# spcl/gms

Hardware: AMD Instinct MI355X
Metric: edges-intersected/sec + achieved HBM GB/s, RMAT-26 triangle count @1/2/4/8 GPU (higher is better)
Workload: dtype int32 ids / uint64 counts

## Files before the change

### gms_amd/capi.py

```python
import ctypes as C
import os
import weakref

import numpy as np

_HERE = os.path.dirname(os.path.abspath(__file__))
LIB_PATH = os.environ.get("GMSX_LIB") or os.path.join(_HERE, "lib", "libgmsx.so")

_i64p = np.ctypeslib.ndpointer(np.int64, flags="C_CONTIGUOUS")
_i32p = np.ctypeslib.ndpointer(np.int32, flags="C_CONTIGUOUS")
_u32p = np.ctypeslib.ndpointer(np.uint32, flags="C_CONTIGUOUS")

GEN_KRONECKER, GEN_UNIFORM = 0, 1
RELABEL_NEVER, RELABEL_AUTO, RELABEL_ALWAYS = 0, 1, 2
TC_AUTO, TC_ORIENTED, TC_FULL = 0, 1, 2
UPLOAD_DEFAULT, UPLOAD_TRUSTED, UPLOAD_FOR_TC = 0, 1, 2
PREPARE_TC = 1
SETOP_INTERSECT, SETOP_DIFFERENCE = 0, 1
OK, ERR_INVALID, ERR_NOMEM, ERR_IO, ERR_FORMAT, ERR_DIRECTED, ERR_NO_DEVICE = 0, -1, -2, -3, -4, -5, -6
ERR_DEVICE_MEM, ERR_NOT_CANONICAL, ERR_OVERFLOW, ERR_UNSUPPORTED, ERR_KERNEL, ERR_COMM, ERR_TIMEOUT = -7, -8, -9, -10, -11, -12, -13
COMM_ID_BYTES = 128

SYMBOLS = [
    "gmsx_strerror", "gmsx_version",
# ... 348 lines not shown
        _check(lib().gmsx_csr_save_sgx(self._h, os.fsencode(path)), "gmsx_csr_save_sgx")

    @property
    def is_mapped(self):
        return bool(lib().gmsx_csr_is_mapped(self._h))

    def relabel_by_degree(self):
        h = C.c_void_p()
        _check(lib().gmsx_csr_relabel_by_degree(self._h, C.byref(h)), "gmsx_csr_relabel_by_degree")
        return HostCSR(h)

    def worth_relabelling(self):
        return bool(lib().gmsx_csr_worth_relabelling(self._h))

    @property
    def num_nodes(self):
        return lib().gmsx_csr_num_nodes(self._h)

    @property
    def num_edges(self):
        return lib().gmsx_csr_num_edges(self._h)

    @property
    def nnz(self):
        return lib().gmsx_csr_num_edges_directed(self._h)

    def offsets(self):
        return np.ctypeslib.as_array(lib().gmsx_csr_offsets(self._h), shape=(self.num_nodes + 1,))

    def neighbors(self):
        nnz = self.nnz
        if nnz == 0:
            return np.zeros(0, dtype=np.int32)
        return np.ctypeslib.as_array(lib().gmsx_csr_neighbors(self._h), shape=(nnz,))

    def merge_elements(self):
        return int(lib().gmsx_csr_merge_elements(self._h))

    def fingerprint(self):
        return int(lib().gmsx_csr_fingerprint(self._h, 0)), int(lib().gmsx_csr_fingerprint(self._h, 1))

    def __del__(self):
        if getattr(self, "_h", None):
            lib().gmsx_csr_free(self._h)
            self._h = None


def set_host_threads(n=0):
    return int(lib().gmsx_set_host_threads(int(n)))


def set_option(name, value):
    _check(lib().gmsx_set_option(name.encode(), None if value is None else str(value).encode()), f"gmsx_set_option({name})")


def reset_options():
    lib().gmsx_reset_options()


def option_names():
    out, i, p = [], 0, C.c_char_p()
    while lib().gmsx_option_name(i, C.byref(p)) == 0:
        out.append(p.value.decode())
        i += 1
    return out


class options:

    def __init__(self, **kw):
        self.kw = kw

    def __enter__(self):
        for k, v in self.kw.items():
            set_option(k, v)
        return self

    def __exit__(self, *exc):
        for k in self.kw:
            set_option(k, None)
        return False


def init(device=-1):
    _check(lib().gmsx_init(device), "gmsx_init")


def set_stream(stream_ptr):
    _check(lib().gmsx_set_stream(C.c_void_p(stream_ptr)), "gmsx_set_stream")


def hbm_read_probe(nbytes=4 << 30, iterations=20):
    v = C.c_double(0)
    _check(lib().gmsx_hbm_read_probe(int(nbytes), int(iterations), C.byref(v)), "gmsx_hbm_read_probe")
    return v.value


def device_info():
    name = C.create_string_buffer(256)
    cu, mem = C.c_int(0), C.c_int64(0)
    _check(lib().gmsx_device_info(name, 256, C.byref(cu), C.byref(mem)), "gmsx_device_info")
    return {"name": name.value.decode(), "compute_units": cu.value, "hbm_bytes": mem.value}


class DeviceGraph:

    def __init__(self, handle):
        self._h = handle

    @classmethod
    def upload(cls, off, neigh, flags=UPLOAD_DEFAULT):
        off = np.ascontiguousarray(off, dtype=np.int64)
        neigh = np.ascontiguousarray(neigh, dtype=np.int32)
        h = C.c_void_p()
        _check(lib().gmsx_graph_upload(off.size - 1, off, neigh if neigh.size else np.zeros(1, np.int32), flags, C.byref(h)),
               "gmsx_graph_upload")
        g = cls(h)
        g._host = (weakref.ref(off), weakref.ref(neigh))
        return g

    @classmethod
    def from_csr(cls, csr, flags=UPLOAD_DEFAULT, shard=None):
        h = C.c_void_p()
        if shard is None:
            _check(lib().gmsx_graph_upload_csr(csr._h, flags, C.byref(h)), "gmsx_graph_upload_csr")
        else:
            _check(lib().gmsx_graph_upload_csr_shard(csr._h, flags, int(shard[0]), int(shard[1]), C.byref(h)), "gmsx_graph_upload_csr_shard")
        g = cls(h)
        g._host = (weakref.ref(csr),)
        return g

    num_nodes = property(lambda self: lib().gmsx_graph_num_nodes(self._h))
    num_edges = property(lambda self: lib().gmsx_graph_num_edges(self._h))
    device_bytes = property(lambda self: lib().gmsx_graph_device_bytes(self._h))
    max_out_degree = property(lambda self: lib().gmsx_graph_max_out_degree(self._h))
    tc_passes = property(lambda self: lib().gmsx_graph_tc_passes(self._h))

    def prepare(self, what=PREPARE_TC):
        _check(lib().gmsx_graph_prepare(self._h, what), "gmsx_graph_prepare")

    def tc_total(self, algo=TC_AUTO, stats=False):
        out, st = C.c_uint64(0), Stats()
        _check(lib().gmsx_tc_total(self._h, algo, C.byref(out), C.byref(st)), "gmsx_tc_total")
        return (int(out.value), st.as_dict()) if stats else int(out.value)

    def tc_partial(self, part, nparts, algo=TC_AUTO, stats=False):
        out, st = C.c_uint64(0), Stats()
        _check(lib().gmsx_tc_partial(self._h, algo, part, nparts, C.byref(out), C.byref(st)), "gmsx_tc_partial")
        return (int(out.value), st.as_dict()) if stats else int(out.value)

    BREAKDOWN = ["hub_rows_list", "hub_rows_bitset", "hub_rows_delta", "tail_rows_list", "tail_rows_delta", "entries", "pivot_containers",
                 "of_which_inline_rows", "light_streamed_hub_rows", "light_streamed_tail_rows", "light_pivot_lists_and_descriptors",
                 "count_entries", "count_inline_entries", "count_work_items", "count_light_streamed_members",
                 "core_matrix", "core_k", "reserved17", "reserved18", "reserved19", "reserved20"]
    BREAKDOWN_BYTES = ("hub_rows_list", "hub_rows_bitset", "hub_rows_delta", "tail_rows_list", "tail_rows_delta", "entries", "pivot_containers",
                       "light_streamed_hub_rows", "light_streamed_tail_rows", "light_pivot_lists_and_descriptors", "core_matrix")

    def tc_stream_breakdown(self):
        out = np.zeros(21, dtype=np.uint64)
        _check(lib().gmsx_tc_stream_breakdown(self._h, out), "gmsx_tc_stream_breakdown")
        return dict(zip(self.BREAKDOWN, (int(x) for x in out)))

    def tc_row_histogram(self):
        out = np.zeros(256, dtype=np.uint64)
        _check(lib().gmsx_tc_row_histogram(self._h, out), "gmsx_tc_row_histogram")
        return out[:240].reshape(5, 24, 2).astype(np.int64), out[240:].astype(np.int64)

    def tc_comembership(self, batch):
        out = np.zeros(8, dtype=np.uint64)
        _check(lib().gmsx_tc_comembership(self._h, int(batch), out), "gmsx_tc_comembership")
        return dict(entries=int(out[0]), units=int(out[1]), distinct_rows=int(out[2]), batched_units=int(out[3]), items=int(out[4]))

    def tc_vertex_count2(self, stats=False):
        c, st = np.zeros(self.num_nodes, dtype=np.int64), Stats()
        _check(lib().gmsx_tc_vertex_count2(self._h, c, C.byref(st)), "gmsx_tc_vertex_count2")
        return (c, st.as_dict()) if stats else c

    def intersect_count_batch(self, u, v, stats=False):
        u = np.ascontiguousarray(u, dtype=np.int32)
        v = np.ascontiguousarray(v, dtype=np.int32)
        out, st = np.zeros(max(u.size, 1), dtype=np.uint32), Stats()
        _check(lib().gmsx_intersect_count_batch(self._h, u.size, u if u.size else np.zeros(1, np.int32),
                                                v if v.size else np.zeros(1, np.int32), out, C.byref(st)),
               "gmsx_intersect_count_batch")
        out = out[:u.size]
        return (out, st.as_dict()) if stats else out

    def set_op_batch(self, op, u, v, stats=False):
        code = {"intersect": SETOP_INTERSECT, "difference": SETOP_DIFFERENCE}[op]
        u = np.ascontiguousarray(u, dtype=np.int32)
        v = np.ascontiguousarray(v, dtype=np.int32)
        uu, vv = (u if u.size else np.zeros(1, np.int32)), (v if v.size else np.zeros(1, np.int32))
        off, st = np.zeros(u.size + 1, dtype=np.int64), Stats()
        _check(lib().gmsx_set_op_batch(self._h, code, u.size, uu, vv, off, None, 0, C.byref(st)), "gmsx_set_op_batch (sizing)")
        ids = np.zeros(max(int(off[-1]), 1), dtype=np.int32)
        _check(lib().gmsx_set_op_batch(self._h, code, u.size, uu, vv, off, ids.ctypes.data_as(C.c_void_p), int(off[-1]), C.byref(st)), "gmsx_set_op_batch")
        ids = ids[:int(off[-1])]
        return (off, ids, st.as_dict()) if stats else (off, ids)

    SIM = {"jaccard": 0, "overlap": 1, "adamic_adar": 2, "resource": 3, "common_neighbors": 4, "total_neighbors": 5, "pref_attachment": 6}

    def vertex_similarity_batch(self, metric, u, v, stats=False):
        u = np.ascontiguousarray(u, dtype=np.int32)
        v = np.ascontiguousarray(v, dtype=np.int32)
        out, st = np.zeros(max(u.size, 1), dtype=np.float64), Stats()
        m = self.SIM[metric] if isinstance(metric, str) else int(metric)
        _check(lib().gmsx_vertex_similarity_batch(self._h, m, u.size, u if u.size else np.zeros(1, np.int32),
                                                  v if v.size else np.zeros(1, np.int32), out, C.byref(st)), "gmsx_vertex_similarity_batch")
        out = out[:u.size]
        return (out, st.as_dict()) if stats else out

    def kclique_count(self, k, stats=False):
        ordered, cliques, st = C.c_uint64(0), C.c_uint64(0), Stats()
        _check(lib().gmsx_kclique_count(self._h, k, C.byref(ordered), C.byref(cliques), C.byref(st)), "gmsx_kclique_count")
        r = (int(ordered.value), int(cliques.value))
        return (r + (st.as_dict(),)) if stats else r

    def kclique_star_count(self, k, members=True, stats=False):
        stars, mem, st = C.c_uint64(0), C.c_uint64(0), Stats()
        _check(lib().gmsx_kclique_star_count(self._h, k, C.byref(stars), C.byref(mem) if members else None, C.byref(st)), "gmsx_kclique_star_count")
        r = (int(stars.value), int(mem.value) if members else None)
        return (r + (st.as_dict(),)) if stats else r

    def kclique_star_list_info(self, k, cliques_only=False, part=0, nparts=1):
        info = KcliqueStarListInfo()
        flags = KCSTAR_CLIQUES_ONLY if cliques_only else KCSTAR_DEFAULT
        _check(lib().gmsx_kclique_star_list(self._h, k, flags, part, nparts, None, None, None, 0, 0, C.byref(info), None),
               "gmsx_kclique_star_list (sizing)")
        return info.as_dict()

    def kclique_star_list(self, k, cliques_only=False, part=0, nparts=1, stats=False):
        info, st = KcliqueStarListInfo(), Stats()
        flags = KCSTAR_CLIQUES_ONLY if cliques_only else KCSTAR_DEFAULT
        _check(lib().gmsx_kclique_star_list(self._h, k, flags, part, nparts, None, None, None, 0, 0, C.byref(info), C.byref(st)),
               "gmsx_kclique_star_list (sizing)")
        sizing = st.as_dict()
        nc, nm = int(info.cliques), int(info.star_members)
        cl = np.zeros(max(nc * k, 1), dtype=np.int32)
        soff = mem = None
        if not cliques_only:
            soff = np.zeros(nc + 1, dtype=np.int64)
            mem = np.zeros(max(nm, 1), dtype=np.int32)
        _check(lib().gmsx_kclique_star_list(self._h, k, flags, part, nparts, cl.ctypes.data_as(C.c_void_p),
                                            None if cliques_only else soff.ctypes.data_as(C.c_void_p),
                                            None if cliques_only else mem.ctypes.data_as(C.c_void_p), nc, nm, C.byref(info), C.byref(st)),
               "gmsx_kclique_star_list")
        cl = cl[:nc * k].reshape(nc, k)
        if mem is not None:
            mem = mem[:nm]
        if stats:
            return cl, soff, mem, {"sizing": sizing, "fill": st.as_dict(), "info": info.as_dict()}
        return cl, soff, mem

    def kclique_partial(self, k, part, nparts, stats=False):
        out, st = C.c_uint64(0), Stats()
        _check(lib().gmsx_kclique_partial(self._h, k, part, nparts, C.byref(out), C.byref(st)), "gmsx_kclique_partial")
        return (int(out.value), st.as_dict()) if stats else int(out.value)

    def bk_count(self, rank=None, stats=False):
        out, st = C.c_uint64(0), Stats()
        rp = None
        if rank is not None:
            rank = np.ascontiguousarray(rank, dtype=np.int32)
            rp = rank.ctypes.data_as(C.c_void_p)
        _check(lib().gmsx_bk_count(self._h, rp, C.byref(out), C.byref(st)), "gmsx_bk_count")
        return (int(out.value), st.as_dict()) if stats else int(out.value)

    def bk_partial(self, part, nparts, rank=None, stats=False):
        out, st = C.c_uint64(0), Stats()
        rp = None
        if rank is not None:
            rank = np.ascontiguousarray(rank, dtype=np.int32)
            rp = rank.ctypes.data_as(C.c_void_p)
        _check(lib().gmsx_bk_partial(self._h, rp, part, nparts, C.byref(out), C.byref(st)), "gmsx_bk_partial")
        return (int(out.value), st.as_dict()) if stats else int(out.value)

    def bk_list_info(self, rank=None, part=0, nparts=1):
        info = BkListInfo()
        rp = None
        if rank is not None:
            rank = np.ascontiguousarray(rank, dtype=np.int32)
            rp = rank.ctypes.data_as(C.c_void_p)
        _check(lib().gmsx_bk_list(self._h, rp, part, nparts, None, None, 0, 0, C.byref(info), None), "gmsx_bk_list (sizing)")
        return info.as_dict()

    def bk_list(self, rank=None, part=0, nparts=1, stats=False):
        info, st = BkListInfo(), Stats()
        rp = None
        if rank is not None:
            rank = np.ascontiguousarray(rank, dtype=np.int32)
            rp = rank.ctypes.data_as(C.c_void_p)
        _check(lib().gmsx_bk_list(self._h, rp, part, nparts, None, None, 0, 0, C.byref(info), C.byref(st)), "gmsx_bk_list (sizing)")
        sizing = st.as_dict()
        off = np.zeros(int(info.cliques) + 1, dtype=np.int64)
        mem = np.zeros(max(int(info.members), 1), dtype=np.int32)
        _check(lib().gmsx_bk_list(self._h, rp, part, nparts, off.ctypes.data_as(C.c_void_p), mem.ctypes.data_as(C.c_void_p), off.size,
                                  int(info.members), C.byref(info), C.byref(st)), "gmsx_bk_list")
        mem = mem[:int(info.members)]
        if stats:
            return off, mem, {"sizing": sizing, "fill": st.as_dict(), "info": info.as_dict()}
        return off, mem

    def adg_rank(self, epsilon=0.001, rank_format=True, stats=False):
        out, rounds, st = np.zeros(max(self.num_nodes, 1), dtype=np.int32), C.c_int32(0), Stats()
        _check(lib().gmsx_adg_rank(self._h, float(epsilon), int(bool(rank_format)), out, C.byref(rounds), C.byref(st)), "gmsx_adg_rank")
        r = (out[:self.num_nodes], int(rounds.value))
        return (r + (st.as_dict(),)) if stats else r
# ... 257 lines not shown
```

### gms_amd/csrc/hip/device_graph.hip

```cpp
#include "device_graph.hpp"

#include <algorithm>
#include <mutex>
#include <array>
#include <chrono>
#include <cstdio>
#include <cstdlib>
#include <cstring>
#include <memory>
#include <new>
#include <random>

#include <rocprim/device/device_radix_sort.hpp>
#include <rocprim/device/device_scan.hpp>
#include <rocprim/device/device_segmented_radix_sort.hpp>
#include <rocprim/iterator/transform_iterator.hpp>

#include "../host/gmsx_internal.hpp"
#include "../host/tc_core_plan.hpp"
#include "kc4_mfma.hpp"

namespace gmsx {

Ctx &ctx() {
    static Ctx c;
    return c;
}

int ensure_init() { return ctx().device >= 0 ? GMSX_OK : gmsx_init(-1); }


__device__ __forceinline__ unsigned long long arc_mix(unsigned long long x) {
    x ^= x >> 30;
    x *= 0xbf58476d1ce4e5b9ull;
    x ^= x >> 27;
    x *= 0x94d049bb133111ebull;
    x ^= x >> 31;
    return x;
}
__global__ __launch_bounds__(256) void k_validate(int64_t n, const int64_t *__restrict__ off,
                                                  const int32_t *__restrict__ adj, int check_symmetry, unsigned long long key0,
                                                  unsigned long long key1,
                                                  unsigned long long *__restrict__ acc ) {
    const int lane = threadIdx.x & 63;
    const int64_t wave0 = (int64_t(blockIdx.x) * blockDim.x + threadIdx.x) >> 6;
    const int64_t nwaves = (int64_t(gridDim.x) * blockDim.x) >> 6;
    unsigned flags = 0;
    unsigned long long elems = 0;
    unsigned long long maxdeg = 0;
    unsigned long long f0 = 0, r0 = 0, f1 = 0, r1 = 0;
    for (int64_t u = wave0; u < n; u += nwaves) {
        const int64_t b = off[u], e = off[u + 1];
        const unsigned long long du = (unsigned long long)(e - b);
        if (du > maxdeg) maxdeg = du;
        if (lane == 0) elems += du * du;
        for (int64_t j = b + lane; j < e; j += 64) {
            const int32_t v = adj[j];
            if (v < 0 || v >= n) { flags |= 2; continue; }
            if (v == u) flags |= 4;
            if (j + 1 < e && adj[j + 1] <= v) flags |= 1;
            if (check_symmetry) {
                const unsigned long long uv = ((unsigned long long)uint32_t(u) << 32) | uint32_t(v), vu = ((unsigned long long)uint32_t(v) << 32) | uint32_t(u);
                f0 += arc_mix(uv ^ key0);
                r0 += arc_mix(vu ^ key0);
                f1 += arc_mix(uv * 0x9e3779b97f4a7c15ull + key1);
                r1 += arc_mix(vu * 0x9e3779b97f4a7c15ull + key1);
            }
        }
    }
    for (int s = 32; s > 0; s >>= 1) {
        elems += __shfl_down(elems, s);
        flags |= __shfl_down(flags, s);
        const unsigned long long o = __shfl_down(maxdeg, s);
        maxdeg = o > maxdeg ? o : maxdeg;
        f0 += __shfl_down(f0, s);
        r0 += __shfl_down(r0, s);
        f1 += __shfl_down(f1, s);
        r1 += __shfl_down(r1, s);
    }
    if (lane == 0) {
        if (flags) atomicOr(&acc[0], (unsigned long long)flags);
        if (elems) atomicAdd(&acc[1], elems);
        atomicMax(&acc[2], maxdeg);
        if (check_symmetry) {
            atomicAdd(&acc[3], f0);
            atomicAdd(&acc[4], r0);
            atomicAdd(&acc[5], f1);
            atomicAdd(&acc[6], r1);
        }
    }
}

__global__ void k_rank_keys(int64_t n, const int64_t *__restrict__ off, unsigned long long *__restrict__ keys) {
    const int64_t u = int64_t(blockIdx.x) * blockDim.x + threadIdx.x;
    if (u < n) keys[u] = ((unsigned long long)(off[u + 1] - off[u]) << 32) | (unsigned long long)u;
}
__global__ void k_assign_ids(int64_t n, const unsigned long long *__restrict__ sorted_keys, int32_t *__restrict__ oldid,
                             int32_t *__restrict__ newid) {
    const int64_t i = int64_t(blockIdx.x) * blockDim.x + threadIdx.x;
    if (i < n) {
        const int32_t o = int32_t(sorted_keys[i] & 0xffffffffull);
        oldid[i] = o;
        newid[o] = int32_t(i);
    }
}

__global__ __launch_bounds__(256) void k_count_parts(int64_t n, const int64_t *__restrict__ off, const int32_t *__restrict__ adj,
                                                     const int32_t *__restrict__ newid, int hub_limit, int64_t *__restrict__ hcnt,
                                                     int64_t *__restrict__ tcnt, int32_t *__restrict__ dplus) {
    const int lane = threadIdx.x & 63;
    const int64_t wave0 = (int64_t(blockIdx.x) * blockDim.x + threadIdx.x) >> 6;
    const int64_t nwaves = (int64_t(gridDim.x) * blockDim.x) >> 6;
    for (int64_t u = wave0; u < n; u += nwaves) {
        const int64_t b = off[u], e = off[u + 1];
        const int32_t nu = newid[u];
        int ch = 0, ct = 0;
        for (int64_t j = b + lane; j < e; j += 64) {
            const int32_t nv = newid[adj[j]];
            if (nv < nu) {
                if (nv < hub_limit) ch++; else ct++;
            }
        }
        for (int s = 32; s > 0; s >>= 1) {
            ch += __shfl_down(ch, s);
            ct += __shfl_down(ct, s);
        }
        if (lane == 0) {
            hcnt[nu] = (ch + 1) & ~1;
            tcnt[nu] = ct;
            dplus[nu] = ch + ct;
        }
    }
}

__global__ __launch_bounds__(256) void k_fill_parts(int64_t n, const int64_t *__restrict__ off, const int32_t *__restrict__ adj,
                                                    const int32_t *__restrict__ newid, int hub_limit, const int64_t *__restrict__ hoff,
                                                    const int64_t *__restrict__ toff, uint16_t *__restrict__ hadj,
                                                    int32_t *__restrict__ tadj) {
    const int lane = threadIdx.x & 63;
    const int64_t wave0 = (int64_t(blockIdx.x) * blockDim.x + threadIdx.x) >> 6;
    const int64_t nwaves = (int64_t(gridDim.x) * blockDim.x) >> 6;
    for (int64_t u = wave0; u < n; u += nwaves) {
        const int64_t b = off[u], e = off[u + 1];
        const int32_t nu = newid[u];
        int64_t ho = hoff[nu], to = toff[nu];
        const int64_t hend = hoff[nu + 1];
        for (int64_t base = b; base < e; base += 64) {
            const int64_t j = base + lane;
            bool kh = false, kt = false;
            int32_t nv = 0;
            if (j < e) {
                nv = newid[adj[j]];
                kh = nv < nu && nv < hub_limit;
                kt = nv < nu && nv >= hub_limit;
            }
            const unsigned long long mh = __ballot(kh), mt = __ballot(kt);
            const unsigned long long below = (1ull << lane) - 1ull;
            if (kh) hadj[ho + __popcll(mh & below)] = uint16_t(nv);
            if (kt) tadj[to + __popcll(mt & below)] = nv;
            ho += __popcll(mh);
            to += __popcll(mt);
        }
        if (lane == 0 && ho < hend) hadj[ho] = 0xFFFF;
    }
}

__device__ inline uint32_t delta_encode(const uint16_t *__restrict__ row, int len, uint32_t *__restrict__ emit) {
    uint32_t units = 0;
    int i = 0;
    while (i < len && row[i] != 0xFFFFu) {
        uint32_t w[4] = {row[i], 0u, 0u, 0u};
        uint32_t cur = row[i];
// ... 212 lines not shown
    else
        for (int64_t w = 0; w < units * 4; ++w) dst[w] = w < len ? uint32_t(tadj[b + w]) : 0xfffffffeu;
}

__global__ void k_dense_sizes(int32_t limit, const int32_t *__restrict__ dplus, int64_t *__restrict__ sizes) {
    const int32_t v = int32_t(blockIdx.x * blockDim.x + threadIdx.x);
    if (v < limit) sizes[v] = bitset_words(v);
    if (v == limit) sizes[v] = 0;
}
__global__ __launch_bounds__(256) void k_dense_fill(int32_t limit, const int64_t *__restrict__ hoff, const uint16_t *__restrict__ hadj,
                                                    const int64_t *__restrict__ toff, const int32_t *__restrict__ tadj,
                                                    const int64_t *__restrict__ bmoff, uint32_t *__restrict__ pool) {
    const int lane = threadIdx.x & 63;
    const int32_t wave0 = int32_t((int64_t(blockIdx.x) * blockDim.x + threadIdx.x) >> 6);
    const int32_t nwaves = int32_t((int64_t(gridDim.x) * blockDim.x) >> 6);
    for (int32_t v = wave0; v < limit; v += nwaves) {
        const int64_t b = bmoff[v];
        if (bmoff[v + 1] == b) continue;
        for (int64_t j = hoff[v] + lane; j < hoff[v + 1]; j += 64) {
            const uint32_t id = hadj[j];
            if (id != 0xFFFFu) atomicOr(&pool[b + (id >> 5)], 1u << (id & 31u));
        }
        for (int64_t j = toff[v] + lane; j < toff[v + 1]; j += 64) {
            const uint32_t id = uint32_t(tadj[j]);
            atomicOr(&pool[b + (id >> 5)], 1u << (id & 31u));
        }
    }
}
__global__ __launch_bounds__(256) void k_core_fill(int32_t K, int WS, const int64_t *__restrict__ hoff, const uint16_t *__restrict__ hadj,
                                                   uint32_t *__restrict__ bits) {
    const int lane = threadIdx.x & 63;
    const int32_t wave0 = int32_t((int64_t(blockIdx.x) * blockDim.x + threadIdx.x) >> 6);
    const int32_t nwaves = int32_t((int64_t(gridDim.x) * blockDim.x) >> 6);
    for (int32_t i = wave0; i < K; i += nwaves)
        for (int64_t j = hoff[i] + lane; j < hoff[i + 1]; j += 64) {
            const uint32_t id = hadj[j];
            if (id < uint32_t(i)) atomicOr(&bits[size_t(i) * size_t(WS) + (id >> 5)], 1u << (id & 31u));
        }
}
__global__ __launch_bounds__(256) void k_core_units(int32_t cap, const int64_t *__restrict__ hoff, const uint16_t *__restrict__ hadj,
                                                    const int32_t *__restrict__ dplus, unsigned long long *__restrict__ bucket) {
    const int lane = threadIdx.x & 63;
    const int32_t wave0 = int32_t((int64_t(blockIdx.x) * blockDim.x + threadIdx.x) >> 6);
    const int32_t nwaves = int32_t((int64_t(gridDim.x) * blockDim.x) >> 6);
    for (int32_t u = wave0; u < cap; u += nwaves) {
        const int64_t hb = hoff[u];
        const int hl = int(hoff[u + 1] - hb);
        unsigned long long units = 0;
        for (int i = lane; i < hl; i += 64) {
            const uint32_t v = hadj[hb + i];
            if (v >= uint32_t(u)) continue;
            const uint32_t ids = uint32_t(min(i, dplus[v]));
            units += min((ids + 7u) / 8u, (v + 127u) / 128u);
        }
        for (int s = 32; s > 0; s >>= 1) units += __shfl_down(units, s);
        if (lane == 0 && units) atomicAdd(&bucket[u / kTcCoreBucket], units);
    }
}
__global__ __launch_bounds__(256) void k_tail_split(int64_t n, const int64_t *__restrict__ toff, const int32_t *__restrict__ tadj, int32_t limit,
                                                    int32_t *__restrict__ tsplit) {
    const int lane = threadIdx.x & 63;
    const int64_t wave0 = (int64_t(blockIdx.x) * blockDim.x + threadIdx.x) >> 6;
    const int64_t nwaves = (int64_t(gridDim.x) * blockDim.x) >> 6;
    for (int64_t u = wave0; u < n; u += nwaves) {
        int c = 0;
        for (int64_t j = toff[u] + lane; j < toff[u + 1]; j += 64) c += tadj[j] < limit;
        for (int s = 32; s > 0; s >>= 1) c += __shfl_down(c, s);
        if (lane == 0) tsplit[u] = c;
    }
}

__global__ void k_order_keys(int64_t n, const int32_t *__restrict__ dplus, int32_t *__restrict__ keys, int32_t *__restrict__ vals) {
    const int64_t i = int64_t(blockIdx.x) * blockDim.x + threadIdx.x;
    if (i < n) {
        keys[i] = dplus[i];
        vals[i] = int32_t(i);
    }
}

__global__ void k_warm(unsigned long long *p) {
    if (p) p[0] = 0;
}
__global__ void k_count_ge(int64_t n, const int32_t *__restrict__ order, const int32_t *__restrict__ dplus, int32_t thr, int64_t *__restrict__ out) {
    int64_t lo = 0, hi = n;
    while (lo < hi) {
        const int64_t mid = (lo + hi) >> 1;
        if (dplus[order[mid]] >= thr) lo = mid + 1; else hi = mid;
    }
    out[0] = lo;
}
__global__ void k_task_limits(int64_t n, const unsigned long long *__restrict__ srow, const unsigned long long *__restrict__ srow2,
                              const unsigned long long *__restrict__ trow, uint32_t hub_max, uint32_t tail_max, unsigned long long *__restrict__ out) {
    const int64_t v = int64_t(blockIdx.x) * blockDim.x + threadIdx.x;
    if (v >= n) return;
    if ((srow[v] & 0x3fffffull) > hub_max || (srow2[v] & 0x3fffffull) > hub_max || (trow[v] & 0x3fffffull) > tail_max) atomicOr(out, 1ull);
}

static constexpr int kInlineChunk = 64;
static constexpr int kDefaultInlineFirst = 28;
static constexpr int kInlineFirstMax = 64;
__device__ __forceinline__ bool takes_inline(int32_t v, int32_t inline_limit, const int32_t *__restrict__ dplus) {
    return v < inline_limit || dplus[v] >= kHeavy;
}
template <bool FILL>
__global__ __launch_bounds__(256) void k_inline_rows(int64_t first, int64_t end, const int32_t *__restrict__ order, const int64_t *__restrict__ hoff,
                                                     const uint16_t *__restrict__ hadj, const int64_t *__restrict__ toff, const int32_t *__restrict__ tadj,
                                                     const int32_t *__restrict__ dplus, int32_t inline_limit, int inline_first, int32_t core, const int32_t *__restrict__ opos, int nparts, int part,
                                                     unsigned long long *__restrict__ cnt_h,
                                                     unsigned long long *__restrict__ cnt_t, const int64_t *__restrict__ ihoff,
                                                     const int64_t *__restrict__ itoff, int64_t base_h, uint16_t *__restrict__ pool_h, int64_t base_t,
                                                     int32_t *__restrict__ pool_t) {
    const int lane = threadIdx.x & 63;
    const int64_t wave0 = (int64_t(blockIdx.x) * blockDim.x + threadIdx.x) >> 6;
    const int64_t nwaves = (int64_t(gridDim.x) * blockDim.x) >> 6;
    for (int64_t pos = first + wave0; pos < end; pos += nwaves) {
        const int32_t u = order[pos];
        if (u < core) continue;
        const int64_t hb = hoff[u], tb = toff[u];
        const int first_u = dplus[u] >= kHeavy ? inline_first : kInlineFirstMax;
        const int hl = min(int(hoff[u + 1] - hb), first_u), tl = min(int(toff[u + 1] - tb), first_u - hl);
        int32_t mv = 0x7fffffff;
        if (lane < hl) {
            const uint32_t x = hadj[hb + lane];
            if (x != 0xFFFFu) mv = int32_t(x);
        } else if (lane - hl < tl) {
            mv = tadj[tb + (lane - hl)];
        }
        const bool valid = mv != 0x7fffffff, is_tail = valid && lane >= hl;
        const unsigned long long vmask = __ballot(valid);
        const int nhub = __popcll(__ballot(valid && lane < hl));
        const int below = __popcll(vmask & ((1ull << lane) - 1ull));
        const bool give = valid && below > 0 && takes_inline(mv, inline_limit, dplus);
        const bool mine = give && (nparts <= 1 || shard_of(opos[mv], nparts) == part);
        const int nh = mine ? (is_tail ? nhub : below) : 0;
        const int nt = mine && is_tail ? lane - hl : 0;
        if (!FILL) {
            if (nh) atomicAdd(&cnt_h[mv], (unsigned long long)nh);
            if (nt) atomicAdd(&cnt_t[mv], (unsigned long long)nt);
        } else {
            int64_t at_h = 0, at_t = 0;
            if (nh) at_h = (base_h + ihoff[mv]) * 8 + int64_t(atomicAdd(&cnt_h[mv], (unsigned long long)nh));
            if (nt) at_t = (base_t + itoff[mv]) * 4 + int64_t(atomicAdd(&cnt_t[mv], (unsigned long long)nt));
            for (int k = 0; k < nhub; ++k) {
                const int32_t x = __shfl(mv, k);
                if (k < nh) pool_h[at_h + k] = uint16_t(x);
            }
            for (int k = 0; k < tl; ++k) {
                const int32_t x = __shfl(mv, hl + k);
                if (k < nt) pool_t[at_t + k] = x;
            }
        }
    }
}
__global__ void k_inline_units(int64_t n, const unsigned long long *__restrict__ ids_h, const unsigned long long *__restrict__ ids_t,
                               int64_t *__restrict__ units_h, int64_t *__restrict__ units_t) {
    const int64_t v = int64_t(blockIdx.x) * blockDim.x + threadIdx.x;
    if (v > n) return;
    units_h[v] = v < n ? int64_t((ids_h[v] + 7) / 8) : 0;
    units_t[v] = v < n ? int64_t((ids_t[v] + 3) / 4) : 0;
}
static constexpr int kDefaultHotWindows = 0, kDefaultHotKB = 2048, kDefaultHotMin = 16;
__device__ __forceinline__ int64_t receiver_of(int32_t w, const int32_t *__restrict__ dplus, const int32_t *__restrict__ opos, const int64_t *__restrict__ lidx,
                                               int64_t n_heavy) {
    return dplus[w] >= kHeavy ? int64_t(opos[w]) : n_heavy + lidx[w];
}
__global__ void k_opos(int64_t n, const int32_t *__restrict__ order, int32_t *__restrict__ opos) {
    const int64_t p = int64_t(blockIdx.x) * blockDim.x + threadIdx.x;
    if (p < n) opos[order[p]] = int32_t(p);
}
__global__ void k_light_flags(int64_t limit, const int32_t *__restrict__ dplus, int64_t *__restrict__ flags) {
    const int64_t w = int64_t(blockIdx.x) * blockDim.x + threadIdx.x;
    if (w <= limit) flags[w] = (w < limit && dplus[w] < kHeavy) ? 1 : 0;
}
__global__ void k_recv_vertices(int64_t n_heavy, int64_t limit, const int32_t *__restrict__ order, const int32_t *__restrict__ dplus, const int64_t *__restrict__ lidx,
                                int32_t *__restrict__ recv_v) {
    const int64_t i = int64_t(blockIdx.x) * blockDim.x + threadIdx.x;
    if (i < n_heavy) recv_v[i] = order[i];
    if (i < limit && dplus[i] < kHeavy) recv_v[n_heavy + lidx[i]] = int32_t(i);
}
template <bool FILL>
__global__ void k_inline_entries(int64_t n, const int32_t *__restrict__ dplus, const int32_t *__restrict__ opos, const int64_t *__restrict__ lidx, int64_t n_heavy,
                                 int32_t inline_limit, const int64_t *__restrict__ ihoff, const int64_t *__restrict__ itoff, int64_t base_h, int64_t base_t,
                                 uint32_t *__restrict__ cnt, uint32_t *__restrict__ cur, const int64_t *__restrict__ hbeg, const int64_t *__restrict__ tbeg,
                                 TaskList htask, TaskList ttask, unsigned long long *__restrict__ totals, TcClasses cc) {
    const int kClasses = cc.count();
    const int64_t v = int64_t(blockIdx.x) * blockDim.x + threadIdx.x;
    if (v >= n) return;
    const int64_t uh = ihoff[v + 1] - ihoff[v], ut = itoff[v + 1] - itoff[v];
    if (uh == 0 && ut == 0) return;
    if (dplus[v] < kHeavy && v >= inline_limit) return;
    const int64_t p = receiver_of(int32_t(v), dplus, opos, lidx, n_heavy);
    uint32_t *c = cnt + p * kClasses;
    for (int64_t o = 0; o < uh; o += kInlineChunk) {
        const unsigned long long units = (unsigned long long)min(int64_t(kInlineChunk), uh - o);
        const unsigned long long d = ((unsigned long long)(base_h + ihoff[v] + o) << 24) | ((unsigned long long)kFormList << 22) | units;
        const int cls = hub_class(cc, d);
        if (!FILL) atomicAdd(&c[cls], 1u);
        else htask.put(hbeg[p] + c[cls] + atomicAdd(&cur[p * kClasses + cls], 1u), d);
    }
    for (int64_t o = 0; o < ut; o += kInlineChunk) {
        const unsigned long long units = (unsigned long long)min(int64_t(kInlineChunk), ut - o);
        const unsigned long long d = ((unsigned long long)(base_t + itoff[v] + o) << 24) | ((unsigned long long)kFormList << 22) | units;
        const int cls = tail_class(cc, d);
        if (!FILL) atomicAdd(&c[cls], 1u);
        else ttask.put(tbeg[p] + c[cls] + atomicAdd(&cur[p * kClasses + cls], 1u), d);
    }
    if (!FILL) {
        atomicAdd(&totals[0], (unsigned long long)((uh + kInlineChunk - 1) / kInlineChunk));
        atomicAdd(&totals[1], (unsigned long long)((ut + kInlineChunk - 1) / kInlineChunk));
    }
}
__global__ void k_list_sizes(int64_t n_recv, uint32_t *__restrict__ cnt, int64_t *__restrict__ hcnt, int64_t *__restrict__ tcnt, TcClasses cc) {
    const int kClasses = cc.count(), hub_end = cc.tail_base();
    const int64_t p = int64_t(blockIdx.x) * blockDim.x + threadIdx.x;
    if (p > n_recv) return;
    if (p == n_recv) { hcnt[p] = 0; tcnt[p] = 0; return; }
    uint32_t *c = cnt + p * kClasses;
    uint32_t run = 0;
    for (int k = 0; k < hub_end; ++k) { const uint32_t x = c[k]; c[k] = run; run += x; }
    hcnt[p] = run;
    run = 0;
    for (int k = hub_end; k < kClasses; ++k) { const uint32_t x = c[k]; c[k] = run; run += x; }
    tcnt[p] = run;
}

__global__ void k_ledge_count(int64_t first, int64_t end, const int32_t *__restrict__ order, const int64_t *__restrict__ toff, const int32_t *__restrict__ tadj,
                              const int32_t *__restrict__ tsplit, const int32_t *__restrict__ dplus, int32_t core, int64_t *__restrict__ cnt) {
    const int64_t pos = first + int64_t(blockIdx.x) * blockDim.x + threadIdx.x;
    if (pos > end) return;
    int64_t c = 0;
    if (pos < end) {
        const int32_t u = order[pos];
        const int64_t tb = toff[u];
        const int tl = int(toff[u + 1] - tb);
        if (u >= core)
            for (int i = tsplit[u]; i < tl; ++i) c += dplus[tadj[tb + i]] < kHeavy ? 1 : 0;
    }
    cnt[pos - first] = c;
}
__global__ void k_ledge_fill(int64_t first, int64_t end, const int32_t *__restrict__ order, const int64_t *__restrict__ hoff, const int64_t *__restrict__ toff,
                             const int32_t *__restrict__ tadj, const int32_t *__restrict__ tsplit, const int32_t *__restrict__ dplus,
                             int32_t core, const int64_t *__restrict__ ebeg, int nparts, int part, uint4 *__restrict__ ledge) {
    const int64_t pos = first + int64_t(blockIdx.x) * blockDim.x + threadIdx.x;
    if (pos >= end) return;
    const int32_t u = order[pos];
    if (u < core) return;
    const int64_t hb = hoff[u], tb = toff[u];
    const int tl = int(toff[u + 1] - tb);
    const unsigned long long hu = (unsigned long long)hb | ((unsigned long long)(hoff[u + 1] - hb) << 40);
    int64_t e = ebeg[pos - first];
    for (int i = tsplit[u]; i < tl; ++i) {
        const int32_t v = tadj[tb + i];
        if (dplus[v] >= kHeavy) continue;
        if (nparts <= 1 || shard_of(e, nparts) == part) {
            const unsigned long long tu = (unsigned long long)tb | ((unsigned long long)i << 40);
            const unsigned long long hv = (unsigned long long)hoff[v] | ((unsigned long long)(hoff[v + 1] - hoff[v]) << 40);
            const unsigned long long tv = (unsigned long long)toff[v] | ((unsigned long long)(toff[v + 1] - toff[v]) << 40);
            const int64_t slot = nparts <= 1 ? e : e / nparts;
            ledge[2 * slot] = make_uint4(uint32_t(hu), uint32_t(hu >> 32), uint32_t(tu), uint32_t(tu >> 32));
            ledge[2 * slot + 1] = make_uint4(uint32_t(hv), uint32_t(hv >> 32), uint32_t(tv), uint32_t(tv >> 32));
        }
        ++e;
    }
}

__global__ void k_lpack_count(int64_t first, int64_t end, const int32_t *__restrict__ order, const int64_t *__restrict__ hoff, const uint16_t *__restrict__ hadj,
                              const int64_t *__restrict__ toff, const int32_t *__restrict__ tadj, const int32_t *__restrict__ tsplit, const int32_t *__restrict__ dplus,
                              int32_t core, int64_t *__restrict__ cnt) {
    const int64_t p = int64_t(blockIdx.x) * blockDim.x + threadIdx.x, nl = end - first;
    if (p >= nl) return;
    int64_t c[kLightClasses];
#pragma unroll
    for (int k = 0; k < kLightClasses; ++k) c[k] = 0;
    const int32_t u = order[first + p];
    if (u >= core) {
        const int64_t tb = toff[u];
        const int tl = int(toff[u + 1] - tb), ah = light_hub_ids(hoff, hadj, u);
        for (int i = tsplit[u]; i < tl; ++i) {
            const int32_t v = tadj[tb + i];
            if (dplus[v] >= kHeavy) continue;
            const int cls = light_class(ah, i, light_hub_ids(hoff, hadj, v), int(toff[v + 1] - toff[v]));
#pragma unroll
            for (int k = 0; k < kLightClasses; ++k) c[k] += cls == k ? 1 : 0;
        }
    }
#pragma unroll
    for (int k = 0; k < kLightClasses; ++k) cnt[int64_t(k) * nl + p] = c[k];
}
struct LpackPlan {
    int64_t class_beg[kLightClasses];
    int64_t unit_base[kLightClasses];
};
__device__ __forceinline__ uint4 lpack_hub_unit(const uint16_t *__restrict__ row, int len, int q) {
    uint32_t w[4];
#pragma unroll
    for (int j = 0; j < 4; ++j) {
        const int i = 8 * q + 2 * j;
        const uint32_t lo = i < len ? row[i] : 0xFFFFu, hi = i + 1 < len ? row[i + 1] : 0xFFFFu;
        w[j] = lo | (hi << 16);
    }
    return make_uint4(w[0], w[1], w[2], w[3]);
}
__device__ __forceinline__ uint4 lpack_tail_unit(const int32_t *__restrict__ row, int len, int q, uint32_t filler) {
    uint32_t w[4];
#pragma unroll
    for (int j = 0; j < 4; ++j) w[j] = 4 * q + j < len ? uint32_t(row[4 * q + j]) : filler;
    return make_uint4(w[0], w[1], w[2], w[3]);
}
__global__ void k_lpack_fill(int64_t first, int64_t end, const int32_t *__restrict__ order, const int64_t *__restrict__ hoff, const uint16_t *__restrict__ hadj,
                             const int64_t *__restrict__ toff, const int32_t *__restrict__ tadj, const int32_t *__restrict__ tsplit, const int32_t *__restrict__ dplus,
                             int32_t core, const int64_t *__restrict__ beg, const LpackPlan plan, int nparts, int part, uint4 *__restrict__ lpack) {
    const int64_t p = int64_t(blockIdx.x) * blockDim.x + threadIdx.x, nl = end - first;
    if (p >= nl) return;
    const int32_t u = order[first + p];
    if (u < core) return;
    int64_t next[kLightClasses];
#pragma unroll
    for (int k = 0; k < kLightClasses; ++k) next[k] = beg[int64_t(k) * nl + p] - plan.class_beg[k];
    const int64_t hb = hoff[u], tb = toff[u];
    const int tl = int(toff[u + 1] - tb), ah = light_hub_ids(hoff, hadj, u);
    for (int i = tsplit[u]; i < tl; ++i) {
        const int32_t v = tadj[tb + i];
        if (dplus[v] >= kHeavy) continue;
        const int64_t hv = hoff[v], tv = toff[v];
        const int bh = light_hub_ids(hoff, hadj, v), bt = int(toff[v + 1] - tv);
        const int cls = light_class(ah, i, bh, bt);
        int64_t k = 0, base = 0;
#pragma unroll
        for (int c = 0; c < kLightClasses; ++c)
            if (cls == c) {
                k = next[c]++;
                base = plan.unit_base[c];
            }
        if (nparts > 1 && shard_of(k, nparts) != part) continue;
        const LightShape sh = light_shape(cls);
        uint4 *blk = lpack + base + (nparts <= 1 ? k : k / nparts) * sh.stride();
        for (int q = 0; q < sh.ah; ++q) *blk++ = lpack_hub_unit(hadj + hb, ah, q);
        for (int q = 0; q < sh.at; ++q) *blk++ = lpack_tail_unit(tadj + tb, i, q, 0xFFFFFFFFu);
        for (int q = 0; q < sh.bh; ++q) *blk++ = lpack_hub_unit(hadj + hv, bh, q);
        for (int q = 0; q < sh.bt; ++q) *blk++ = lpack_tail_unit(tadj + tv, bt, q, 0xFFFFFFFEu);
    }
}

__device__ __forceinline__ uint32_t cut_hub_units(const uint32_t *__restrict__ spool, unsigned long long d, int below, int32_t v) {
    const uint32_t units = uint32_t(d) & 0x3fffffu, form = (uint32_t(d) >> 22) & 3u;
    if (form == kFormList) return min(units, uint32_t(below + 7) / 8u);
    if (form == kFormBitset) return min(units, uint32_t(v + 127) / 128u);
    const uint4 *row = reinterpret_cast<const uint4 *>(spool) + (d >> 24);
    uint32_t lo = 0, hi = units;
    while (lo < hi) {
        const uint32_t mid = (lo + hi) >> 1;
        if (int32_t(row[mid].x & 0xffffu) < v) lo = mid + 1; else hi = mid;
    }
    return lo;
}
__device__ __forceinline__ uint32_t cut_tail_units(const uint32_t *__restrict__ tpool, unsigned long long d, int below, int32_t v) {
    const uint32_t units = uint32_t(d) & 0x3fffffu, form = (uint32_t(d) >> 22) & 3u;
    if (form != kFormDelta) return min(units, uint32_t(below + 3) / 4u);
    const uint4 *row = reinterpret_cast<const uint4 *>(tpool) + (d >> 24);
    uint32_t lo = 0, hi = units;
    while (lo < hi) {
        const uint32_t mid = (lo + hi) >> 1;
        if (int32_t(row[mid].x) < v) lo = mid + 1; else hi = mid;
    }
    return lo;
}
__device__ __forceinline__ uint32_t claim_by_class(uint32_t *ctr, int cls, bool active, int lane) {
    uint32_t mine = 0;
    unsigned long long todo = __ballot(active);
    while (todo) {
        const int leader = __ffsll((long long)todo) - 1;
        const int c = __builtin_amdgcn_readlane(cls, leader);
        const unsigned long long same = __ballot(active && cls == c);
        uint32_t base = 0;
        if (lane == leader) base = atomicAdd(&ctr[c], uint32_t(__popcll(same)));
        base = uint32_t(__builtin_amdgcn_readlane(int(base), leader));
        if (active && cls == c) mine = base + uint32_t(__popcll(same & ((1ull << lane) - 1ull)));
        todo &= ~same;
    }
    return mine;
}
template <bool FILL>
__global__ __launch_bounds__(256) void k_task_lists(int64_t n_heavy, const int32_t *__restrict__ order, const int64_t *__restrict__ hoff,
                                                    const uint16_t *__restrict__ hadj, const int64_t *__restrict__ toff, const int32_t *__restrict__ tadj,
                                                    const int32_t *__restrict__ dplus, const unsigned long long *__restrict__ srow,
                                                    const unsigned long long *__restrict__ srow2, const int32_t *__restrict__ ksplit,
                                                    const unsigned long long *__restrict__ trow, int two_sided, const int32_t *__restrict__ opos,
                                                    uint32_t *__restrict__ cnt, uint32_t *__restrict__ cur, const int64_t *__restrict__ hbeg,
                                                    const int64_t *__restrict__ tbeg, TaskList htask, TaskList ttask,
                                                    int32_t *__restrict__ tunits, unsigned long long *__restrict__ reversed, const uint32_t *__restrict__ spool,
                                                    const uint32_t *__restrict__ tpool, int32_t inline_limit, int inline_first, int32_t core, int nparts, int part, TcClasses cc) {
    const int kClasses = cc.count();
    const int lane = threadIdx.x & 63;
    const int64_t wave0 = (int64_t(blockIdx.x) * blockDim.x + threadIdx.x) >> 6;
    const int64_t nwaves = (int64_t(gridDim.x) * blockDim.x) >> 6;
    unsigned long long rev = 0;
    for (int64_t pos = wave0; pos < n_heavy; pos += nwaves) {
        const int32_t u = order[pos];
        if (u < core) continue;
        const int64_t hb = hoff[u], tb = toff[u];
        const int hl = int(hoff[u + 1] - hb), tl = int(toff[u + 1] - tb);
        const unsigned long long du_s = srow[u], du_s2 = srow2[u], du_t = trow[u];
        const int ks_u = ksplit[u];
        uint32_t *cu = cnt + pos * kClasses, *ru = cur + pos * kClasses;
        const bool own_u = nparts <= 1 || shard_of(pos, nparts) == part;
        int kept = 0;
        for (int base = 0; base < hl + tl; base += 64) {
            const int i = base + lane;
            int32_t v = -1;
            if (i < hl) {
                const uint32_t x = hadj[hb + i];
                if (x != 0xFFFFu) v = int32_t(x);
            } else if (i < hl + tl) v = tadj[tb + i - hl];
            if (v >= 0 && i > 0 && i < inline_first && takes_inline(v, inline_limit, dplus)) v = -1;
            bool reverse = false;
            uint32_t ch = 0, ch2 = 0, ct = 0;
            if (v >= 0 && i > 0 && two_sided && dplus[v] >= kHeavy) {
                if (i < hl) {
                    ch = cut_hub_units(spool, du_s, i, v);
                    if (du_s2 && i > ks_u) ch2 = cut_hub_units(spool, du_s2, i - ks_u, v);
                } else {
                    ch = uint32_t(du_s) & 0x3fffffu;
                    ch2 = uint32_t(du_s2) & 0x3fffffu;
                }
                ct = (i < hl || toff[v + 1] == toff[v]) ? 0u : cut_tail_units(tpool, du_t, i - hl, v);
                const uint32_t keep = uint32_t(srow[v] & 0x3fffffull) + uint32_t(srow2[v] & 0x3fffffull) + (i > hl ? uint32_t(trow[v] & 0x3fffffull) : 0u);
                reverse = ch + ch2 + ct < keep;
            }
            const bool fwd = v >= 0 && !reverse && own_u;
            if (reverse && nparts > 1 && shard_of(opos[v], nparts) != part) v = -1;
            const unsigned long long fh = (fwd && i > 0) ? srow[v] : 0ull, fh2 = (fwd && i > 0) ? srow2[v] : 0ull, ft = (fwd && i > hl) ? trow[v] : 0ull;
            const bool fh_on = (fh & 0x3fffffull) != 0, fh2_on = (fh2 & 0x3fffffull) != 0, ft_on = (ft & 0x3fffffull) != 0;
            const uint32_t sh = claim_by_class(FILL ? ru : cu, hub_class(cc, fh), fh_on, lane);
            const uint32_t sh2 = claim_by_class(FILL ? ru : cu, hub_class(cc, fh2), fh2_on, lane);
            const uint32_t st = claim_by_class(FILL ? ru : cu, tail_class(cc, ft), ft_on, lane);
            if (FILL) {
                if (fh_on) htask.put(hbeg[pos] + cu[hub_class(cc, fh)] + sh, fh);
                if (fh2_on) htask.put(hbeg[pos] + cu[hub_class(cc, fh2)] + sh2, fh2);
                if (ft_on) ttask.put(tbeg[pos] + cu[tail_class(cc, ft)] + st, ft);
            }
            kept += __popcll(__ballot(fwd));
            if (v >= 0 && reverse) {
                const int64_t pv = opos[v];
                const unsigned long long rh = ch ? (du_s & ~0x3fffffull) | ch : 0ull, rh2 = ch2 ? (du_s2 & ~0x3fffffull) | ch2 : 0ull,
                                         rt = ct ? (du_t & ~0x3fffffull) | ct : 0ull;
                uint32_t *cv = cnt + pv * kClasses;
                if (!FILL) {
                    if (rh) atomicAdd(&cv[hub_class(cc, rh)], 1u);
                    if (rh2) atomicAdd(&cv[hub_class(cc, rh2)], 1u);
                    if (rt) atomicAdd(&cv[tail_class(cc, rt)], 1u);
                    atomicAdd(&tunits[pv], 1);
                    ++rev;
                } else {
                    uint32_t *rv = cur + pv * kClasses;
                    if (rh) htask.put(hbeg[pv] + cv[hub_class(cc, rh)] + atomicAdd(&rv[hub_class(cc, rh)], 1u), rh);
                    if (rh2) htask.put(hbeg[pv] + cv[hub_class(cc, rh2)] + atomicAdd(&rv[hub_class(cc, rh2)], 1u), rh2);
                    if (rt) ttask.put(tbeg[pv] + cv[tail_class(cc, rt)] + atomicAdd(&rv[tail_class(cc, rt)], 1u), rt);
                }
            }
        }
        if (!FILL && lane == 0 && kept) atomicAdd(&tunits[pos], kept);
    }
    if (!FILL) {
        for (int s = 32; s > 0; s >>= 1) rev += __shfl_down(rev, s);
        if (lane == 0 && rev) atomicAdd(reversed, rev);
    }
}
__global__ void k_item_counts(int64_t n_recv, const int64_t *__restrict__ lbeg, const uint32_t *__restrict__ cnt, TcClasses cc, int phases, int64_t *__restrict__ items) {
    const int64_t p = int64_t(blockIdx.x) * blockDim.x + threadIdx.x;
    if (p > n_recv) return;
    if (p == n_recv) { items[int64_t(phases) * n_recv] = 0; return; }
    for (int ph = 0; ph < phases; ++ph) {
        int64_t b = 0, e = lbeg[p + 1] - lbeg[p];
        if (phases > 1) hub_phase_range(cc, cnt + p * cc.count(), e, ph, &b, &e);
        items[int64_t(ph) * n_recv + p] = (e - b + kTaskChunk - 1) / kTaskChunk;
    }
}
__global__ void k_item_fill(int64_t n_recv, const int32_t *__restrict__ recv_v, const int32_t *__restrict__ opos, const int64_t *__restrict__ lbeg,
                            const int64_t *__restrict__ ioff, TaskList task, const int64_t *__restrict__ coff, int kind,
                            const uint32_t *__restrict__ cnt, TcClasses cc, int phases, gmsx_tc_item *__restrict__ items) {
    const int64_t p = int64_t(blockIdx.x) * blockDim.x + threadIdx.x;
    if (p >= n_recv) return;
    const int32_t w = recv_v[p];
    const uint64_t cont = uint64_t(coff[w]) | (uint64_t(coff[w + 1] - coff[w]) << 40);
    for (int ph = 0; ph < phases; ++ph) {
    int64_t b = 0, e = lbeg[p + 1] - lbeg[p];
    if (phases > 1) hub_phase_range(cc, cnt + p * cc.count(), e, ph, &b, &e);
    b += lbeg[p];
    e += lbeg[p];
    int64_t k = ioff[int64_t(ph) * n_recv + p];
    for (int64_t x = b; x < e; x += kTaskChunk, ++k) {
        const int ne = int(min(int64_t(kTaskChunk), e - x));
        gmsx_tc_item it{};
        it.bc = uint64_t(x) | (uint64_t(ne) << 40);
        it.cont = cont;
        it.pivot = w;
        it.pos = opos[w];
        it.kind = uint32_t(kind);
        for (int f = 0; f < 4; ++f) {
            int lo = 0, hi = ne;
            while (lo < hi) {
                const int mid = (lo + hi) >> 1;
                if (int((uint32_t(task.get(x + mid)) >> 22) & 3u) < f) lo = mid + 1; else hi = mid;
            }
            it.fbeg[f] = uint16_t(lo);
        }
        items[k] = it;
    }
    }
}

static int grid_for_waves(int64_t rows) {
    const int64_t want = (rows + 3) / 4;
    const int64_t cap = int64_t(ctx().compute_units > 0 ? ctx().compute_units : 256) * 32;
    return int(want < 1 ? 1 : (want > cap ? cap : want));
}

template <class T>
static int dmalloc(T **p, int64_t count, gmsx_graph *g, int line = __builtin_LINE()) {
    const size_t bytes = size_t(count > 0 ? count : 1) * sizeof(T);
    const bool trace = opt("MEM_TRACE") != nullptr;
    if (trace && g && bytes >= (1u << 20)) std::fprintf(stderr, "gmsx mem: device_graph.hip:%d %.3f GB (elements of %zu B)\n", line, double(bytes) * 1e-9, sizeof(T));
    if (g && g->tc_building && g->tc_limit_bytes > 0 && g->device_bytes + int64_t(bytes) - g->tc_base_bytes > g->tc_limit_bytes) {
        *p = nullptr;
        return GMSX_ERR_DEVICE_MEM;
    }
    if (hipMalloc(reinterpret_cast<void **>(p), bytes) != hipSuccess) {
        (void)hipGetLastError();
        *p = nullptr;
        return GMSX_ERR_DEVICE_MEM;
    }
    if (g) g->device_bytes += int64_t(bytes);
    return GMSX_OK;
}

struct DevGuard {
    void *p;
    ~DevGuard() { (void)hipFree(p); }
};

static void free_tc(gmsx_graph *g) {
    auto drop = [](auto *&p) {
        (void)hipFree(p);
        p = nullptr;
    };
    drop(g->tsplit); drop(g->srow); drop(g->srow2); drop(g->ksplit); drop(g->spool); drop(g->trow); drop(g->htask.lo); drop(g->htask.hi); drop(g->ttask.lo); drop(g->ttask.hi); drop(g->hitem); drop(g->titem); drop(g->tunits);
    drop(g->ledge); drop(g->lpack); drop(g->tpool); drop(g->shard_hitem); drop(g->shard_titem); drop(g->core_bits);
    g->tc_core = 0;
    g->shard_idx_part = g->shard_idx_nparts = -1;
    g->device_bytes -= g->tc_bytes;
    g->tc_bytes = 0;
    g->tc_ready = false;
    g->htask_entries = g->ttask_entries = g->hitems = g->titems = g->inline_hentries = g->inline_tentries = 0;
    g->n_ledge = g->ledge_total = 0;
    for (int c = 0; c < 8; ++c) g->lpack_base[c] = g->lpack_n[c] = g->lpack_total[c] = 0;
    g->task_reverse = g->inline_units = g->spool_units = g->tpool_units = 0;
    g->stats_part = g->stats_nparts = -1;
}

static void free_graph(gmsx_graph *g) {
    if (!g) return;
    (void)hipFree(g->off);
    (void)hipFree(g->adj);
    (void)hipFree(g->newid);
    (void)hipFree(g->oldid);
    (void)hipFree(g->hoff);
    (void)hipFree(g->hadj);
    (void)hipFree(g->toff);
    (void)hipFree(g->tadj);
    (void)hipFree(g->bmoff);
    (void)hipFree(g->bmpool);
    (void)hipFree(g->tsplit);
    (void)hipFree(g->srow);
    (void)hipFree(g->srow2);
    (void)hipFree(g->ksplit);
    (void)hipFree(g->spool);
    (void)hipFree(g->trow);
    (void)hipFree(g->htask.lo);
    (void)hipFree(g->htask.hi);
    (void)hipFree(g->ttask.lo);
    (void)hipFree(g->ttask.hi);
    (void)hipFree(g->hitem);
    (void)hipFree(g->titem);
    (void)hipFree(g->tunits);
    (void)hipFree(g->shard_hitem);
    (void)hipFree(g->shard_titem);
    (void)hipFree(g->ledge);
    (void)hipFree(g->lpack);
    (void)hipFree(g->core_bits);
    (void)hipFree(g->tpool);
    (void)hipFree(g->dplus);
    (void)hipFree(g->order);
    (void)hipFree(g->kc_rel);
    (void)hipFree(g->kc_aoff);
    (void)hipFree(g->kc_arena);
    (void)hipFree(g->kc_rec);
    (void)hipFree(g->kc_item);
    (void)hipFree(g->kc_relt);
    (void)hipFree(g->kc_rect);
    (void)hipFree(g->kc_itemt);
    (void)hipFree(g->scratch);
    (void)hipFree(g->acc);
    delete g;
}

int exclusive_scan_i64(const int64_t *in, int64_t *out, int64_t count, hipStream_t s) {
    size_t tmp_bytes = 0;
    GMSX_HIP(rocprim::exclusive_scan(nullptr, tmp_bytes, in, out, int64_t(0), size_t(count), rocprim::plus<int64_t>(), s));
    void *tmp = nullptr;
    GMSX_HIP(hipMalloc(&tmp, tmp_bytes ? tmp_bytes : 8));
    DevGuard g_tmp{tmp};
    GMSX_HIP(rocprim::exclusive_scan(tmp, tmp_bytes, in, out, int64_t(0), size_t(count), rocprim::plus<int64_t>(), s));
    GMSX_HIP(hipStreamSynchronize(s));
    return GMSX_OK;
}

struct OffsetMinus {
    int64_t base;
    __host__ __device__ int64_t operator()(int64_t x) const { return x - base; }
};
__global__ void k_lower_bound_i64(int64_t count, const int64_t *__restrict__ a, int64_t target, int64_t *__restrict__ out) {
    int64_t lo = 0, hi = count;
    while (lo < hi) {
        const int64_t mid = (lo + hi) >> 1;
        if (a[mid] < target) lo = mid + 1; else hi = mid;
    }
    out[0] = lo;
}
template <class K>
static int sort_rows(K *keys, int64_t entries, int64_t n, const int64_t *d_off, int end_bit, hipStream_t s) {
    if (n <= 0 || entries <= 0) return GMSX_OK;
    int64_t chunk = int64_t(1) << 31;
    if (const char *e = opt("SORT_CHUNK")) {
        const long long v = std::atoll(e);
        if (v > 0) chunk = v;
    }
    int64_t *d_v = nullptr;
    GMSX_HIP(hipMalloc(reinterpret_cast<void **>(&d_v), sizeof(int64_t)));
    DevGuard g_v{d_v};
    GMSX_HIP(hipStreamSynchronize(s));
    int64_t v0 = 0, base = 0;
    while (v0 < n) {
        int64_t v1 = n;
        if (entries - base > chunk) {
            hipLaunchKernelGGL(k_lower_bound_i64, dim3(1), dim3(1), 0, s, n + 1, d_off, base + chunk + 1, d_v);
            GMSX_HIP(hipStreamSynchronize(s));
            GMSX_HIP(hipMemcpy(&v1, d_v, sizeof(int64_t), hipMemcpyDeviceToHost));
            v1 = std::max(v0 + 1, std::min(n, v1 - 1));
        }
        int64_t end = 0;
        GMSX_HIP(hipMemcpy(&end, d_off + v1, sizeof(int64_t), hipMemcpyDeviceToHost));
        const int64_t cnt = end - base;
        if (cnt >= (int64_t(1) << 32)) return GMSX_ERR_UNSUPPORTED;
        if (cnt > 0) {
            K *sorted = nullptr;
            GMSX_HIP(hipMalloc(reinterpret_cast<void **>(&sorted), size_t(cnt) * sizeof(K)));
            DevGuard g_sorted{sorted};
            auto begin = rocprim::make_transform_iterator(d_off + v0, OffsetMinus{base});
            auto endit = rocprim::make_transform_iterator(d_off + v0 + 1, OffsetMinus{base});
            size_t tmp_bytes = 0;
            GMSX_HIP(rocprim::segmented_radix_sort_keys(nullptr, tmp_bytes, keys + base, sorted, unsigned(cnt), unsigned(v1 - v0), begin, endit, 0, end_bit, s));
            void *tmp = nullptr;
            GMSX_HIP(hipMalloc(&tmp, tmp_bytes ? tmp_bytes : 8));
            DevGuard g_tmp{tmp};
            GMSX_HIP(rocprim::segmented_radix_sort_keys(tmp, tmp_bytes, keys + base, sorted, unsigned(cnt), unsigned(v1 - v0), begin, endit, 0, end_bit, s));
            GMSX_HIP(hipMemcpyAsync(keys + base, sorted, size_t(cnt) * sizeof(K), hipMemcpyDeviceToDevice, s));
            GMSX_HIP(hipStreamSynchronize(s));
        }
        v0 = v1;
        base = end;
    }
    return GMSX_OK;
}

template <class K, class V>
static int sort_segment_pairs(K *keys, V *vals, int64_t entries, int64_t n, const int64_t *d_off, int end_bit, hipStream_t s) {
    if (n <= 0 || entries <= 0) return GMSX_OK;
    int64_t chunk = int64_t(1) << 31;
    if (const char *e = opt("SORT_CHUNK")) {
        const long long v = std::atoll(e);
        if (v > 0) chunk = v;
    }
    int64_t *d_v = nullptr;
    GMSX_HIP(hipMalloc(reinterpret_cast<void **>(&d_v), sizeof(int64_t)));
    DevGuard g_v{d_v};
    GMSX_HIP(hipStreamSynchronize(s));
    int64_t v0 = 0, base = 0;
    while (v0 < n) {
        int64_t v1 = n;
        if (entries - base > chunk) {
            hipLaunchKernelGGL(k_lower_bound_i64, dim3(1), dim3(1), 0, s, n + 1, d_off, base + chunk + 1, d_v);
            GMSX_HIP(hipStreamSynchronize(s));
            GMSX_HIP(hipMemcpy(&v1, d_v, sizeof(int64_t), hipMemcpyDeviceToHost));
            v1 = std::max(v0 + 1, std::min(n, v1 - 1));
        }
        int64_t end = 0;
        GMSX_HIP(hipMemcpy(&end, d_off + v1, sizeof(int64_t), hipMemcpyDeviceToHost));
        const int64_t cnt = end - base;
        if (cnt >= (int64_t(1) << 32)) return GMSX_ERR_UNSUPPORTED;
        if (cnt > 0) {
            K *k_out = nullptr;
            V *v_out = nullptr;
            GMSX_HIP(hipMalloc(reinterpret_cast<void **>(&k_out), size_t(cnt) * sizeof(K)));
            DevGuard g_ko{k_out};
            GMSX_HIP(hipMalloc(reinterpret_cast<void **>(&v_out), size_t(cnt) * sizeof(V)));
            DevGuard g_vo{v_out};
            auto begin = rocprim::make_transform_iterator(d_off + v0, OffsetMinus{base});
            auto endit = rocprim::make_transform_iterator(d_off + v0 + 1, OffsetMinus{base});
            size_t tmp_bytes = 0;
// ... 157 lines not shown
    GMSX_HIP(hipMemsetAsync(g->hadj + g->hub_entries, 0xff, 8 * sizeof(uint16_t), s));
    GMSX_HIP(hipMemsetAsync(g->tadj + g->tail_entries, 0xff, 4 * sizeof(int32_t), s));
    if (n > 0)
        hipLaunchKernelGGL(k_fill_parts, dim3(grid_for_waves(n)), dim3(256), 0, s, n, g->off, g->adj, g->newid, hub_limit, g->hoff, g->toff,
                           g->hadj, g->tadj);

    pt.mark("containers count+fill");
    if (int rc = sort_rows(g->hadj, g->hub_entries, n, g->hoff, 16, s)) return rc;
    if (int rc = sort_rows(g->tadj, g->tail_entries, n, g->toff, 32, s)) return rc;
    g->rows_sorted = true;

    pt.mark("row sorts");
    g->dense_limit = int32_t(std::min<int64_t>(n, hub_limit));
    g->bitset_limit = g->dense_limit;
    {
        const int32_t K = g->bitset_limit;
        int64_t *sizes = nullptr;
        if (int rc = dmalloc(&sizes, int64_t(K) + 1, nullptr)) return rc;
        DevGuard g_sz{sizes};
        if (int rc = dmalloc(&g->bmoff, int64_t(K) + 1, g)) return rc;
        hipLaunchKernelGGL(k_dense_sizes, dim3(unsigned(K / 256 + 1)), dim3(256), 0, s, K, g->dplus, sizes);
        if (int rc = exclusive_scan_i64(sizes, g->bmoff, int64_t(K) + 1, s)) return rc;
        GMSX_HIP(hipMemcpy(&g->bmpool_words, g->bmoff + K, sizeof(int64_t), hipMemcpyDeviceToHost));
        if (int rc = dmalloc(&g->bmpool, g->bmpool_words + 4, g)) return rc;
        GMSX_HIP(hipMemsetAsync(g->bmpool, 0, size_t(g->bmpool_words + 4) * sizeof(uint32_t), s));
        if (K > 0 && g->bmpool_words > 0)
            hipLaunchKernelGGL(k_dense_fill, dim3(grid_for_waves(K)), dim3(256), 0, s, K, g->hoff, g->hadj, g->toff, g->tadj, g->bmoff, g->bmpool);
    }
    pt.mark("bitsets");
    if (int rc = dmalloc(&g->order, n, g)) return rc;
    if (n > 0) {
        int32_t *keys_in = nullptr, *vals_in = nullptr, *keys_out = nullptr;
        if (int rc = dmalloc(&keys_out, n, nullptr)) return rc;
        DevGuard g_ko{keys_out};
        if (int rc = dmalloc(&keys_in, n, nullptr)) return rc;
        DevGuard g_ki{keys_in};
        if (int rc = dmalloc(&vals_in, n, nullptr)) return rc;
        DevGuard g_vi{vals_in};
        hipLaunchKernelGGL(k_order_keys, dim3(tb), dim3(256), 0, s, n, g->dplus, keys_in, vals_in);
        size_t tmp_bytes = 0;
        GMSX_HIP(rocprim::radix_sort_pairs_desc(nullptr, tmp_bytes, keys_in, keys_out, vals_in, g->order, size_t(n), 0, 32, s));
        void *tmp = nullptr;
        GMSX_HIP(hipMalloc(&tmp, tmp_bytes ? tmp_bytes : 8));
        DevGuard g_tmp{tmp};
        GMSX_HIP(rocprim::radix_sort_pairs_desc(tmp, tmp_bytes, keys_in, keys_out, vals_in, g->order, size_t(n), 0, 32, s));
        int32_t top = 0;
        GMSX_HIP(hipMemcpyAsync(&top, keys_out, sizeof(int32_t), hipMemcpyDeviceToHost, s));
        GMSX_HIP(hipStreamSynchronize(s));
        g->max_dplus = top;
    }

    pt.mark("d+ order");
    GMSX_HIP(hipStreamSynchronize(s));
    GMSX_HIP(hipGetLastError());
    g->hub_limit = hub_limit;
    g->upload_flags = flags;
    return GMSX_OK;
}

static int build_tc_sets(gmsx_graph *g) {
    hipStream_t s = ctx().stream;
    PhaseTimer pt(s, "tc build");
    const int64_t n = g->n;
    const uint32_t flags = g->upload_flags;
    const int hub_limit = g->hub_limit;
    const unsigned tb = unsigned((n + 255) / 256);
    int32_t *opos = nullptr;
    if (int rc = dmalloc(&opos, n + 1, nullptr)) return rc;
    DevGuard g_opos{opos};
    if (n > 0) hipLaunchKernelGGL(k_opos, dim3(tb), dim3(256), 0, s, n, g->order, opos);
    {
        long long want = kTcCoreDefault;
        if (const char *e = opt("TC_CORE")) want = std::atoll(e);
        g->tc_core = 0;
        if (want > 0) g->tc_core = tc_core_clamp(want, hub_limit, n);
        else if (want < 0) {
            const int cap = tc_core_clamp(kTcCoreCap, hub_limit, n) / kTcCoreBucket * kTcCoreBucket;
            if (cap > 0) {
                const int nbk = cap / kTcCoreBucket;
                unsigned long long *bucket = nullptr;
                if (int rc = dmalloc(&bucket, nbk, nullptr)) return rc;
                DevGuard g_b{bucket};
                GMSX_HIP(hipMemsetAsync(bucket, 0, size_t(nbk) * sizeof(unsigned long long), s));
                hipLaunchKernelGGL(k_core_units, dim3(grid_for_waves(cap)), dim3(256), 0, s, cap, g->hoff, g->hadj, g->dplus, bucket);
                std::vector<uint64_t> h(size_t(nbk), 0);
                static_assert(sizeof(uint64_t) == sizeof(unsigned long long), "bucket words");
                GMSX_HIP(hipMemcpyAsync(h.data(), bucket, size_t(nbk) * sizeof(uint64_t), hipMemcpyDeviceToHost, s));
                GMSX_HIP(hipStreamSynchronize(s));
                g->tc_core = choose_tc_core(h, cap);
            }
        }
        if (g->tc_core > 0) {
            const int32_t K = g->tc_core;
            const int WS = kc4m_stride(K);
            const int64_t words = int64_t(K) * WS + 8;
            if (int rc = dmalloc(&g->core_bits, words, g)) return rc;
            GMSX_HIP(hipMemsetAsync(g->core_bits, 0, size_t(words) * sizeof(uint32_t), s));
            hipLaunchKernelGGL(k_core_fill, dim3(grid_for_waves(K)), dim3(256), 0, s, K, WS, g->hoff, g->hadj, g->core_bits);
        }
    }
    pt.mark("core matrix");
    {
        int64_t want = std::min<int64_t>(524288, n / 256);
        bool forced = false;
        if (const char *e = opt("INLINE_LIMIT")) {
            const long long v = std::atoll(e);
            if (v >= 0 && v <= (1ll << 31) - 1) { want = v; forced = true; }
        }
        if (!forced && ((flags >> 8) & 0xffffu)) want = int64_t(4) * hub_limit;
        g->inline_limit = int32_t(std::min<int64_t>(n, std::max<int64_t>(want, g->dense_limit)));
        g->inline_first = kDefaultInlineFirst;
        if (const char *e = opt("TC_INLINE_FIRST")) g->inline_first = std::max(1, std::min(kInlineFirstMax, std::atoi(e)));
        if (int rc = dmalloc(&g->tsplit, n, g)) return rc;
        if (n > 0) hipLaunchKernelGGL(k_tail_split, dim3(grid_for_waves(n)), dim3(256), 0, s, n, g->toff, g->tadj, g->inline_limit, g->tsplit);
    }

    pt.mark("tail split");
    int64_t n_heavy = 0, n_work = 0;
    unsigned long long *inl_h = nullptr, *inl_t = nullptr;
    int64_t *ihoff = nullptr, *itoff = nullptr;
    if (int rc = dmalloc(&inl_h, n + 1, nullptr)) return rc;
    DevGuard g_inl_h{inl_h};
    if (int rc = dmalloc(&inl_t, n + 1, nullptr)) return rc;
    DevGuard g_inl_t{inl_t};
    if (int rc = dmalloc(&ihoff, n + 1, nullptr)) return rc;
    DevGuard g_ihoff{ihoff};
    if (int rc = dmalloc(&itoff, n + 1, nullptr)) return rc;
    DevGuard g_itoff{itoff};
    int64_t inline_h_units = 0, inline_t_units = 0;
    {
        if (n > 0) {
            int64_t *d_cnt = nullptr;
            if (int rc = dmalloc(&d_cnt, 2, nullptr)) return rc;
            DevGuard g_c{d_cnt};
            hipLaunchKernelGGL(k_count_ge, dim3(1), dim3(1), 0, s, n, g->order, g->dplus, int32_t(kHeavy), d_cnt);
            hipLaunchKernelGGL(k_count_ge, dim3(1), dim3(1), 0, s, n, g->order, g->dplus, int32_t(2), d_cnt + 1);
            GMSX_HIP(hipStreamSynchronize(s));
            int64_t h[2] = {0, 0};
            GMSX_HIP(hipMemcpy(h, d_cnt, sizeof(h), hipMemcpyDeviceToHost));
            n_heavy = h[0];
            n_work = h[1];
        }
        GMSX_HIP(hipMemsetAsync(inl_h, 0, size_t(n + 1) * sizeof(unsigned long long), s));
        GMSX_HIP(hipMemsetAsync(inl_t, 0, size_t(n + 1) * sizeof(unsigned long long), s));
        if (n_work > 0)
            hipLaunchKernelGGL(k_inline_rows<false>, dim3(grid_for_waves(n_work)), dim3(256), 0, s, int64_t(0), n_work, g->order, g->hoff, g->hadj,
                               g->toff, g->tadj, g->dplus, g->inline_limit, g->inline_first, g->tc_core, opos, g->shard_nparts, g->shard_part, inl_h, inl_t, ihoff, itoff, int64_t(0), static_cast<uint16_t *>(nullptr),
                               int64_t(0), static_cast<int32_t *>(nullptr));
        int64_t *uh = nullptr, *ut = nullptr;
        if (int rc = dmalloc(&uh, n + 1, nullptr)) return rc;
        DevGuard g_uh{uh};
        if (int rc = dmalloc(&ut, n + 1, nullptr)) return rc;
        DevGuard g_ut{ut};
        hipLaunchKernelGGL(k_inline_units, dim3(unsigned(n / 256 + 1)), dim3(256), 0, s, n, inl_h, inl_t, uh, ut);
        if (int rc = exclusive_scan_i64(uh, ihoff, n + 1, s)) return rc;
        if (int rc = exclusive_scan_i64(ut, itoff, n + 1, s)) return rc;
        GMSX_HIP(hipMemcpy(&inline_h_units, ihoff + n, sizeof(int64_t), hipMemcpyDeviceToHost));
        GMSX_HIP(hipMemcpy(&inline_t_units, itoff + n, sizeof(int64_t), hipMemcpyDeviceToHost));
        g->inline_units = inline_h_units + inline_t_units;
    }

    pt.mark("inline row sizes");
    int64_t inline_h_base = 0, inline_t_base = 0;
    {
        int delta_mode = g->rows_sorted ? 1 : 0;
        if (const char *e = opt("TC_DELTA")) {
            const int v = std::atoi(e);
            if (v >= 0 && v <= 2 && g->rows_sorted) delta_mode = v;
        }
        int delta_pct = 85;
        if (const char *e = opt("TC_DELTA_PCT")) {
            const int v = std::atoi(e);
            if (v >= 10 && v <= 100) delta_pct = v;
        }
        int gap12_mode = 0;
        if (const char *e = opt("TC_GAP12")) {
            const int v = std::atoi(e);
            if (v >= 0 && v <= 2 && g->rows_sorted) gap12_mode = v;
        }
        int hybrid_mode = 0;
        if (const char *e = opt("TC_HYBRID")) {
            const int v = std::atoi(e);
            if (v >= 0 && v <= 2 && g->rows_sorted) hybrid_mode = v;
        }
        int64_t *units = nullptr, *uoff = nullptr, *small = nullptr, *soff = nullptr;
        uint32_t *real = nullptr;
        unsigned char *form = nullptr;
        const int64_t n2 = 2 * n;
        if (int rc = dmalloc(&units, n2 + 1, nullptr)) return rc;
        DevGuard g_u{units};
        if (int rc = dmalloc(&uoff, n2 + 1, nullptr)) return rc;
        DevGuard g_o{uoff};
        if (int rc = dmalloc(&small, n2 + 1, nullptr)) return rc;
        DevGuard g_s{small};
        if (int rc = dmalloc(&soff, n2 + 1, nullptr)) return rc;
        DevGuard g_so{soff};
        if (int rc = dmalloc(&real, n2 + 1, nullptr)) return rc;
        DevGuard g_r{real};
        if (int rc = dmalloc(&form, n2 + 1, nullptr)) return rc;
        DevGuard g_f{form};
        if (int rc = dmalloc(&g->ksplit, n + 1, g)) return rc;
        hipLaunchKernelGGL(k_srow_sizes, dim3(unsigned(n / 256 + 1)), dim3(256), 0, s, n, g->hoff, g->hadj, g->dplus, g->dense_limit, delta_mode, delta_pct, gap12_mode,
                           hybrid_mode, units, small, real, form, g->ksplit);
        if (int rc = exclusive_scan_i64(units, uoff, n2 + 1, s)) return rc;
        if (int rc = exclusive_scan_i64(small, soff, n2 + 1, s)) return rc;
        int64_t big_units = 0, small_units = 0;
        GMSX_HIP(hipMemcpy(&big_units, uoff + n2, sizeof(int64_t), hipMemcpyDeviceToHost));
        GMSX_HIP(hipMemcpy(&small_units, soff + n2, sizeof(int64_t), hipMemcpyDeviceToHost));
        g->spool_units = big_units + small_units + inline_h_units;
        inline_h_base = big_units + small_units;
        if (g->spool_units >= (int64_t(1) << 40)) return GMSX_ERR_DEVICE_MEM;
        if (int rc = dmalloc(&g->srow, n, g)) return rc;
        if (int rc = dmalloc(&g->srow2, n, g)) return rc;
        if (int rc = dmalloc(&g->spool, (g->spool_units + kPoolSlack) * 4, g)) return rc;
        GMSX_HIP(hipMemsetAsync(g->spool, 0, size_t((g->spool_units + kPoolSlack) * 4) * sizeof(uint32_t), s));
        if (inline_h_units > 0) GMSX_HIP(hipMemsetAsync(g->spool + inline_h_base * 4, 0xff, size_t(inline_h_units) * 16, s));
        if (n > 0)
            hipLaunchKernelGGL(k_srow_fill, dim3(unsigned((n + 255) / 256)), dim3(256), 0, s, n, g->hoff, g->hadj, g->bmoff, g->bmpool, uoff, soff, real, form,
                               g->ksplit, g->srow, g->srow2, g->spool);
        GMSX_HIP(hipStreamSynchronize(s));
    }
    {
        int delta_mode = g->rows_sorted ? 1 : 0;
        if (const char *e = opt("TC_TAIL_DELTA")) {
            const int v = std::atoi(e);
            if (v >= 0 && v <= 2 && g->rows_sorted) delta_mode = v;
        }
        int64_t *units = nullptr, *uoff = nullptr, *small = nullptr, *soff = nullptr;
        uint32_t *real = nullptr;
        unsigned char *form = nullptr;
        if (int rc = dmalloc(&units, n + 1, nullptr)) return rc;
        DevGuard g_u{units};
        if (int rc = dmalloc(&uoff, n + 1, nullptr)) return rc;
        DevGuard g_o{uoff};
        if (int rc = dmalloc(&small, n + 1, nullptr)) return rc;
        DevGuard g_s{small};
        if (int rc = dmalloc(&soff, n + 1, nullptr)) return rc;
        DevGuard g_so{soff};
        if (int rc = dmalloc(&real, n + 1, nullptr)) return rc;
        DevGuard g_r{real};
        if (int rc = dmalloc(&form, n + 1, nullptr)) return rc;
        DevGuard g_f{form};
        hipLaunchKernelGGL(k_trow_sizes, dim3(unsigned(n / 256 + 1)), dim3(256), 0, s, n, g->toff, g->tadj, delta_mode, units, small, real, form);
        if (int rc = exclusive_scan_i64(units, uoff, n + 1, s)) return rc;
        if (int rc = exclusive_scan_i64(small, soff, n + 1, s)) return rc;
        int64_t big_units = 0, small_units = 0;
        GMSX_HIP(hipMemcpy(&big_units, uoff + n, sizeof(int64_t), hipMemcpyDeviceToHost));
        GMSX_HIP(hipMemcpy(&small_units, soff + n, sizeof(int64_t), hipMemcpyDeviceToHost));
        inline_t_base = big_units + small_units;
        g->tpool_units = inline_t_base + inline_t_units;
        if (g->tpool_units >= (int64_t(1) << 40)) return GMSX_ERR_DEVICE_MEM;
        if (int rc = dmalloc(&g->trow, n, g)) return rc;
        if (int rc = dmalloc(&g->tpool, (g->tpool_units + kPoolSlack) * 4, g)) return rc;
        GMSX_HIP(hipMemsetD32Async(reinterpret_cast<hipDeviceptr_t>(g->tpool), int(0xFFFFFFFEu), size_t(g->tpool_units + kPoolSlack) * 4, s));
        if (n > 0)
            hipLaunchKernelGGL(k_trow_fill, dim3(unsigned((n + 255) / 256)), dim3(256), 0, s, n, g->toff, g->tadj, uoff, soff, real, form, g->trow, g->tpool);
        GMSX_HIP(hipStreamSynchronize(s));
    }

    pt.mark("tail stream rows");
    if (n_work > 0) {
        GMSX_HIP(hipMemsetAsync(inl_h, 0, size_t(n + 1) * sizeof(unsigned long long), s));
        GMSX_HIP(hipMemsetAsync(inl_t, 0, size_t(n + 1) * sizeof(unsigned long long), s));
        hipLaunchKernelGGL(k_inline_rows<true>, dim3(grid_for_waves(n_work)), dim3(256), 0, s, int64_t(0), n_work, g->order, g->hoff, g->hadj, g->toff,
                           g->tadj, g->dplus, g->inline_limit, g->inline_first, g->tc_core, opos, g->shard_nparts, g->shard_part, inl_h, inl_t, ihoff, itoff, inline_h_base, reinterpret_cast<uint16_t *>(g->spool),
                           inline_t_base, reinterpret_cast<int32_t *>(g->tpool));
    }
    pt.mark("inline rows fill");
    {
        const int64_t nl = n_work - n_heavy;
        g->n_ledge = g->ledge_total = 0;
        g->light_packed = opt_int("TC_LIGHT_PACKED", 1) != 0;
        for (int c = 0; c < 8; ++c) g->lpack_base[c] = g->lpack_n[c] = g->lpack_total[c] = 0;
        if (nl > 0 && g->light_packed) {
            int64_t *ecnt = nullptr, *ebeg = nullptr;
            const int64_t cells = int64_t(kLightClasses) * nl;
            if (int rc = dmalloc(&ecnt, cells + 1, nullptr)) return rc;
            DevGuard g_ec{ecnt};
            if (int rc = dmalloc(&ebeg, cells + 1, nullptr)) return rc;
            DevGuard g_eb{ebeg};
            GMSX_HIP(hipMemsetAsync(ecnt + cells, 0, sizeof(int64_t), s));
            hipLaunchKernelGGL(k_lpack_count, dim3(unsigned(nl / 256 + 1)), dim3(256), 0, s, n_heavy, n_work, g->order, g->hoff, g->hadj, g->toff, g->tadj, g->tsplit, g->dplus,
                               g->tc_core, ecnt);
            if (int rc = exclusive_scan_i64(ecnt, ebeg, cells + 1, s)) return rc;
            const int np = g->shard_nparts > 1 ? g->shard_nparts : 1, pp = g->shard_nparts > 1 ? g->shard_part : 0;
            LpackPlan plan{};
            int64_t units = 0;
            for (int c = 0; c < kLightClasses; ++c) {
                int64_t b[2] = {0, 0};
                GMSX_HIP(hipMemcpy(&b[0], ebeg + int64_t(c) * nl, sizeof(int64_t), hipMemcpyDeviceToHost));
                GMSX_HIP(hipMemcpy(&b[1], ebeg + int64_t(c + 1) * nl, sizeof(int64_t), hipMemcpyDeviceToHost));
                const int64_t total = b[1] - b[0], full = total / np, rem = total % np;
                plan.class_beg[c] = b[0];
                plan.unit_base[c] = units;
                g->lpack_total[c] = total;
                g->lpack_n[c] = np <= 1 ? total : full + (((full & 1) ? np - 1 - pp : pp) < rem ? 1 : 0);
                g->lpack_base[c] = units;
                units += g->lpack_n[c] * light_shape(c).stride();
                g->ledge_total += total;
                g->n_ledge += g->lpack_n[c];
            }
            if (opt("MEM_TRACE"))
                for (int c = 0; c < kLightClasses; ++c) {
                    const LightShape k = light_shape(c);
                    std::fprintf(stderr, "gmsx light class %d (ids <= %d / %d / %d / %d, %d units): %lld blocks\n", c, 8 * k.ah, 4 * k.at, 8 * k.bh, 4 * k.bt, k.stride(),
                                 (long long)g->lpack_total[c]);
                }
            if (int rc = dmalloc(&g->lpack, units + 1, g)) return rc;
            hipLaunchKernelGGL(k_lpack_fill, dim3(unsigned(nl / 256 + 1)), dim3(256), 0, s, n_heavy, n_work, g->order, g->hoff, g->hadj, g->toff, g->tadj, g->tsplit, g->dplus,
                               g->tc_core, ebeg, plan, np, pp, g->lpack);
            GMSX_HIP(hipStreamSynchronize(s));
        } else if (nl > 0) {
            int64_t *ecnt = nullptr, *ebeg = nullptr;
            if (int rc = dmalloc(&ecnt, nl + 1, nullptr)) return rc;
            DevGuard g_ec{ecnt};
            if (int rc = dmalloc(&ebeg, nl + 1, nullptr)) return rc;
            DevGuard g_eb{ebeg};
            hipLaunchKernelGGL(k_ledge_count, dim3(unsigned(nl / 256 + 1)), dim3(256), 0, s, n_heavy, n_work, g->order, g->toff, g->tadj, g->tsplit, g->dplus, g->tc_core, ecnt);
            if (int rc = exclusive_scan_i64(ecnt, ebeg, nl + 1, s)) return rc;
            GMSX_HIP(hipMemcpy(&g->ledge_total, ebeg + nl, sizeof(int64_t), hipMemcpyDeviceToHost));
            const int np = g->shard_nparts > 1 ? g->shard_nparts : 1, pp = g->shard_nparts > 1 ? g->shard_part : 0;
            {
                const int64_t full = g->ledge_total / np, rem = g->ledge_total % np;
                g->n_ledge = np <= 1 ? g->ledge_total : full + (((full & 1) ? np - 1 - pp : pp) < rem ? 1 : 0);
            }
            if (int rc = dmalloc(&g->ledge, 2 * g->n_ledge + 2, g)) return rc;
            hipLaunchKernelGGL(k_ledge_fill, dim3(unsigned(nl / 256 + 1)), dim3(256), 0, s, n_heavy, n_work, g->order, g->hoff, g->toff, g->tadj, g->tsplit, g->dplus, g->tc_core, ebeg,
                               np, pp, g->ledge);
            GMSX_HIP(hipStreamSynchronize(s));
        }
    }
    pt.mark("light pivot list");
    {
        int two_sided = 1;
        if (const char *e = opt("TC_TWO_SIDED")) two_sided = std::atoi(e) != 0;
        const unsigned vb = unsigned(n / 256 + 1);
        const int64_t L = g->inline_limit;
        int64_t *lflag = nullptr, *lidx = nullptr;
        if (int rc = dmalloc(&lflag, L + 1, nullptr)) return rc;
        DevGuard g_lf{lflag};
        if (int rc = dmalloc(&lidx, L + 1, nullptr)) return rc;
        DevGuard g_li{lidx};
        hipLaunchKernelGGL(k_light_flags, dim3(unsigned(L / 256 + 1)), dim3(256), 0, s, L, g->dplus, lflag);
        if (int rc = exclusive_scan_i64(lflag, lidx, L + 1, s)) return rc;
        int64_t n_light_recv = 0;
        GMSX_HIP(hipMemcpy(&n_light_recv, lidx + L, sizeof(int64_t), hipMemcpyDeviceToHost));
        const int64_t n_recv = n_heavy + n_light_recv;
        int32_t *recv_v = nullptr;
        if (int rc = dmalloc(&recv_v, n_recv + 1, nullptr)) return rc;
        DevGuard g_rv{recv_v};
        if (std::max<int64_t>(n_heavy, L) > 0)
            hipLaunchKernelGGL(k_recv_vertices, dim3(unsigned(std::max<int64_t>(n_heavy, L) / 256 + 1)), dim3(256), 0, s, n_heavy, L, g->order, g->dplus, lidx, recv_v);
        {
            auto env_int = [](const char *name, int dflt) { return int(opt_int(name, dflt)); };
            g->tc_hot_windows = std::max(0, std::min(kMaxHotWindows, env_int("TC_HOT_WINDOWS", kDefaultHotWindows)));
            g->tc_window_units = uint32_t(std::max(1, env_int("TC_HOT_KB", kDefaultHotKB))) * 64u;
            g->tc_hot_min = std::max(1, env_int("TC_HOT_MIN", kDefaultHotMin));
        }
        const TcClasses cc{g->tc_hot_windows, g->tc_window_units, g->tc_hot_min};
        const int kClasses = cc.count();
        uint32_t *cnt = nullptr, *cur = nullptr;
        if (int rc = dmalloc(&cnt, n_recv * kClasses + 1, nullptr)) return rc;
        DevGuard g_cnt{cnt};
        if (int rc = dmalloc(&cur, n_recv * kClasses + 1, nullptr)) return rc;
        DevGuard g_cur{cur};
        GMSX_HIP(hipMemsetAsync(cnt, 0, size_t(n_recv * kClasses + 1) * sizeof(uint32_t), s));
        GMSX_HIP(hipMemsetAsync(cur, 0, size_t(n_recv * kClasses + 1) * sizeof(uint32_t), s));
        if (int rc = dmalloc(&g->tunits, n_heavy + 1, g)) return rc;
        GMSX_HIP(hipMemsetAsync(g->tunits, 0, size_t(n_heavy + 1) * sizeof(int32_t), s));
        unsigned long long *totals = nullptr;
        if (int rc = dmalloc(&totals, 4, nullptr)) return rc;
        DevGuard g_tot{totals};
        GMSX_HIP(hipMemsetAsync(totals, 0, 4 * sizeof(unsigned long long), s));
        int64_t *hcnt = nullptr, *tcnt = nullptr, *hbeg = nullptr, *tbeg = nullptr;
        if (int rc = dmalloc(&hcnt, n_recv + 1, nullptr)) return rc;
        DevGuard g_hc{hcnt};
        if (int rc = dmalloc(&tcnt, n_recv + 1, nullptr)) return rc;
        DevGuard g_tc{tcnt};
        if (int rc = dmalloc(&hbeg, n_recv + 1, nullptr)) return rc;
        DevGuard g_hb{hbeg};
        if (int rc = dmalloc(&tbeg, n_recv + 1, nullptr)) return rc;
        DevGuard g_tb{tbeg};
        const int grid = grid_for_waves(n_heavy);
        if (g->spool_units + kPoolSlack >= (int64_t(1) << 32) || g->tpool_units + kPoolSlack >= (int64_t(1) << 32)) return GMSX_ERR_DEVICE_MEM;
        {
            uint32_t hub_max = kTaskHubUnitsMax, tail_max = kTaskTailUnitsMax;
            if (const char *e = opt("TC_TEST_MAX_UNITS")) hub_max = tail_max = uint32_t(std::max(1, std::atoi(e)));
            if (n > 0) hipLaunchKernelGGL(k_task_limits, dim3(vb), dim3(256), 0, s, n, g->srow, g->srow2, g->trow, hub_max, tail_max, totals + 3);
        }
        if (n > 0)
            hipLaunchKernelGGL(k_inline_entries<false>, dim3(vb), dim3(256), 0, s, n, g->dplus, opos, lidx, n_heavy, g->inline_limit, ihoff, itoff, inline_h_base,
                               inline_t_base, cnt, cur, hbeg, tbeg, TaskList{}, TaskList{}, totals, cc);
        if (n_heavy > 0)
            hipLaunchKernelGGL(k_task_lists<false>, dim3(grid), dim3(256), 0, s, n_heavy, g->order, g->hoff, g->hadj, g->toff, g->tadj, g->dplus, g->srow, g->srow2, g->ksplit, g->trow,
                               two_sided, opos, cnt, cur, hbeg, tbeg, TaskList{}, TaskList{}, g->tunits,
                               totals + 2, g->spool, g->tpool, g->inline_limit, g->inline_first, g->tc_core, g->shard_nparts, g->shard_part, cc);
        pt.mark("task lists count");
        hipLaunchKernelGGL(k_list_sizes, dim3(unsigned(n_recv / 256 + 1)), dim3(256), 0, s, n_recv, cnt, hcnt, tcnt, cc);
        if (int rc = exclusive_scan_i64(hcnt, hbeg, n_recv + 1, s)) return rc;
        if (int rc = exclusive_scan_i64(tcnt, tbeg, n_recv + 1, s)) return rc;
        unsigned long long tot[4] = {0, 0, 0, 0};
        GMSX_HIP(hipMemcpy(&g->htask_entries, hbeg + n_recv, sizeof(int64_t), hipMemcpyDeviceToHost));
        GMSX_HIP(hipMemcpy(&g->ttask_entries, tbeg + n_recv, sizeof(int64_t), hipMemcpyDeviceToHost));
        GMSX_HIP(hipMemcpy(tot, totals, sizeof(tot), hipMemcpyDeviceToHost));
        if (tot[3]) return GMSX_ERR_UNSUPPORTED;
        g->inline_hentries = int64_t(tot[0]);
        g->inline_tentries = int64_t(tot[1]);
        g->task_reverse = int64_t(tot[2]);
        if (g->htask_entries >= (int64_t(1) << 40) || g->ttask_entries >= (int64_t(1) << 40)) return GMSX_ERR_DEVICE_MEM;
        if (int rc = dmalloc(&g->htask.lo, g->htask_entries + 2, g)) return rc;
        if (int rc = dmalloc(&g->htask.hi, g->htask_entries + 2, g)) return rc;
        if (int rc = dmalloc(&g->ttask.lo, g->ttask_entries + 2, g)) return rc;
        if (int rc = dmalloc(&g->ttask.hi, g->ttask_entries + 2, g)) return rc;
        if (n > 0)
            hipLaunchKernelGGL(k_inline_entries<true>, dim3(vb), dim3(256), 0, s, n, g->dplus, opos, lidx, n_heavy, g->inline_limit, ihoff, itoff, inline_h_base,
                               inline_t_base, cnt, cur, hbeg, tbeg, g->htask, g->ttask, totals, cc);
        if (n_heavy > 0)
            hipLaunchKernelGGL(k_task_lists<true>, dim3(grid), dim3(256), 0, s, n_heavy, g->order, g->hoff, g->hadj, g->toff, g->tadj, g->dplus, g->srow, g->srow2, g->ksplit, g->trow,
                               two_sided, opos, cnt, cur, hbeg, tbeg, g->htask, g->ttask, g->tunits, totals + 2, g->spool, g->tpool, g->inline_limit, g->inline_first, g->tc_core, g->shard_nparts, g->shard_part, cc);
        pt.mark("task lists fill");
        const int hub_phases = cc.hub_phases();
        const int64_t slots = int64_t(hub_phases) * n_recv;
        int64_t *icnt = nullptr, *ioff = nullptr;
        if (int rc = dmalloc(&icnt, slots + 1, nullptr)) return rc;
        DevGuard g_ic{icnt};
        if (int rc = dmalloc(&ioff, slots + 1, nullptr)) return rc;
        DevGuard g_io{ioff};
        const unsigned rb = unsigned(n_recv / 256 + 1);
        hipLaunchKernelGGL(k_item_counts, dim3(rb), dim3(256), 0, s, n_recv, hbeg, cnt, cc, hub_phases, icnt);
        if (int rc = exclusive_scan_i64(icnt, ioff, slots + 1, s)) return rc;
        GMSX_HIP(hipMemcpy(&g->hitems, ioff + slots, sizeof(int64_t), hipMemcpyDeviceToHost));
        if (int rc = dmalloc(&g->hitem, g->hitems + 1, g)) return rc;
        if (n_recv > 0) hipLaunchKernelGGL(k_item_fill, dim3(rb), dim3(256), 0, s, n_recv, recv_v, opos, hbeg, ioff, g->htask, g->hoff, 0, cnt, cc, hub_phases, g->hitem);
        hipLaunchKernelGGL(k_item_counts, dim3(rb), dim3(256), 0, s, n_recv, tbeg, cnt, cc, 1, icnt);
        if (int rc = exclusive_scan_i64(icnt, ioff, n_recv + 1, s)) return rc;
        GMSX_HIP(hipMemcpy(&g->titems, ioff + n_recv, sizeof(int64_t), hipMemcpyDeviceToHost));
        if (int rc = dmalloc(&g->titem, g->titems + 1, g)) return rc;
        if (n_recv > 0) hipLaunchKernelGGL(k_item_fill, dim3(rb), dim3(256), 0, s, n_recv, recv_v, opos, tbeg, ioff, g->ttask, g->toff, 1, cnt, cc, 1, g->titem);
        if (g->hitems >= (int64_t(1) << 31) || g->titems >= (int64_t(1) << 31)) return GMSX_ERR_DEVICE_MEM;
        GMSX_HIP(hipStreamSynchronize(s));
    }
    pt.mark("work items");
    GMSX_HIP(hipStreamSynchronize(s));
    GMSX_HIP(hipGetLastError());
    {
        auto drop = [&](auto *&p, size_t bytes) {
            if (!p) return;
            (void)hipFree(p);
            p = nullptr;
            g->device_bytes -= int64_t(bytes);
        };
        const size_t nn = size_t(n > 0 ? n : 1);
        drop(g->tsplit, nn * sizeof(int32_t));
        drop(g->srow2, nn * sizeof(unsigned long long));
        const char *keep = opt("TC_KEEP_ROWS");
        if (!(keep && std::atoi(keep) != 0)) {
            drop(g->srow, nn * sizeof(unsigned long long));
            drop(g->trow, nn * sizeof(unsigned long long));
        }
        drop(g->ksplit, size_t(n + 1) * sizeof(int32_t));
    }
    return GMSX_OK;
}

static int build_tc_once(gmsx_graph *g) {
    g->tc_base_bytes = g->device_bytes;
    g->tc_building = true;
    const int rc = build_tc_sets(g);
    g->tc_building = false;
    g->tc_bytes = g->device_bytes - g->tc_base_bytes;
    if (rc) {
        free_tc(g);
        return rc;
    }
    g->tc_ready = true;
    return GMSX_OK;
}

int ensure_tc(const gmsx_graph *cg) {
    gmsx_graph *g = const_cast<gmsx_graph *>(cg);
    if (g->tc_ready) return GMSX_OK;
    if (const char *e = opt("TC_MEM_LIMIT_MB")) {
        const long long v = std::atoll(e);
        g->tc_limit_bytes = v > 0 ? int64_t(v) << 20 : 0;
    }
    int rc = build_tc_once(g);
    if (rc == GMSX_ERR_DEVICE_MEM && g->shard_nparts == 1) {
        (void)hipGetLastError();
        for (int k = 2; k <= 4096 && rc == GMSX_ERR_DEVICE_MEM; k *= 2) {
            g->shard_part = 0;
            g->shard_nparts = k;
            rc = build_tc_once(g);
            if (rc == GMSX_OK) g->tc_passes = k;
        }
        if (rc) {
            g->shard_part = 0;
            g->shard_nparts = 1;
        }
    }
    return rc;
}

__global__ void k_shard_flags(int64_t n_items, const gmsx_tc_item *__restrict__ items, int nparts, int part, int64_t *__restrict__ flags) {
    const int64_t i = int64_t(blockIdx.x) * blockDim.x + threadIdx.x;
    if (i <= n_items) flags[i] = (i < n_items && shard_of(items[i].pos, nparts) == part) ? 1 : 0;
}
__global__ void k_shard_scatter(int64_t n_items, const int64_t *__restrict__ flags, const int64_t *__restrict__ slot, const gmsx_tc_item *__restrict__ items,
                                gmsx_tc_item *__restrict__ out) {
    const int64_t i = int64_t(blockIdx.x) * blockDim.x + threadIdx.x;
    if (i < n_items && flags[i]) out[slot[i]] = items[i];
}
int tc_shard_items(const gmsx_graph *g, int part, int nparts) {
    if (g->shard_idx_part == part && g->shard_idx_nparts == nparts) return GMSX_OK;
    hipStream_t s = ctx().stream;
    (void)hipFree(g->shard_hitem);
    (void)hipFree(g->shard_titem);
    g->shard_hitem = g->shard_titem = nullptr;
    g->shard_idx_part = g->shard_idx_nparts = -1;
    auto one = [&](const gmsx_tc_item *items, int64_t n_items, gmsx_tc_item **idx, int64_t *count) -> int {
        *count = 0;
        if (n_items == 0) return GMSX_OK;
        int64_t *flags = nullptr, *slot = nullptr;
        if (int rc = dmalloc(&flags, n_items + 1, nullptr)) return rc;
        DevGuard g_f{flags};
        if (int rc = dmalloc(&slot, n_items + 1, nullptr)) return rc;
        DevGuard g_s{slot};
        hipLaunchKernelGGL(k_shard_flags, dim3(unsigned(n_items / 256 + 1)), dim3(256), 0, s, n_items, items, nparts, part, flags);
        if (int rc = exclusive_scan_i64(flags, slot, n_items + 1, s)) return rc;
        GMSX_HIP(hipMemcpy(count, slot + n_items, sizeof(int64_t), hipMemcpyDeviceToHost));
        if (int rc = dmalloc(idx, *count + 1, nullptr)) return rc;
        hipLaunchKernelGGL(k_shard_scatter, dim3(unsigned(n_items / 256 + 1)), dim3(256), 0, s, n_items, flags, slot, items, *idx);
        GMSX_HIP(hipStreamSynchronize(s));
        return GMSX_OK;
    };
    if (int rc = one(g->hitem, g->hitems, &g->shard_hitem, &g->shard_hitems)) return rc;
    if (int rc = one(g->titem, g->titems, &g->shard_titem, &g->shard_titems)) return rc;
    g->shard_idx_part = part;
    g->shard_idx_nparts = nparts;
    return GMSX_OK;
}

int ensure_tc_shard(const gmsx_graph *cg, int part, int nparts) {
    gmsx_graph *g = const_cast<gmsx_graph *>(cg);
    if (g->tc_ready && g->shard_part == part && g->shard_nparts == nparts) return GMSX_OK;
    free_tc(g);
    g->shard_part = part;
    g->shard_nparts = nparts;
    return build_tc_once(g);
}

int count_dplus_ge(const gmsx_graph *g, int32_t threshold, int64_t *out) {
    if (g->n == 0) {
        *out = 0;
        return GMSX_OK;
    }
    for (int i = 0; i < g->ge_used; ++i)
        if (g->ge_thr[i] == threshold) {
            *out = g->ge_cnt[i];
            return GMSX_OK;
        }
    hipStream_t s = ctx().stream;
    hipLaunchKernelGGL(k_count_ge, dim3(1), dim3(1), 0, s, g->n, g->order, g->dplus, threshold, reinterpret_cast<int64_t *>(g->scratch + 8));
    GMSX_HIP(hipMemcpyAsync(out, g->scratch + 8, sizeof(int64_t), hipMemcpyDeviceToHost, s));
    GMSX_HIP(hipStreamSynchronize(s));
    if (g->ge_used < 40) {
        g->ge_thr[g->ge_used] = threshold;
        g->ge_cnt[g->ge_used] = *out;
        ++g->ge_used;
    }
    return GMSX_OK;
}

}

using namespace gmsx;

extern "C" {

int gmsx_init(int device) {
    return gmsx::guard([&]() -> int {
        Ctx &c = ctx();
        int count = 0;
        if (hipGetDeviceCount(&count) != hipSuccess || count <= 0) {
            (void)hipGetLastError();
            return GMSX_ERR_NO_DEVICE;
        }
        if (device < 0) {
            if (hipGetDevice(&device) != hipSuccess) return GMSX_ERR_NO_DEVICE;
        }
        if (device >= count) return GMSX_ERR_INVALID;
        if (c.device >= 0 && c.device != device) return GMSX_ERR_UNSUPPORTED;
        if (hipSetDevice(device) != hipSuccess) return GMSX_ERR_NO_DEVICE;
        if (c.device == device) return GMSX_OK;
        if (!c.own_stream) {
            if (hipStreamCreateWithFlags(&c.own_stream, hipStreamNonBlocking) != hipSuccess) return GMSX_ERR_NO_DEVICE;
            for (auto &e : c.ev)
                if (hipEventCreate(&e) != hipSuccess) return GMSX_ERR_NO_DEVICE;
            for (auto &st : c.side)
                if (hipStreamCreateWithFlags(&st, hipStreamNonBlocking) != hipSuccess) return GMSX_ERR_NO_DEVICE;
            if (hipEventCreateWithFlags(&c.ev_fork, hipEventDisableTiming) != hipSuccess) return GMSX_ERR_NO_DEVICE;
            for (auto &e : c.ev_join)
                if (hipEventCreateWithFlags(&e, hipEventDisableTiming) != hipSuccess) return GMSX_ERR_NO_DEVICE;
        }
        hipDeviceProp_t prop;
        if (hipGetDeviceProperties(&prop, device) != hipSuccess) return GMSX_ERR_NO_DEVICE;
        c.compute_units = prop.multiProcessorCount;
        c.stream = c.own_stream;
        c.device = device;
        if (const char *e = opt("INIT_LAZY"); !(e && std::atoi(e) != 0)) {
            hipLaunchKernelGGL(gmsx::k_warm, dim3(1), dim3(64), 0, c.stream, static_cast<unsigned long long *>(nullptr));
            if (!gmsx::h2d_staged_off()) (void)gmsx::h2d_stage();
            if (hipStreamSynchronize(c.stream) != hipSuccess) return GMSX_ERR_NO_DEVICE;
        }
        return GMSX_OK;
    });
}

int gmsx_set_stream(void *hip_stream) {
    return gmsx::guard([&]() -> int {
        if (int rc = ensure_init()) return rc;
        ctx().stream = hip_stream ? static_cast<hipStream_t>(hip_stream) : ctx().own_stream;
        return GMSX_OK;
    });
}

int gmsx_device_info(char *name, size_t name_len, int *compute_units, int64_t *hbm_bytes) {
    return gmsx::guard([&]() -> int {
        if (int rc = ensure_init()) return rc;
        hipDeviceProp_t prop;
// ... 110 lines not shown
```

### gms_amd/csrc/hip/device_graph.hpp

```cpp
#pragma once
#include <hip/hip_runtime.h>

#include <cstdint>

#include "gmsx.h"
#include "gmsx_internal.hpp"

#if !defined(GMSX_DEV_HOOKS) &&                                                                                                               \
    (defined(GMSX_KC_NO_PROBE) || defined(GMSX_KC_NO_HITS) || defined(GMSX_KC_NO_TAIL) || defined(GMSX_KC_NO_INNER) || defined(GMSX_KC_CELLS_ONLY) ||   \
     defined(GMSX_KC_NO_ROWS) || defined(GMSX_KC_BUILD_ONLY) || defined(GMSX_KC_NO_SLAB_CALL) || defined(GMSX_KC_NO_PAIRS) || defined(GMSX_KC_SLAB_ROW_SCAN) || \
     defined(GMSX_BK_AB) || defined(GMSX_BK_NO_HIT_ATOMICS) || defined(GMSX_BK_STATS) || defined(GMSX_TC_NO_PROBE) || defined(GMSX_TC_STAGING_ONLY))
#error "A/B switches need -DGMSX_DEV_HOOKS (tools/ab_lib.sh sets it); the default build of libgmsx.so carries none of them"
#endif

struct __attribute__((aligned(64))) gmsx_tc_item {
    uint64_t bc;
    uint64_t cont;
    int32_t pivot;
    int32_t pos;
    uint32_t kind;
    uint16_t fbeg[4];
    uint32_t reserved[7];
};
static_assert(sizeof(gmsx_tc_item) == 64, "work item record = one 64-byte line");
constexpr uint32_t kTaskHubUnitsMax = (1u << 14) - 1, kTaskTailUnitsMax = (1u << 15) - 1;
struct TaskList {
    uint32_t *lo = nullptr;
    uint16_t *hi = nullptr;
    bool tail = false;
    __host__ __device__ TaskList at(int64_t first) const { return TaskList{lo + first, hi + first, tail}; }
    __device__ __forceinline__ unsigned long long get(int64_t i) const {
        const uint32_t l = lo[i], h = hi[i];
        const unsigned long long first = ((unsigned long long)h << 16) | (l >> 16);
        const uint32_t form = tail ? ((l >> 15) & 1u) << 1 : (l >> 14) & 3u, units = tail ? l & kTaskTailUnitsMax : l & kTaskHubUnitsMax;
        return (first << 24) | ((unsigned long long)form << 22) | units;
    }
    __device__ __forceinline__ void put(int64_t i, unsigned long long d) const {
        const uint32_t first = uint32_t(d >> 24), form = (uint32_t(d) >> 22) & 3u, units = uint32_t(d) & 0x3fffffu;
        lo[i] = (first << 16) | (tail ? (form >> 1) << 15 : form << 14) | units;
        hi[i] = uint16_t(first >> 16);
    }
};
struct gmsx_graph {
    int64_t n = 0, nnz = 0, m = 0;
    int64_t *off = nullptr;
    int32_t *adj = nullptr;
    int32_t *newid = nullptr;
    int32_t *oldid = nullptr;
    int64_t *hoff = nullptr;
    uint16_t *hadj = nullptr;
    int64_t *toff = nullptr;
    int32_t *tadj = nullptr;
    int64_t *bmoff = nullptr;
    uint32_t *bmpool = nullptr;
    int32_t dense_limit = 0;
    int32_t bitset_limit = 0;
    unsigned long long *srow = nullptr;
    unsigned long long *srow2 = nullptr;
    int32_t *ksplit = nullptr;
    uint32_t *spool = nullptr;
    int64_t spool_units = 0;
    TaskList htask{nullptr, nullptr, false};
    TaskList ttask{nullptr, nullptr, true};
    int64_t htask_entries = 0, ttask_entries = 0;
    struct gmsx_tc_item *hitem = nullptr, *titem = nullptr;
    int64_t hitems = 0, titems = 0;
    int64_t inline_hentries = 0, inline_tentries = 0;
    mutable struct gmsx_tc_item *shard_hitem = nullptr, *shard_titem = nullptr;
    mutable int64_t shard_hitems = 0, shard_titems = 0;
    mutable int shard_idx_part = -1, shard_idx_nparts = -1;
    int32_t *tunits = nullptr;
    int64_t task_reverse = 0;
    uint4 *ledge = nullptr;
    int64_t n_ledge = 0, ledge_total = 0;
    uint4 *lpack = nullptr;
    int64_t lpack_base[8] = {0, 0, 0, 0, 0, 0, 0, 0};
    int64_t lpack_n[8] = {0, 0, 0, 0, 0, 0, 0, 0};
    int64_t lpack_total[8] = {0, 0, 0, 0, 0, 0, 0, 0};
    bool light_packed = false;
    uint32_t *core_bits = nullptr;
    int32_t tc_core = 0;
    mutable int core_bytes_k = -1, core_bytes_part = -1, core_bytes_nparts = -1;
    mutable uint64_t core_bytes = 0;
    int tc_hot_windows = 0;
    uint32_t tc_window_units = 1;
    int tc_hot_min = 0;
    int inline_first = 64;
    int32_t inline_limit = 0;
    int64_t inline_units = 0;
    unsigned long long *trow = nullptr;
    uint32_t *tpool = nullptr;
    int64_t tpool_units = 0;
    int32_t *tsplit = nullptr;
    int64_t dense_rows = 0, bmpool_words = 0;
    bool rows_sorted = false;
    int32_t *dplus = nullptr;
    int32_t *order = nullptr;
    int64_t hub_entries = 0, tail_entries = 0;
    int32_t max_dplus = 0;
    int32_t max_deg = 0;
    mutable bool kc_rev_tried = false;
    mutable uint32_t *kc_rel = nullptr;
    mutable int64_t *kc_aoff = nullptr;
    mutable uint32_t *kc_arena = nullptr;
    mutable ulonglong2 *kc_rec = nullptr;
    mutable uint4 *kc_item = nullptr;
    mutable uint32_t *kc_relt = nullptr;
    mutable ulonglong2 *kc_rect = nullptr;
    mutable uint4 *kc_itemt = nullptr;
    mutable int64_t kc_recst = 0, kc_itemst = 0;
    mutable int64_t kc_recs = 0, kc_items = 0, kc_arena_words = 0, kc_rev_bytes = 0;
    mutable double kc_rev_build_ms = 0.0;
    unsigned long long *scratch = nullptr;
    unsigned long long *acc = nullptr;
    mutable int32_t ge_thr[40] = {0};
    mutable int64_t ge_cnt[40] = {0};
    mutable int ge_used = 0;
    mutable int stats_part = -1, stats_nparts = -1;
    mutable uint64_t stats_units = 0, stats_probes = 0, stats_bytes = 0;
    int shard_part = 0, shard_nparts = 1;
    int tc_passes = 1;
    int64_t tc_limit_bytes = 0, tc_base_bytes = 0;
    bool tc_building = false;
    bool tc_ready = false;
    int64_t tc_bytes = 0;
    int hub_limit = 0;
    uint32_t upload_flags = 0;
    uint64_t alg_elements = 0;
    int64_t device_bytes = 0;
};

namespace gmsx {

static constexpr int kHub = 65535;
static constexpr int kBitmapWords = 2048;
static constexpr int kAccWords = 64 * 16 + 16;
static constexpr int kFormList = 0, kFormBitset = 1, kFormDelta = 2, kFormGap12 = 3;
static constexpr int kPoolSlack = 64;
static constexpr int kTaskChunk = 512;
static constexpr int kLenClasses = 12;
static constexpr int kHubClasses = 4 * kLenClasses, kTailClasses = 2 * kLenClasses;
static constexpr int kMaxHotWindows = 8;
struct TcClasses {
    int hot_windows;
    uint32_t window_units;
    int hot_min;
    __host__ __device__ int hub_phases() const { return hot_windows + 1; }
    __host__ __device__ int tail_base() const { return hub_phases() * kHubClasses; }
    __host__ __device__ int count() const { return tail_base() + kTailClasses; }
    __host__ __device__ int phase(unsigned long long d) const {
        if (hot_windows <= 0) return 0;
        const unsigned long long w = (d >> 24) / window_units;
        return w < (unsigned long long)hot_windows ? int(w) : hot_windows;
    }
};
__host__ __device__ inline int length_class(uint32_t u) {
    return u <= 16 ? (u <= 4 ? 0 : u <= 8 ? 1 : u <= 12 ? 2 : 3) : u <= 64 ? (u <= 24 ? 4 : u <= 32 ? 5 : u <= 48 ? 6 : 7) : (u <= 96 ? 8 : u <= 128 ? 9 : u <= 192 ? 10 : 11);
}
__host__ __device__ inline int hub_class(const TcClasses &cc, unsigned long long d) {
    return cc.phase(d) * kHubClasses + int((uint32_t(d) >> 22) & 3u) * kLenClasses + length_class(uint32_t(d) & 0x3fffffu);
}
__host__ __device__ inline int tail_class(const TcClasses &cc, unsigned long long d) {
    return cc.tail_base() + (((uint32_t(d) >> 22) & 3u) == 2u ? kLenClasses : 0) + length_class(uint32_t(d) & 0x3fffffu);
}
__host__ __device__ inline void hub_phase_range(const TcClasses &cc, const uint32_t *c, int64_t len, int ph, int64_t *b, int64_t *e) {
    int64_t start = 0;
    for (int q = 0;; ++q) {
        const int64_t end = q < cc.hot_windows ? int64_t(c[(q + 1) * kHubClasses]) : len;
        const bool own = q == cc.hot_windows || end - start >= cc.hot_min;
        if (q == ph) {
            *b = start;
            *e = own ? end : start;
            return;
        }
        if (own) start = end;
    }
}
__host__ __device__ inline int shard_of(int64_t pos, int nparts) {
    const int j = int(pos % nparts);
    return ((pos / nparts) & 1) ? nparts - 1 - j : j;
}
static constexpr int kHeavy = 64;
static constexpr int kDeltaIds = 14;

struct LightShape {
    int ah, at, bh, bt;
    __host__ __device__ constexpr int stride() const { return ah + at + bh + bt; }
};
static constexpr int kLightClasses = 6;
static_assert(kLightClasses <= 8, "gmsx_graph::lpack_base");
__host__ __device__ constexpr LightShape light_shape(int c) {
    return c == 0 ? LightShape{2, 3, 2, 4} : c == 1 ? LightShape{1, 2, 5, 8} : c == 2 ? LightShape{2, 4, 5, 9} : c == 3 ? LightShape{3, 8, 4, 9}
         : c == 4 ? LightShape{6, 8, 6, 10} : LightShape{8, 16, 8, 16};
}
static_assert(kHeavy <= 8 * light_shape(kLightClasses - 1).ah && kHeavy <= 4 * light_shape(kLightClasses - 1).at &&
              kHeavy <= 8 * light_shape(kLightClasses - 1).bh && kHeavy <= 4 * light_shape(kLightClasses - 1).bt, "the last class must hold every light row");
static constexpr int kLightMaxUnits = light_shape(kLightClasses - 1).stride();
__host__ __device__ inline int light_class(int ah, int at, int bh, int bt) {
    for (int c = 0; c < kLightClasses - 1; ++c) {
        const LightShape k = light_shape(c);
        if (ah <= 8 * k.ah && at <= 4 * k.at && bh <= 8 * k.bh && bt <= 4 * k.bt) return c;
    }
    return kLightClasses - 1;
}
__device__ __forceinline__ int light_hub_ids(const int64_t *__restrict__ hoff, const uint16_t *__restrict__ hadj, int32_t v) {
    const int64_t b = hoff[v], e = hoff[v + 1];
    return int(e - b) - ((e > b && hadj[e - 1] == 0xFFFFu) ? 1 : 0);
}

__host__ __device__ inline int64_t bitset_words(int32_t v) { return ((int64_t(v) + 31) / 32 + 3) & ~int64_t(3); }

struct Ctx {
    int device = -1;
    hipStream_t stream = nullptr;
    hipStream_t own_stream = nullptr;
    hipEvent_t ev[4] = {nullptr, nullptr, nullptr, nullptr};
    hipStream_t side[2] = {nullptr, nullptr};
    hipEvent_t ev_fork = nullptr, ev_join[2] = {nullptr, nullptr};
    int compute_units = 0;
};
Ctx &ctx();
int ensure_init();
int kclique_vertex_counts(const gmsx_graph *g, unsigned long long *d_counts, gmsx_stats *st);
int count_dplus_ge(const gmsx_graph *g, int32_t threshold, int64_t *out);
int exclusive_scan_i64(const int64_t *in, int64_t *out, int64_t count, hipStream_t s);
int ensure_tc(const gmsx_graph *g);
int ensure_tc_shard(const gmsx_graph *g, int part, int nparts);
int tc_shard_items(const gmsx_graph *g, int part, int nparts);
int tc_vertex_counts_device(const gmsx_graph *g, unsigned long long *d_counts, gmsx_stats *st);
int tc_full_partial(const gmsx_graph *g, int part, int nparts, uint64_t *partial, gmsx_stats *st);

__device__ __forceinline__ int uni32(int x) { return __builtin_amdgcn_readfirstlane(x); }
__device__ __forceinline__ uint32_t uni32(uint32_t x) { return uint32_t(__builtin_amdgcn_readfirstlane(int(x))); }
__device__ __forceinline__ int64_t uni64(int64_t x) {
    const uint32_t lo = uint32_t(__builtin_amdgcn_readfirstlane(int(uint32_t(uint64_t(x)))));
    const uint32_t hi = uint32_t(__builtin_amdgcn_readfirstlane(int(uint32_t(uint64_t(x) >> 32))));
    return int64_t((uint64_t(hi) << 32) | lo);
}
__device__ __forceinline__ unsigned long long uni64(unsigned long long x) { return (unsigned long long)uni64(int64_t(x)); }

#define GMSX_HIP(call)                                                    \
    do {                                                                  \
// ... 9 lines not shown
```

### gms_amd/csrc/hip/tc.hip

```cpp
#include "device_graph.hpp"
#include "kc4_mfma.hpp"
#include "../host/tc_core_plan.hpp"

#include <algorithm>
#include <type_traits>
#include <rocprim/device/device_radix_sort.hpp>
#include <rocprim/device/device_reduce.hpp>
#include <rocprim/device/device_reduce_by_key.hpp>
#include <cstdio>
#include <cstdlib>
#include <cstring>

namespace gmsx {

static constexpr int kAccSlots = 64;
static constexpr int kAccStride = 16;

struct __attribute__((packed, aligned(4))) u4u { uint32_t x, y, z, w; };

__device__ __forceinline__ int64_t readlane64(int64_t x, int l) {
    const uint32_t lo = __builtin_amdgcn_readlane(uint32_t(uint64_t(x)), l);
    const uint32_t hi = __builtin_amdgcn_readlane(uint32_t(uint64_t(x) >> 32), l);
    return int64_t((uint64_t(hi) << 32) | lo);
}
// ... 678 lines not shown
    if (trips > 0) {
        Units cur = load(0);
        for (int64_t t = 0; t < trips; ++t) {
#pragma unroll
            for (int s = 0; s < STEPS; ++s) mine[16 * s + sub] = cur.u[s];
            wave_lds_fence();
            cur = load(t + 1);
            uint32_t c = 0;
#pragma unroll
            for (int r = 0; r < RAH; ++r) {
                const uint32_t a = ah[sub + 16 * r];
                c += (lds_has<BH>(bh, a) && a != 0xFFFFu && (16 * (r + 1) <= AH || sub + 16 * r < AH)) ? 1u : 0u;
            }
#pragma unroll
            for (int r = 0; r < RAT; ++r) {
                const uint32_t a = (16 * (r + 1) <= AT || sub + 16 * r < AT) ? at[sub + 16 * r] : 0xFFFFFFFFu;
                c += lds_has<BT>(bt, a) ? 1u : 0u;
            }
            wave_lds_fence();
            total += g0 + t * ngroups < count ? c : 0u;
        }
    }
    block_add(total, red, lane, wave, tid, acc);
}

__global__ __launch_bounds__(1024) void k_tc_core(const uint32_t *__restrict__ bits, int WS, int K, int nb, int nblk, int part, int nparts,
                                                  unsigned long long *__restrict__ acc) {
    __shared__ unsigned long long red[16];
    auto lane_id = [] { return int(__builtin_amdgcn_mbcnt_hi(~0u, __builtin_amdgcn_mbcnt_lo(~0u, 0u))); };
    const int wave = uni32(int(threadIdx.x) >> 6);
    const int x = blockIdx.x & 7, y = blockIdx.x >> 3, Y = int(gridDim.x) >> 3;
    const int Q = 16 * Y, q = y * 16 + wave;
    const int ns = (nblk - part + nparts - 1) / nparts;
    uint32_t cnt = 0;
    for (int j = 0;; ++j) {
        const int sidx = (8 * j + ((j & 1) ? 7 - x : x)) * Q + q;
        if (sidx >= ns) break;
        const int t = sidx * nparts + part;
        int c = int((__builtin_sqrtf(8.0f * float(t) + 1.0f) - 1.0f) * 0.5f);
        while (c * (c + 1) / 2 > t) --c;
        while ((c + 1) * (c + 2) / 2 <= t) ++c;
        const int bj = nb - 1 - c, bi = bj + (t - c * (c + 1) / 2);
        int lane = lane_id();
        asm volatile("" : "+v"(lane));
        cnt += Kc4mBlock<2>::run(bits, WS, K, bi, bj, lane);
    }
    const int lane = lane_id();
    unsigned long long total = cnt;
    for (int sft = 32; sft > 0; sft >>= 1) total += __shfl_down(total, sft);
    if (lane == 0) red[wave] = total;
    __syncthreads();
    if (wave == 0 && lane == 0) {
        unsigned long long t = 0;
        for (int w = 0; w < 16; ++w) t += red[w];
        if (t) atomicAdd(&acc[(blockIdx.x & (kAccSlots - 1)) * kAccStride], t);
    }
}

__global__ __launch_bounds__(256) void k_tc_stats(const int64_t *__restrict__ hoff, const uint16_t *__restrict__ hadj,
                                                  const int64_t *__restrict__ toff, const int32_t *__restrict__ tadj,
                                                  const int32_t *__restrict__ dplus, const int32_t *__restrict__ order,
                                                  const int32_t *__restrict__ tunits, int32_t inline_limit, int inline_first, int32_t core, int packed, int64_t end, int nparts, int part,
                                                  unsigned long long *__restrict__ out) {
    const int lane = threadIdx.x & 63;
    const int64_t wave0 = (int64_t(blockIdx.x) * blockDim.x + threadIdx.x) >> 6;
    const int64_t nwaves = (int64_t(gridDim.x) * blockDim.x) >> 6;
    unsigned long long units = 0, probes = 0, bytes = 0;
    for (int64_t pos = wave0; pos < end; pos += nwaves) {
        if (nparts > 1 && shard_of(pos, nparts) != part) continue;
        const int32_t u = order[pos];
        const int du = dplus[u];
        if (du >= kHeavy) {
            if (lane == 0) units += (unsigned long long)tunits[pos];
            if (u < core) {
                if (lane == 0) units += (unsigned long long)du;
                continue;
            }
            const int hl = min(int(hoff[u + 1] - hoff[u]), inline_first), tl = min(int(toff[u + 1] - toff[u]), inline_first - hl);
            int32_t v = -1;
            if (lane < hl) {
                const uint32_t x = hadj[hoff[u] + lane];
                if (x != 0xFFFFu) v = int32_t(x);
            } else if (lane - hl < tl) v = tadj[toff[u] + lane - hl];
            if (v >= 0 && lane > 0 && (v < inline_limit || dplus[v] >= kHeavy)) ++units;
            continue;
        }
        const int hl = int(hoff[u + 1] - hoff[u]);
        if (lane == 0) units += (unsigned long long)du;
        if (du < 2 || u < core) continue;
        const int ah = packed ? light_hub_ids(hoff, hadj, u) : 0;
        for (int64_t j = toff[u] + lane; j < toff[u + 1]; j += 64) {
            const int32_t v = tadj[j];
            if (v < inline_limit || dplus[v] >= kHeavy) continue;
            const unsigned long long hv = (unsigned long long)(hoff[v + 1] - hoff[v]), tv = (unsigned long long)(toff[v + 1] - toff[v]);
            if (packed) bytes += 16ull * (unsigned long long)light_shape(light_class(ah, int(j - toff[u]), light_hub_ids(hoff, hadj, v), int(tv))).stride();
            else bytes += 32ull + 2ull * hl + 4ull * (unsigned long long)(j - toff[u]) + 2ull * hv + 4ull * tv;
            probes += hv + tv;
        }
    }
    for (int s = 32; s > 0; s >>= 1) {
        units += __shfl_down(units, s);
        probes += __shfl_down(probes, s);
        bytes += __shfl_down(bytes, s);
    }
    if (lane == 0) {
        if (units) atomicAdd(&out[0], units);
        if (probes) atomicAdd(&out[1], probes);
        if (bytes) atomicAdd(&out[2], bytes);
    }
}
__global__ __launch_bounds__(256) void k_tc_item_stats(const int64_t *__restrict__ coff, int bytes_per_id, int tail, const TaskList task,
                                                       const gmsx_tc_item *__restrict__ items, int64_t n_items, int nparts, int part,
                                                       unsigned long long *__restrict__ out) {
    const int lane = threadIdx.x & 63;
    const int64_t wave0 = (int64_t(blockIdx.x) * blockDim.x + threadIdx.x) >> 6;
    const int64_t nwaves = (int64_t(gridDim.x) * blockDim.x) >> 6;
    unsigned long long probes = 0, bytes = 0;
    auto slots = [tail](unsigned long long d) -> unsigned long long {
        const unsigned long long n = d & 0x3fffffull, f = (d >> 22) & 3ull;
        return n * (tail ? (f == kFormDelta ? 6ull : 4ull) : (f == kFormList ? 8ull : f == kFormDelta ? 14ull : f == kFormGap12 ? 10ull : 4ull));
    };
    for (int64_t q = wave0; q < n_items; q += nwaves) {
        const gmsx_tc_item &it = items[q];
        if (nparts > 1 && shard_of(it.pos, nparts) != part) continue;
        const int ne = int(it.bc >> 40);
        const int64_t b = int64_t(it.bc & 0xffffffffffull);
        if (lane == 0) bytes += (unsigned long long)bytes_per_id * (unsigned long long)(coff[it.pivot + 1] - coff[it.pivot]);
        for (int i = lane; i < ne; i += 64) {
            const unsigned long long d = task.get(b + i);
            bytes += 6ull + 16ull * (d & 0x3fffffull);
            probes += slots(d);
        }
    }
    for (int s = 32; s > 0; s >>= 1) {
        probes += __shfl_down(probes, s);
        bytes += __shfl_down(bytes, s);
    }
    if (lane == 0) {
        if (probes) atomicAdd(&out[1], probes);
        if (bytes) atomicAdd(&out[2], bytes);
    }
}

__global__ __launch_bounds__(256) void k_tc_breakdown(const int64_t *__restrict__ hoff, const uint16_t *__restrict__ hadj, const int64_t *__restrict__ toff, const int32_t *__restrict__ tadj,
                                                      const int32_t *__restrict__ dplus, const int32_t *__restrict__ order,
                                                      const TaskList htask, const gmsx_tc_item *__restrict__ hitem, int64_t hitems,
                                                      const TaskList ttask, const gmsx_tc_item *__restrict__ titem, int64_t titems,
                                                      int32_t inline_limit, int32_t core, int packed, int64_t first_light, int64_t end_light,
                                                      unsigned long long *__restrict__ out) {
    const int lane = threadIdx.x & 63;
    const int64_t wave0 = (int64_t(blockIdx.x) * blockDim.x + threadIdx.x) >> 6;
    const int64_t nwaves = (int64_t(gridDim.x) * blockDim.x) >> 6;
    unsigned long long c[15] = {0, 0, 0, 0, 0, 0, 0, 0, 0, 0, 0, 0, 0, 0, 0};
    for (int64_t q = wave0; q < hitems + titems; q += nwaves) {
        const bool tail = q >= hitems;
        const gmsx_tc_item &it = tail ? titem[q - hitems] : hitem[q];
        const TaskList task = tail ? ttask : htask;
        const int ne = int(it.bc >> 40);
        const int64_t b0 = int64_t(it.bc & 0xffffffffffull);
        if (lane == 0) {
            c[6] += tail ? 4ull * (unsigned long long)(toff[it.pivot + 1] - toff[it.pivot]) : 2ull * (unsigned long long)(hoff[it.pivot + 1] - hoff[it.pivot]);
            c[11] += (unsigned long long)ne;
            c[13] += 1;
        }
        for (int i = lane; i < ne; i += 64) {
            const unsigned long long d = task.get(b0 + i);
            const unsigned long long db = 16ull * (d & 0x3fffffull);
            const int fd = int((d >> 22) & 3);
            if (tail) c[fd == kFormDelta ? 4 : 3] += db;
            else c[fd == kFormList ? 0 : fd == kFormBitset ? 1 : 2] += db;
            c[5] += 6;
        }
    }
    for (int64_t pos = first_light + wave0; pos < end_light; pos += nwaves) {
        const int32_t u = order[pos];
        if (u < core) continue;
        const int64_t tb0 = toff[u], te = toff[u + 1];
        const unsigned long long hl = (unsigned long long)(hoff[u + 1] - hoff[u]);
        const int ah = packed ? light_hub_ids(hoff, hadj, u) : 0;
        for (int64_t j = tb0 + lane; j < te; j += 64) {
            const int32_t v = tadj[j];
            if (v < inline_limit || dplus[v] >= kHeavy) continue;
            c[14] += 1;
            if (packed) {
                const LightShape k = light_shape(light_class(ah, int(j - tb0), light_hub_ids(hoff, hadj, v), int(toff[v + 1] - toff[v])));
                c[8] += 16ull * (unsigned long long)(k.ah + k.bh);
                c[9] += 16ull * (unsigned long long)(k.at + k.bt);
                continue;
            }
            c[8] += 2ull * (unsigned long long)(hoff[v + 1] - hoff[v]);
            c[9] += 4ull * (unsigned long long)(toff[v + 1] - toff[v]);
            c[10] += 32ull + 2ull * hl + 4ull * (unsigned long long)(j - tb0);
        }
    }
    for (int k = 0; k < 15; ++k) {
        unsigned long long x = c[k];
        for (int s = 32; s > 0; s >>= 1) x += __shfl_down(x, s);
        if (lane == 0 && x) atomicAdd(&out[k], x);
    }
}

__device__ __forceinline__ int hist_bin(unsigned long long units) {
    if (units <= 16) return int(units) - 1;
    int b = 16;
    for (unsigned long long lim = 32; units > lim && b < 23; lim <<= 1) ++b;
    return b;
}
__global__ __launch_bounds__(256) void k_tc_comember_keys(const TaskList htask, const gmsx_tc_item *__restrict__ hitem, int64_t hitems, int batch,
                                                         unsigned long long *__restrict__ keys, uint32_t *__restrict__ vals, unsigned long long *__restrict__ sums) {
    unsigned long long ents = 0, units = 0;
    for (int64_t i = blockIdx.x; i < hitems; i += gridDim.x) {
        const gmsx_tc_item it = hitem[i];
        const unsigned long long first = it.bc & 0xffffffffffull;
        const int n = int(it.bc >> 40);
        const unsigned long long b = (unsigned long long)(it.pos / batch) << 40;
        for (int e = threadIdx.x; e < n; e += 256) {
            const unsigned long long d = htask.get(int64_t(first + e));
            keys[first + e] = b | (d >> 24);
            vals[first + e] = uint32_t(d & 0x3fffffull);
            ++ents;
            units += d & 0x3fffffull;
        }
    }
    for (int sft = 32; sft > 0; sft >>= 1) {
        ents += __shfl_xor(ents, sft);
        units += __shfl_xor(units, sft);
    }
    if ((threadIdx.x & 63) == 0) {
        atomicAdd(&sums[0], ents);
        atomicAdd(&sums[1], units);
    }
}
__global__ __launch_bounds__(256) void k_tc_sum_u32(const uint32_t *__restrict__ v, unsigned long long n, unsigned long long *__restrict__ out) {
    unsigned long long t = 0;
    for (unsigned long long i = (unsigned long long)blockIdx.x * 256 + threadIdx.x; i < n; i += (unsigned long long)gridDim.x * 256) t += v[i];
    for (int sft = 32; sft > 0; sft >>= 1) t += __shfl_xor(t, sft);
    if ((threadIdx.x & 63) == 0) atomicAdd(out, t);
}
__global__ __launch_bounds__(256) void k_tc_row_hist(const int64_t *__restrict__ hoff, const uint16_t *__restrict__ hadj,
                                                     const int64_t *__restrict__ toff, const int32_t *__restrict__ tadj,
                                                     const int32_t *__restrict__ dplus, const int32_t *__restrict__ order,
                                                     const unsigned long long *__restrict__ srow, const unsigned long long *__restrict__ trow,
                                                     const TaskList htask, const gmsx_tc_item *__restrict__ hitem, int64_t hitems,
                                                     const TaskList ttask, const gmsx_tc_item *__restrict__ titem, int64_t titems,
                                                     int64_t end, unsigned long long *__restrict__ out) {
    __shared__ unsigned long long h[256];
    for (int i = threadIdx.x; i < 256; i += 256) h[i] = 0;
    __syncthreads();
    const int lane = threadIdx.x & 63;
    const int64_t wave0 = (int64_t(blockIdx.x) * blockDim.x + threadIdx.x) >> 6;
    const int64_t nwaves = (int64_t(gridDim.x) * blockDim.x) >> 6;
    auto add = [&](int cls, unsigned long long units) {
        if (units == 0) return;
        const int b = (cls * 24 + hist_bin(units)) * 2;
        atomicAdd(&h[b], 1ull);
        atomicAdd(&h[b + 1], units);
    };
    for (int64_t q = wave0; q < hitems + titems; q += nwaves) {
        const bool tail = q >= hitems;
        const gmsx_tc_item &it = tail ? titem[q - hitems] : hitem[q];
        const TaskList task = tail ? ttask : htask;
        const int ne = int(it.bc >> 40);
        const int64_t b0 = int64_t(it.bc & 0xffffffffffull);
        if (lane == 0) {
            atomicAdd(&h[240], (unsigned long long)ne);
            atomicAdd(&h[242], 1ull);
            atomicAdd(&h[243], tail ? 4ull * (unsigned long long)(toff[it.pivot + 1] - toff[it.pivot]) : 2ull * (unsigned long long)(hoff[it.pivot + 1] - hoff[it.pivot]));
        }
        for (int i = lane; i < ne; i += 64) {
            const unsigned long long d = task.get(b0 + i);
            if (tail) add(((d >> 22) & 3) == kFormDelta ? 4 : 3, d & 0x3fffffull);
            else add(min(int((d >> 22) & 3), 2), d & 0x3fffffull);
        }
    }
    for (int64_t pos = wave0; pos < end; pos += nwaves) {
        if (!srow || !trow) break;
        const int32_t u = order[pos];
        const int du = dplus[u];
        if (du < 2) continue;
        const int64_t hb = hoff[u], tb = toff[u];
        const int hl = int(hoff[u + 1] - hb), tl = int(toff[u + 1] - tb);
        const unsigned long long su = (srow[u] & 0x3fffffull) + (trow[u] & 0x3fffffull);
        unsigned long long cur = 0, best = 0, cut = 0;
        for (int i = lane; i < hl + tl; i += 64) {
            int32_t v;
            if (i < hl) {
                const uint32_t x = hadj[hb + i];
                if (x == 0xFFFFu) continue;
                v = int32_t(x);
            } else v = tadj[tb + i - hl];
            const unsigned long long sv = (srow[v] & 0x3fffffull) + (trow[v] & 0x3fffffull);
            cur += sv;
            best += min(su, sv);
            cut += min(sv, dplus[v] >= kHeavy ? (su * (unsigned long long)i + du - 1) / (unsigned long long)du : ~0ull);
        }
        atomicAdd(&h[du >= kHeavy ? 248 : 250], cur);
        atomicAdd(&h[du >= kHeavy ? 249 : 251], best);
        if (du >= kHeavy) atomicAdd(&h[252], cut);
    }
    __syncthreads();
    for (int i = threadIdx.x; i < 256; i += 256)
        if (h[i]) atomicAdd(&out[i], h[i]);
}

static int tc_one(const gmsx_graph *g, int part, int nparts, int cpart, int cnparts, uint64_t *partial, gmsx_stats *st);
static uint64_t core_bytes_of(const gmsx_graph *g, int part, int nparts) {
    if (g->tc_core <= 0 || nparts < 1) return 0;
    if (!(g->core_bytes_k == g->tc_core && g->core_bytes_part == part && g->core_bytes_nparts == nparts)) {
        g->core_bytes = tc_core_bytes(g->tc_core, part, nparts);
        g->core_bytes_k = g->tc_core;
        g->core_bytes_part = part;
        g->core_bytes_nparts = nparts;
    }
    return g->core_bytes;
}

static int tc_oriented(const gmsx_graph *g, int part, int nparts, uint64_t *partial, gmsx_stats *st) {
    if (int rc = ensure_tc(g)) return rc;
    if (g->tc_passes == 1) return tc_one(g, part, nparts, part, nparts, partial, st);
    if (nparts > 1) {
        auto restore = [&](int rc) {
            gmsx_graph *m = const_cast<gmsx_graph *>(g);
            if (m->tc_ready && m->shard_part == 0 && m->shard_nparts == m->tc_passes) return rc;
            (void)ensure_tc_shard(g, 0, g->tc_passes);
            return rc;
        };
        int J = nparts >= g->tc_passes ? 1 : (g->tc_passes + nparts - 1) / nparts;
        if (J > 1 && (J & 1)) ++J;
        for (;; J *= 2) {
            uint64_t total = 0;
            gmsx_stats sum{};
            int rc = GMSX_OK;
            for (int a = 0; a < J && rc == GMSX_OK; ++a) {
                const int sub = a * nparts + ((a & 1) ? nparts - 1 - part : part);
                rc = ensure_tc_shard(g, sub, nparts * J);
                if (rc) break;
                uint64_t pp = 0;
                gmsx_stats sp{};
                rc = tc_one(g, sub, nparts * J, part, a == 0 ? nparts : 0, &pp, st ? &sp : nullptr);
                total += pp;
                sum.kernel_ms += sp.kernel_ms;
                sum.setup_ms += sp.setup_ms;
                sum.units += sp.units;
                sum.probes += sp.probes;
                sum.stream_bytes += sp.stream_bytes;
                sum.launches += sp.launches;
            }
            if (rc == GMSX_ERR_DEVICE_MEM && nparts * J <= (1 << 20)) continue;
            if (rc) return restore(rc);
            *partial = total;
            if (st) *st = sum;
            return GMSX_OK;
// ... 72 lines not shown
            for (int i = 0; i < 2; ++i)
                if (armed[i] && hipEventRecord(c.ev_join[i], c.side[i]) == hipSuccess) (void)hipStreamWaitEvent(s, c.ev_join[i], 0);
        }
    } join{c, s};
    const bool side_light = sides && cnt_light > 0 && n_hitems + n_titems > 0;
    const bool side_tail = sides && !persist && n_hitems > 0 && n_titems > 0;
    if (side_light || side_tail) GMSX_HIP(hipEventRecord(c.ev_fork, s));
    if (side_tail) {
        GMSX_HIP(hipStreamWaitEvent(c.side[0], c.ev_fork, 0));
        join.armed[0] = true;
    }
    if (side_light) {
        GMSX_HIP(hipStreamWaitEvent(c.side[1], c.ev_fork, 0));
        join.armed[1] = true;
    }
    const bool run_core = g->tc_core > 0 && cnparts > 0 && !only;
    if (run_core) {
        const int K = g->tc_core, nb = (K + 63) / 64, nblk = int(tc_core_blocks(K));
        const int64_t ns = (int64_t(nblk) - cpart + cnparts - 1) / cnparts;
        if (ns > 0) {
            const int64_t wgs = std::max<int64_t>(8, std::min<int64_t>(cus / 8 * 8, ((ns + 15) / 16 + 7) / 8 * 8));
            hipLaunchKernelGGL(k_tc_core, dim3(unsigned(wgs)), dim3(1024), 0, s, g->core_bits, kc4m_stride(K), K, nb, nblk, cpart, cnparts, acc);
            ++launches;
        }
    }
    if (persist) {
        const int wgs_env = [] { const char *e = opt("TC_ITEM_WGS"); return e ? std::atoi(e) : 0; }();
        auto grid = [&](int64_t n, int wgs) {
            return unsigned(std::max<int64_t>(1, std::min<int64_t>((n + kGrab - 1) / kGrab, int64_t(cus) * (wgs_env > 0 ? wgs_env : wgs))));
        };
        if (n_hitems > 0) {
            hipLaunchKernelGGL(k_tc_items<false>, dim3(grid(n_hitems, GMSX_TC_HUB_MIN_WAVES)), dim3(256), 0, s, g->hadj, g->tadj, g->spool, g->htask, hitem, int(n_hitems), qhead, acc);
            ++launches;
        }
        if (n_titems > 0) {
            hipLaunchKernelGGL(k_tc_items<true>, dim3(grid(n_titems, GMSX_TC_TAIL_MIN_WAVES)), dim3(256), 0, s, g->hadj, g->tadj, g->tpool, g->ttask, titem, int(n_titems),
                               qhead + kQueueStride, acc);
            ++launches;
        }
    } else {
        if (n_hitems > 0) {
            hipLaunchKernelGGL(k_tc_block, dim3(unsigned(n_hitems)), dim3(256), 0, s, g->hoff, g->hadj, g->spool, g->htask, hitem, acc);
            ++launches;
        }
        if (n_titems > 0) {
            hipLaunchKernelGGL(k_tc_tail, dim3(unsigned(n_titems)), dim3(256), 0, side_tail ? c.side[0] : s, g->toff, g->tadj, g->tpool, g->ttask, titem, acc);
            ++launches;
        }
    }
    if (g->light_packed) {
        auto launch = [&](auto kernel, int k) {
            if (cnt_class[k] <= 0) return;
            const int64_t blocks = std::min<int64_t>((cnt_class[k] + 15) / 16, int64_t(cus) * 8);
            hipLaunchKernelGGL(kernel, dim3(unsigned(blocks)), dim3(256), 0, side_light ? c.side[1] : s, g->lpack + g->lpack_base[k], strided ? nparts : 1, strided ? part : 0,
                               cnt_class[k], acc);
            ++launches;
        };
        static_assert(kLightClasses == 6, "one instance per class");
        launch(k_tc_lpack<0>, 0);
        launch(k_tc_lpack<1>, 1);
        launch(k_tc_lpack<2>, 2);
        launch(k_tc_lpack<3>, 3);
        launch(k_tc_lpack<4>, 4);
        launch(k_tc_lpack<5>, 5);
    } else if (cnt_light > 0) {
        const int64_t blocks = std::min<int64_t>((cnt_light + 15) / 16, int64_t(cus) * 8);
        hipLaunchKernelGGL(k_tc_light, dim3(unsigned(blocks)), dim3(256), 0, side_light ? c.side[1] : s, g->hadj, g->tadj, g->ledge, strided ? nparts : 1,
                           strided ? part : 0, cnt_light, acc);
        ++launches;
    }
    for (int i = 0; i < 2; ++i)
        if (join.armed[i]) {
            join.armed[i] = false;
            GMSX_HIP(hipEventRecord(c.ev_join[i], c.side[i]));
            GMSX_HIP(hipStreamWaitEvent(s, c.ev_join[i], 0));
        }
    GMSX_HIP(hipEventRecord(c.ev[2], s));
    GMSX_HIP(hipGetLastError());

    const bool need_stats = st && !(g->stats_part == part && g->stats_nparts == nparts);
    if (need_stats) {
        if (g->n > 0) {
            const int64_t blocks = std::min<int64_t>((g->n + 3) / 4, cap_blocks);
            hipLaunchKernelGGL(k_tc_stats, dim3(unsigned(blocks)), dim3(256), 0, s, g->hoff, g->hadj, g->toff, g->tadj, g->dplus, g->order,
                               g->tunits, g->inline_limit, g->inline_first, g->tc_core, g->light_packed ? 1 : 0, g->n, nparts, part, acc + kAccSlots * kAccStride);
        }
        if (g->hitems > 0)
            hipLaunchKernelGGL(k_tc_item_stats, dim3(unsigned(std::min<int64_t>((g->hitems + 3) / 4, cap_blocks))), dim3(256), 0, s, g->hoff, 2, 0, g->htask, g->hitem,
                               g->hitems, nparts, part, acc + kAccSlots * kAccStride);
        if (g->titems > 0)
            hipLaunchKernelGGL(k_tc_item_stats, dim3(unsigned(std::min<int64_t>((g->titems + 3) / 4, cap_blocks))), dim3(256), 0, s, g->toff, 4, 1, g->ttask, g->titem,
                               g->titems, nparts, part, acc + kAccSlots * kAccStride);
    }
    unsigned long long host[kAccSlots * kAccStride + 3];
    GMSX_HIP(hipMemcpyAsync(host, acc, sizeof(host), hipMemcpyDeviceToHost, s));
    GMSX_HIP(hipStreamSynchronize(s));
    unsigned long long total = 0;
    for (int i = 0; i < kAccSlots; ++i) total += host[i * kAccStride];
    *partial = total;
    if (st) {
        float ms_setup = 0.f, ms_kernel = 0.f;
        GMSX_HIP(hipEventElapsedTime(&ms_setup, c.ev[0], c.ev[1]));
        GMSX_HIP(hipEventElapsedTime(&ms_kernel, c.ev[1], c.ev[2]));
        st->kernel_ms = ms_kernel;
        st->setup_ms = ms_setup;
        if (need_stats) {
            g->stats_part = part;
            g->stats_nparts = nparts;
            g->stats_units = host[kAccSlots * kAccStride];
            g->stats_probes = host[kAccSlots * kAccStride + 1];
            g->stats_bytes = host[kAccSlots * kAccStride + 2];
        }
        st->units = g->stats_units;
        st->probes = g->stats_probes;
        st->alg_elements = nparts == 1 ? g->alg_elements : 0;
        st->launches = launches;
        st->reserved = 0;
        st->stream_bytes = g->stats_bytes + (run_core ? core_bytes_of(g, cpart, cnparts) : 0);
    }
    return GMSX_OK;
}

}

using namespace gmsx;

extern "C" {

int gmsx_tc_divisor(int algo) { return algo == GMSX_TC_FULL ? 3 : 1; }

int gmsx_tc_stream_breakdown(const gmsx_graph *g, uint64_t *out21) {
    return gmsx::guard([&]() -> int {
        if (!g || !out21) return GMSX_ERR_INVALID;
        if (int rc = ensure_init()) return rc;
        if (int rc = ensure_tc(g)) return rc;
        hipStream_t s = ctx().stream;
        std::memset(out21, 0, 21 * sizeof(uint64_t));
        if (g->n == 0) return GMSX_OK;
        int64_t n_block = 0, n_work = 0;
        if (int rc = count_dplus_ge(g, kHeavy, &n_block)) return rc;
        if (int rc = count_dplus_ge(g, 2, &n_work)) return rc;
        unsigned long long *acc = nullptr;
        GMSX_HIP(hipMalloc(reinterpret_cast<void **>(&acc), 21 * 8));
        struct Guard { void *p; ~Guard() { (void)hipFree(p); } } g1{acc};
        GMSX_HIP(hipMemsetAsync(acc, 0, 21 * 8, s));
        const int cus = ctx().compute_units > 0 ? ctx().compute_units : 256;
        hipLaunchKernelGGL(k_tc_breakdown, dim3(unsigned(cus * 16)), dim3(256), 0, s, g->hoff, g->hadj, g->toff, g->tadj, g->dplus, g->order, g->htask,
                           g->hitem, g->hitems, g->ttask, g->titem, g->titems, g->inline_limit, g->tc_core, g->light_packed ? 1 : 0, n_block, n_work, acc);
        GMSX_HIP(hipMemcpyAsync(out21, acc, 21 * 8, hipMemcpyDeviceToHost, s));
        GMSX_HIP(hipStreamSynchronize(s));
        GMSX_HIP(hipGetLastError());
        out21[7] = uint64_t(g->inline_units) * 16ull;
        out21[12] = uint64_t(g->inline_hentries + g->inline_tentries);
        out21[15] = core_bytes_of(g, 0, 1);
        out21[16] = uint64_t(g->tc_core);
        return GMSX_OK;
    });
}

int gmsx_tc_row_histogram(const gmsx_graph *g, uint64_t *out256) {
    return gmsx::guard([&]() -> int {
        uint64_t *out248 = out256;
        if (!g || !out248) return GMSX_ERR_INVALID;
        if (int rc = ensure_init()) return rc;
        if (int rc = ensure_tc(g)) return rc;
        hipStream_t s = ctx().stream;
        std::memset(out248, 0, 256 * sizeof(uint64_t));
        if (g->n == 0) return GMSX_OK;
        unsigned long long *acc = nullptr;
        GMSX_HIP(hipMalloc(reinterpret_cast<void **>(&acc), 256 * 8));
        struct Guard { void *p; ~Guard() { (void)hipFree(p); } } g1{acc};
        GMSX_HIP(hipMemsetAsync(acc, 0, 256 * 8, s));
        const int cus = ctx().compute_units > 0 ? ctx().compute_units : 256;
        hipLaunchKernelGGL(k_tc_row_hist, dim3(unsigned(cus * 8)), dim3(256), 0, s, g->hoff, g->hadj, g->toff, g->tadj, g->dplus, g->order, g->srow, g->trow,
                           g->htask, g->hitem, g->hitems, g->ttask, g->titem, g->titems, g->n, acc);
        GMSX_HIP(hipGetLastError());
        GMSX_HIP(hipMemcpyAsync(out248, acc, 256 * 8, hipMemcpyDeviceToHost, s));
        GMSX_HIP(hipStreamSynchronize(s));
        GMSX_HIP(hipGetLastError());
        out248[241] = uint64_t(g->inline_hentries + g->inline_tentries);
        return GMSX_OK;
    });
}

int gmsx_tc_comembership(const gmsx_graph *g, int batch, uint64_t *out8) {
    return gmsx::guard([&]() -> int {
        if (!g || !out8 || batch < 1) return GMSX_ERR_INVALID;
        if (int rc = ensure_init()) return rc;
        if (int rc = ensure_tc(g)) return rc;
        hipStream_t s = ctx().stream;
        std::memset(out8, 0, 8 * sizeof(uint64_t));
        const int64_t ne = g->htask_entries;
        if (g->n == 0 || ne == 0 || g->hitems == 0) return GMSX_OK;
        struct Guard { void *p = nullptr; ~Guard() { (void)hipFree(p); } } gk0, gk1, gv0, gv1, gu, ga, gc, gt, gsum;
        unsigned long long *k0 = nullptr, *k1 = nullptr, *uk = nullptr, *cnt = nullptr, *sum = nullptr;
        uint32_t *v0 = nullptr, *v1 = nullptr, *agg = nullptr;
        GMSX_HIP(hipMalloc(reinterpret_cast<void **>(&k0), size_t(ne) * 8)); gk0.p = k0;
        GMSX_HIP(hipMalloc(reinterpret_cast<void **>(&k1), size_t(ne) * 8)); gk1.p = k1;
        GMSX_HIP(hipMalloc(reinterpret_cast<void **>(&v0), size_t(ne) * 4)); gv0.p = v0;
        GMSX_HIP(hipMalloc(reinterpret_cast<void **>(&v1), size_t(ne) * 4)); gv1.p = v1;
        GMSX_HIP(hipMalloc(reinterpret_cast<void **>(&sum), 4 * 8)); gsum.p = sum;
        GMSX_HIP(hipMemsetAsync(k0, 0xff, size_t(ne) * 8, s));
        GMSX_HIP(hipMemsetAsync(v0, 0, size_t(ne) * 4, s));
        GMSX_HIP(hipMemsetAsync(sum, 0, 4 * 8, s));
        hipLaunchKernelGGL(k_tc_comember_keys, dim3(unsigned(std::min<int64_t>(g->hitems, 1 << 20))), dim3(256), 0, s, g->htask, g->hitem, g->hitems, batch, k0, v0, sum);
        size_t tb = 0;
        GMSX_HIP(rocprim::radix_sort_pairs(nullptr, tb, k0, k1, v0, v1, size_t(ne), 0, 64, s));
        void *tmp = nullptr;
        GMSX_HIP(hipMalloc(&tmp, tb ? tb : 8)); gt.p = tmp;
        GMSX_HIP(rocprim::radix_sort_pairs(tmp, tb, k0, k1, v0, v1, size_t(ne), 0, 64, s));
        uk = k0;
        agg = v0;
        GMSX_HIP(hipMalloc(reinterpret_cast<void **>(&cnt), 8)); gc.p = cnt;
        size_t rb = 0;
        GMSX_HIP(rocprim::reduce_by_key(nullptr, rb, k1, v1, size_t(ne), uk, agg, cnt, rocprim::maximum<uint32_t>(), rocprim::equal_to<unsigned long long>(), s));
        void *tmp2 = nullptr;
        Guard g2;
        GMSX_HIP(hipMalloc(&tmp2, rb ? rb : 8)); g2.p = tmp2;
        GMSX_HIP(rocprim::reduce_by_key(tmp2, rb, k1, v1, size_t(ne), uk, agg, cnt, rocprim::maximum<uint32_t>(), rocprim::equal_to<unsigned long long>(), s));
        unsigned long long nuniq = 0;
        GMSX_HIP(hipMemcpyAsync(&nuniq, cnt, 8, hipMemcpyDeviceToHost, s));
        GMSX_HIP(hipStreamSynchronize(s));
        hipLaunchKernelGGL(k_tc_sum_u32, dim3(1024), dim3(256), 0, s, agg, (unsigned long long)nuniq, sum + 2);
        unsigned long long h[4] = {0, 0, 0, 0};
        GMSX_HIP(hipMemcpyAsync(h, sum, sizeof(h), hipMemcpyDeviceToHost, s));
        GMSX_HIP(hipStreamSynchronize(s));
        GMSX_HIP(hipGetLastError());
        out8[0] = uint64_t(h[0]);
        out8[1] = uint64_t(h[1]);
        out8[2] = uint64_t(nuniq);
        out8[3] = uint64_t(h[2]);
        out8[4] = uint64_t(g->hitems);
        return GMSX_OK;
    });
}

int gmsx_tc_partial(const gmsx_graph *g, int algo, int part, int nparts, uint64_t *partial, gmsx_stats *stats) {
    return gmsx::guard([&]() -> int {
        if (!g || !partial || nparts < 1 || part < 0 || part >= nparts) return GMSX_ERR_INVALID;
        if (algo != GMSX_TC_AUTO && algo != GMSX_TC_ORIENTED && algo != GMSX_TC_FULL) return GMSX_ERR_INVALID;
        if (int rc = ensure_init()) return rc;
        if (algo == GMSX_TC_FULL) return tc_full_partial(g, part, nparts, partial, stats);
        if (g->tc_passes == 1 && g->shard_nparts > 1 && (nparts != g->shard_nparts || part != g->shard_part)) return GMSX_ERR_INVALID;
        return tc_oriented(g, part, nparts, partial, stats);
    });
}

int gmsx_tc_total(const gmsx_graph *g, int algo, uint64_t *triangles, gmsx_stats *stats) {
    return gmsx::guard([&]() -> int {
        if (!triangles) return GMSX_ERR_INVALID;
        uint64_t partial = 0;
        if (int rc = gmsx_tc_partial(g, algo, 0, 1, &partial, stats)) return rc;
        const uint64_t div = uint64_t(gmsx_tc_divisor(algo));
        if (partial % div != 0) return GMSX_ERR_KERNEL;
        *triangles = partial / div;
        return GMSX_OK;
    });
}

}
```

### gms_amd/csrc/host/loader.cpp

```cpp
#include "gmsx_internal.hpp"

#include <fcntl.h>
#include <sys/mman.h>
#include <sys/stat.h>
#include <unistd.h>

#include <algorithm>
#ifdef _OPENMP
#include <parallel/algorithm>
#endif
#include <atomic>
#include <cerrno>
#include <cmath>
#include <cstdio>
#include <cstdlib>
#include <cstring>
#include <ctime>
#include <fstream>
#include <limits>
#include <memory>
#include <new>
#include <random>
#include <sstream>
#include <string>
// ... 501 lines not shown
        ++u;
    }
    return finish_el(us, vs, el);
}
static int read_mtx(const std::string &path, EdgeList &el) {
    std::ifstream in(path);
    if (!in.is_open()) return GMSX_ERR_IO;
    std::string start, object, format, field, symmetry, line;
    if (!(in >> start >> object >> format >> field >> symmetry)) return GMSX_ERR_FORMAT;
    if (start != "%%MatrixMarket" || object != "matrix" || format != "coordinate" || field == "complex") return GMSX_ERR_FORMAT;
    const bool weights = field == "real" || field == "double" || field == "integer";
    if (!weights && field != "pattern") return GMSX_ERR_FORMAT;
    if (symmetry != "symmetric" && symmetry != "general" && symmetry != "skew-symmetric") return GMSX_ERR_FORMAT;
    std::getline(in, line);
    long long rows = -1, cols = -1, nz = -1;
    while (std::getline(in, line)) {
        if (!line.empty() && line[0] == '%') continue;
        std::istringstream hs(line);
        if (!(hs >> rows >> cols >> nz)) return GMSX_ERR_FORMAT;
        break;
    }
    if (rows < 0 || rows != cols) return GMSX_ERR_FORMAT;
    std::vector<int32_t> us, vs;
    while (std::getline(in, line)) {
        std::istringstream ls(line);
        long long a, b;
        if (!(ls >> a >> b)) continue;
        if (int rc = push_edge(us, vs, a - 1, b - 1)) return rc;
        if (symmetry == "symmetric")
            if (int rc = push_edge(us, vs, b - 1, a - 1)) return rc;
    }
    return finish_el(us, vs, el);
}

static int validate_csr_arrays(const int64_t *off, const int32_t *ng, int64_t n, int64_t nnz);
static int read_sg(const std::string &path, Csr &g) {
    std::FILE *f = std::fopen(path.c_str(), "rb");
    if (!f) return GMSX_ERR_IO;
    struct Closer { std::FILE *f; ~Closer() { std::fclose(f); } } closer{f};
    unsigned char directed = 0;
    int64_t nnz = 0, n = 0;
    if (std::fread(&directed, 1, 1, f) != 1 || std::fread(&nnz, 8, 1, f) != 1 || std::fread(&n, 8, 1, f) != 1)
        return GMSX_ERR_FORMAT;
    if (n < 0 || nnz < 0 || n > std::numeric_limits<int32_t>::max()) return GMSX_ERR_FORMAT;
    if (int rc = alloc_csr(g, n, nnz)) return rc;
    if (std::fread(g.off.get(), 8, size_t(n + 1), f) != size_t(n + 1)) return GMSX_ERR_FORMAT;
    if (nnz && std::fread(g.neigh.get(), 4, size_t(nnz), f) != size_t(nnz)) return GMSX_ERR_FORMAT;
    if (int rc = validate_csr_arrays(g.off.get(), g.neigh.get(), n, nnz)) return rc;
    g.directed = directed != 0;
    return GMSX_OK;
}


static constexpr char kSgxMagic[8] = {'G', 'M', 'S', 'X', 'C', 'S', 'R', '1'};
static constexpr int64_t kSgxAlign = 64;
static int64_t sgx_neigh_offset(int64_t n) { return (kSgxAlign + (n + 1) * 8 + kSgxAlign - 1) / kSgxAlign * kSgxAlign; }

void ArrayFree::unmap(void *base, size_t bytes) { (void)munmap(base, bytes); }

static int write_sgx(const Csr &g, const char *path) {
    std::FILE *f = std::fopen(path, "wb");
    if (!f) return GMSX_ERR_IO;
    int64_t head[8] = {0, g.directed ? 1 : 0, g.n, g.nnz, 0, 0, 0, 0};
    std::memcpy(head, kSgxMagic, 8);
    const int64_t pad = sgx_neigh_offset(g.n) - (kSgxAlign + (g.n + 1) * 8);
    const char zeros[64] = {0};
    bool ok = std::fwrite(head, 8, 8, f) == 8 && std::fwrite(g.off.get(), 8, size_t(g.n + 1), f) == size_t(g.n + 1) &&
              (pad == 0 || std::fwrite(zeros, 1, size_t(pad), f) == size_t(pad)) &&
              (g.nnz == 0 || std::fwrite(g.neigh.get(), 4, size_t(g.nnz), f) == size_t(g.nnz));
    ok = (std::fclose(f) == 0) && ok;
    return ok ? GMSX_OK : GMSX_ERR_IO;
}

static int validate_csr_arrays(const int64_t *off, const int32_t *ng, int64_t n, int64_t nnz) {
    if (off[0] != 0 || off[n] != nnz) return GMSX_ERR_FORMAT;
    int bad = 0;
#pragma omp parallel for reduction(| : bad) schedule(static)
    for (int64_t u = 0; u < n; ++u) bad |= int(off[u + 1] < off[u]);
    if (bad) return GMSX_ERR_FORMAT;
#pragma omp parallel for reduction(| : bad) schedule(static)
    for (int64_t j = 0; j < nnz; ++j) bad |= int(ng[j] < 0 || int64_t(ng[j]) >= n);
    return bad ? GMSX_ERR_FORMAT : GMSX_OK;
}

static int read_sgx(const std::string &path, Csr &g) {
    const int fd = open(path.c_str(), O_RDONLY | O_CLOEXEC);
    if (fd < 0) return GMSX_ERR_IO;
    struct Closer { int fd; ~Closer() { close(fd); } } closer{fd};
    struct stat st;
    if (fstat(fd, &st) != 0) return GMSX_ERR_IO;
    int64_t head[8];
    if (pread(fd, head, sizeof(head), 0) != ssize_t(sizeof(head)) || std::memcmp(head, kSgxMagic, 8) != 0) return GMSX_ERR_FORMAT;
    const int64_t n = head[2], nnz = head[3];
    if (n < 0 || nnz < 0 || n > std::numeric_limits<int32_t>::max() || (head[1] != 0 && head[1] != 1)) return GMSX_ERR_FORMAT;
    const int64_t noff = sgx_neigh_offset(n);
    if (nnz > (std::numeric_limits<int64_t>::max() - noff) / 4 || int64_t(st.st_size) < noff + nnz * 4) return GMSX_ERR_FORMAT;
    const int64_t page = int64_t(sysconf(_SC_PAGESIZE));
    auto map_part = [&](int64_t at, int64_t bytes, void **base, size_t *len) -> void * {
        const int64_t lo = at / page * page;
        *len = size_t(at - lo + std::max<int64_t>(bytes, 1));
        *base = mmap(nullptr, *len, PROT_READ | PROT_WRITE, MAP_PRIVATE, fd, off_t(lo));
        if (*base == MAP_FAILED) return nullptr;
        (void)madvise(*base, *len, MADV_WILLNEED);
        return static_cast<char *>(*base) + (at - lo);
    };
    void *b0 = nullptr, *b1 = nullptr;
    size_t l0 = 0, l1 = 0;
    void *p_off = map_part(kSgxAlign, (n + 1) * 8, &b0, &l0);
    if (!p_off) return GMSX_ERR_NOMEM;
    g.off = std::unique_ptr<int64_t[], ArrayFree>(static_cast<int64_t *>(p_off), ArrayFree{b0, l0});
    void *p_ng = map_part(noff, nnz * 4, &b1, &l1);
    if (!p_ng) return GMSX_ERR_NOMEM;
    g.neigh = std::unique_ptr<int32_t[], ArrayFree>(static_cast<int32_t *>(p_ng), ArrayFree{b1, l1});
    g.n = n;
    g.nnz = nnz;
    g.directed = head[1] != 0;
    g.mapped = true;
    return validate_csr_arrays(g.off.get(), g.neigh.get(), n, nnz);
}

}

namespace gmsx {
int host_threads() {
#ifdef _OPENMP
    return omp_get_max_threads();
#else
    return 1;
#endif
}
void parallel_memcpy(void *dst, const void *src, size_t bytes) {
#ifdef _OPENMP
#pragma omp parallel
    {
        const size_t nt = size_t(omp_get_num_threads()), t = size_t(omp_get_thread_num());
        const size_t per = ((bytes + nt - 1) / nt + 4095) & ~size_t(4095), lo = std::min(bytes, per * t), hi = std::min(bytes, lo + per);
        if (hi > lo) std::memcpy(static_cast<char *>(dst) + lo, static_cast<const char *>(src) + lo, hi - lo);
    }
#else
    std::memcpy(dst, src, bytes);
#endif
}
namespace {
struct Option {
    const char *name;
    char value[32];
    bool set;
};
Option g_options[] = {
    {"TIMING", "", false}, {"MEM_TRACE", "", false}, {"BK_VERBOSE", "", false},
    {"INLINE_LIMIT", "", false}, {"TC_INLINE_FIRST", "", false}, {"TC_DELTA", "", false}, {"TC_DELTA_PCT", "", false}, {"TC_GAP12", "", false},
    {"TC_HYBRID", "", false}, {"TC_TAIL_DELTA", "", false}, {"TC_TWO_SIDED", "", false}, {"TC_HOT_WINDOWS", "", false}, {"TC_HOT_KB", "", false},
    {"TC_HOT_MIN", "", false}, {"TC_TEST_MAX_UNITS", "", false}, {"TC_KEEP_ROWS", "", false}, {"TC_MEM_LIMIT_MB", "", false}, {"TC_OVERLAP", "", false},
    {"TC_PERSIST", "", false}, {"TC_ITEM_WGS", "", false}, {"TC_CORE", "", false}, {"TC_LIGHT_PACKED", "", false}, {"SORT_CHUNK", "", false}, {"UPLOAD_STAGED", "", false}, {"INIT_LAZY", "", false},
    {"KC_SLAB_MB", "", false}, {"KC_MAXD", "", false}, {"KC_STREAMS", "", false},
    {"KC_REVERSE", "", false}, {"KC_REV_MIN", "", false}, {"KC_REV_FACTOR", "", false}, {"KC_REV_TAIL", "", false}, {"KC_REV_TAIL_MIN", "", false}, {"KC_TRI", "", false}, {"KC_MFMA", "", false}, {"KC_POOL_MB", "", false},
    {"BK_MAXC", "", false}, {"BK_ARENA_MB", "", false}, {"BK_GROUPS", "", false}, {"BK_SMALL_P", "", false}, {"BK_SMALL_P_GROUPS", "", false},
    {"BK_BUDGET", "", false}, {"BK_BUDGET0", "", false}, {"BK_RESUME_GRAB", "", false}, {"BK_SPLIT_BUILD", "", false}, {"BK_TINY_ROOTS", "", false},
    {"BK_TINY_BESIDE", "", false},
    {"BK_LIST_ARENA_MB", "", false},
    {"KCSTAR_SLAB_MB", "", false},
    {"CORE_WG_FRONTIER", "", false},
    {"COLOR_WG_FRONTIER", "", false},
    {"TRUSS_WG_FRONTIER", "", false},
    {"LP_LDS_MAXN", "", false}, {"LP_SLAB_MB", "", false},
    {"SGM_LAUNCH_TASKS", "", false},
    {"CC_SAMPLE", "", false}, {"CC_WAVE_ROW", "", false}, {"CC_WG_ROW", "", false},
    {"C4_LDS_SPAN", "", false}, {"C4_SLAB_MB", "", false}, {"C4_SPLIT_WEDGES", "", false},
};
Option *find_option(const char *name) {
    if (!name) return nullptr;
    for (Option &o : g_options)
        if (std::strcmp(o.name, name) == 0) return &o;
    return nullptr;
}
}

const char *opt(const char *name) {
    const Option *o = find_option(name);
    return o && o->set ? o->value : nullptr;
}

}

using namespace gmsx;

extern "C" {

int gmsx_csr_generate(int generator, int scale, int degree, int relabel, int threads, gmsx_csr **out) {
    return gmsx::guard([&]() -> int {
        if (!out || scale < 1 || degree < 1 || relabel < 0 || relabel > 2) return GMSX_ERR_INVALID;
        if (scale > 30) return GMSX_ERR_OVERFLOW;
        if (generator != GMSX_GEN_KRONECKER && generator != GMSX_GEN_UNIFORM) return GMSX_ERR_INVALID;
    #ifdef _OPENMP
        struct Threads {
            int saved, set;
            ~Threads() { if (set > 0) omp_set_num_threads(saved); }
        } threads_guard{omp_get_max_threads(), threads};
        if (threads > 0) omp_set_num_threads(threads);
    #else
        (void)threads;
    #endif
        int rc;
        {
            Csr g;
            {
                PhaseTimer pt;
                EdgeList el;
                rc = generator == GMSX_GEN_UNIFORM ? make_uniform(scale, degree, el) : make_rmat(scale, degree, el);
                pt.lap("generate edge list");
                if (!rc) rc = build_from_el(el, -1, true, g);
            }
            PhaseTimer pf;
            if (!rc) rc = finish(std::move(g), relabel, out);
            pf.lap("relabel decision + relabel");
        }
        return rc;
    });
}

int gmsx_csr_generate_rmat(int scale, int degree, double a, double b, double c, int relabel, int threads, gmsx_csr **out) {
    return gmsx::guard([&]() -> int {
        if (!out || scale < 1 || degree < 1 || relabel < 0 || relabel > 2) return GMSX_ERR_INVALID;
        if (!(a > 0 && b >= 0 && c >= 0 && a + b + c < 1.0)) return GMSX_ERR_INVALID;
        if (scale > 30) return GMSX_ERR_OVERFLOW;
    #ifdef _OPENMP
        struct Threads {
            int saved, set;
            ~Threads() { if (set > 0) omp_set_num_threads(saved); }
        } threads_guard{omp_get_max_threads(), threads};
        if (threads > 0) omp_set_num_threads(threads);
    #else
        (void)threads;
    #endif
        int rc;
        {
            Csr g;
            {
                EdgeList el;
                rc = make_rmat(scale, degree, el, float(a), float(b), float(c));
                if (!rc) rc = build_from_el(el, -1, true, g);
            }
            if (!rc) rc = finish(std::move(g), relabel, out);
        }
        return rc;
    });
}

int gmsx_csr_from_edges(int64_t num_nodes, int64_t num_edges, const int32_t *src, const int32_t *dst,
                        int symmetrize, int relabel, gmsx_csr **out) {
    return gmsx::guard([&]() -> int {
        if (!out || num_edges < 0 || (num_edges && (!src || !dst)) || relabel < 0 || relabel > 2) return GMSX_ERR_INVALID;
        EdgeList el;
        if (int rc = el.alloc(num_edges)) return rc;
        if (num_edges) {
            std::memcpy(el.u.get(), src, size_t(num_edges) * 4);
            std::memcpy(el.v.get(), dst, size_t(num_edges) * 4);
        }
        Csr g;
        if (int rc = build_from_el(el, num_nodes, symmetrize != 0, g)) return rc;
        return finish(std::move(g), relabel, out);
    });
}

int gmsx_csr_load(const char *path, int symmetrize, int relabel, gmsx_csr **out) {
    return gmsx::guard([&]() -> int {
        if (!path || !out || relabel < 0 || relabel > 2) return GMSX_ERR_INVALID;
        const std::string p(path), suf = suffix_of(p);
        Csr g;
        if (suf == ".sg") {
            if (int rc = read_sg(p, g)) return rc;
        } else if (suf == ".sgx") {
            if (int rc = read_sgx(p, g)) return rc;
        } else if (suf == ".el" || suf == ".wel" || suf == ".gr" || suf == ".graph" || suf == ".mtx") {
            EdgeList el;
            const int rc = suf == ".el" ? read_el(p, el) : suf == ".wel" ? read_wel(p, el) : suf == ".gr" ? read_gr(p, el)
                         : suf == ".graph" ? read_metis(p, el) : read_mtx(p, el);
            if (rc) return rc;
            if (int rc2 = build_from_el(el, -1, symmetrize != 0, g)) return rc2;
        } else {
            return GMSX_ERR_FORMAT;
        }
        return finish(std::move(g), relabel, out);
    });
}

int gmsx_csr_save_sg(const gmsx_csr *h, const char *path) {
    return gmsx::guard([&]() -> int {
        if (!h || !path) return GMSX_ERR_INVALID;
        std::FILE *f = std::fopen(path, "wb");
        if (!f) return GMSX_ERR_IO;
        const Csr &g = h->g;
        const unsigned char directed = g.directed ? 1 : 0;
        bool ok = std::fwrite(&directed, 1, 1, f) == 1 && std::fwrite(&g.nnz, 8, 1, f) == 1 &&
                  std::fwrite(&g.n, 8, 1, f) == 1 && std::fwrite(g.off.get(), 8, size_t(g.n + 1), f) == size_t(g.n + 1) &&
                  (g.nnz == 0 || std::fwrite(g.neigh.get(), 4, size_t(g.nnz), f) == size_t(g.nnz));
        ok = (std::fclose(f) == 0) && ok;
        return ok ? GMSX_OK : GMSX_ERR_IO;
    });
}

int gmsx_csr_save_sgx(const gmsx_csr *h, const char *path) {
    return gmsx::guard([&]() -> int {
        if (!h || !path) return GMSX_ERR_INVALID;
        return write_sgx(h->g, path);
    });
}
// ... 115 lines not shown
```

Baseline: 16.64 billion.

## Gather partial cache-line row tails into per-receiver packed regions for TC

Adds a gather plan to the triangle-count task build: row segments whose end falls partway into a 128-byte line (up to R units) are copied into a per-receiver, line-aligned region and emitted as separate chunked task entries. The row descriptors shrink to cover only the remaining line-aligned part. Pool bases and inline regions are padded to line boundaries. The intent is to cut wasted HBM traffic from partially used cache lines during intersection. In exchange it adds extra preprocessing kernels, copies, and pool memory, and falls back to smaller R when device memory runs out. New stats counters are added to the stream breakdown.

```diff
diff --git a/gms_amd/capi.py b/gms_amd/capi.py
--- a/gms_amd/capi.py
+++ b/gms_amd/capi.py
@@ -524,7 +524,7 @@
     BREAKDOWN = ["hub_rows_list", "hub_rows_bitset", "hub_rows_delta", "tail_rows_list", "tail_rows_delta", "entries", "pivot_containers",
                  "of_which_inline_rows", "light_streamed_hub_rows", "light_streamed_tail_rows", "light_pivot_lists_and_descriptors",
                  "count_entries", "count_inline_entries", "count_work_items", "count_light_streamed_members",
-                 "core_matrix", "core_k", "reserved17", "reserved18", "reserved19", "reserved20"]
+                 "core_matrix", "core_k", "gathered_rows", "row_line_bytes", "partial_line_entries", "gather_limit"]
     BREAKDOWN_BYTES = ("hub_rows_list", "hub_rows_bitset", "hub_rows_delta", "tail_rows_list", "tail_rows_delta", "entries", "pivot_containers",
                        "light_streamed_hub_rows", "light_streamed_tail_rows", "light_pivot_lists_and_descriptors", "core_matrix")
 
diff --git a/gms_amd/csrc/hip/device_graph.hip b/gms_amd/csrc/hip/device_graph.hip
--- a/gms_amd/csrc/hip/device_graph.hip
+++ b/gms_amd/csrc/hip/device_graph.hip
@@ -18,6 +18,7 @@
 
 #include "../host/gmsx_internal.hpp"
 #include "../host/tc_core_plan.hpp"
+#include "../host/tc_gather_plan.hpp"
 #include "kc4_mfma.hpp"
 
 namespace gmsx {
@@ -536,12 +537,13 @@
         }
     }
 }
-__global__ void k_inline_units(int64_t n, const unsigned long long *__restrict__ ids_h, const unsigned long long *__restrict__ ids_t,
+__global__ void k_inline_units(int64_t n, const unsigned long long *__restrict__ ids_h, const unsigned long long *__restrict__ ids_t, bool lines,
                                int64_t *__restrict__ units_h, int64_t *__restrict__ units_t) {
     const int64_t v = int64_t(blockIdx.x) * blockDim.x + threadIdx.x;
     if (v > n) return;
-    units_h[v] = v < n ? int64_t((ids_h[v] + 7) / 8) : 0;
-    units_t[v] = v < n ? int64_t((ids_t[v] + 3) / 4) : 0;
+    const int64_t uh = v < n ? int64_t((ids_h[v] + 7) / 8) : 0, ut = v < n ? int64_t((ids_t[v] + 3) / 4) : 0;
+    units_h[v] = lines ? int64_t(gather_region_units(uint64_t(uh))) : uh;
+    units_t[v] = lines ? int64_t(gather_region_units(uint64_t(ut))) : ut;
 }
 static constexpr int kDefaultHotWindows = 0, kDefaultHotKB = 2048, kDefaultHotMin = 16;
 __device__ __forceinline__ int64_t receiver_of(int32_t w, const int32_t *__restrict__ dplus, const int32_t *__restrict__ opos, const int64_t *__restrict__ lidx,
@@ -564,13 +566,14 @@
 }
 template <bool FILL>
 __global__ void k_inline_entries(int64_t n, const int32_t *__restrict__ dplus, const int32_t *__restrict__ opos, const int64_t *__restrict__ lidx, int64_t n_heavy,
-                                 int32_t inline_limit, const int64_t *__restrict__ ihoff, const int64_t *__restrict__ itoff, int64_t base_h, int64_t base_t,
+                                 int32_t inline_limit, const int64_t *__restrict__ ihoff, const int64_t *__restrict__ itoff,
+                                 const unsigned long long *__restrict__ ids_h, const unsigned long long *__restrict__ ids_t, int64_t base_h, int64_t base_t,
                                  uint32_t *__restrict__ cnt, uint32_t *__restrict__ cur, const int64_t *__restrict__ hbeg, const int64_t *__restrict__ tbeg,
                                  TaskList htask, TaskList ttask, unsigned long long *__restrict__ totals, TcClasses cc) {
     const int kClasses = cc.count();
     const int64_t v = int64_t(blockIdx.x) * blockDim.x + threadIdx.x;
     if (v >= n) return;
-    const int64_t uh = ihoff[v + 1] - ihoff[v], ut = itoff[v + 1] - itoff[v];
+    const int64_t uh = int64_t((ids_h[v] + 7) / 8), ut = int64_t((ids_t[v] + 3) / 4);
     if (uh == 0 && ut == 0) return;
     if (dplus[v] < kHeavy && v >= inline_limit) return;
     const int64_t p = receiver_of(int32_t(v), dplus, opos, lidx, n_heavy);
@@ -764,6 +767,75 @@
     }
     return mine;
 }
+struct GatherPlan {
+    int R = 0;
+    uint32_t *gunits = nullptr;
+    uint32_t *gcur = nullptr;
+    const int64_t *hoff = nullptr;
+    const int64_t *toff = nullptr;
+    int64_t hreg = 0, treg = 0;
+    uint4 *spool = nullptr, *tpool = nullptr;
+};
+__device__ __forceinline__ uint32_t claim_units(uint32_t *ctr, uint32_t mine, int lane) {
+    if (__ballot(mine != 0) == 0ull) return 0u;
+    uint32_t incl = mine;
+#pragma unroll
+    for (int s = 1; s < 64; s <<= 1) {
+        const uint32_t x = uint32_t(__shfl_up(int(incl), s));
+        if (lane >= s) incl += x;
+    }
+    const uint32_t total = uint32_t(__builtin_amdgcn_readlane(int(incl), 63));
+    uint32_t base = 0;
+    if (lane == 0) base = atomicAdd(ctr, total);
+    base = uint32_t(__builtin_amdgcn_readfirstlane(int(base)));
+    return base + incl - mine;
+}
+__device__ __forceinline__ void gather_copy(const GatherPlan &gp, bool tail, int64_t p, unsigned long long d, uint32_t moved, uint32_t at) {
+    uint4 *pool = tail ? gp.tpool : gp.spool;
+    const int slot = gather_slot((uint32_t(d) >> 22) & 3u);
+    const int64_t dst = (tail ? gp.treg + gp.toff[2 * p + slot] : gp.hreg + gp.hoff[2 * p + slot]) + int64_t(at);
+    const int64_t src = int64_t(d >> 24) + int64_t(uint32_t(d) & 0x3fffffu) - int64_t(moved);
+    for (uint32_t k = 0; k < moved; ++k) pool[dst + k] = pool[src + k];
+}
+__global__ void k_gather_sizes(int64_t n_recv, const uint32_t *__restrict__ gunits, int64_t *__restrict__ hsize, int64_t *__restrict__ tsize,
+                               unsigned long long *__restrict__ moved) {
+    const int64_t i = int64_t(blockIdx.x) * blockDim.x + threadIdx.x;
+    if (i > 2 * n_recv) return;
+    const int64_t p = i >> 1, fs = i & 1;
+    const uint32_t gh = i < 2 * n_recv ? gunits[4 * p + fs] : 0u, gt = i < 2 * n_recv ? gunits[4 * p + 2 + fs] : 0u;
+    hsize[i] = int64_t(gather_region_units(gh));
+    tsize[i] = int64_t(gather_region_units(gt));
+    if (gh + gt) atomicAdd(moved, (unsigned long long)gh + gt);
+}
+template <bool FILL>
+__global__ void k_gather_entries(int64_t n_recv, const uint32_t *__restrict__ gunits, const int64_t *__restrict__ ghoff, const int64_t *__restrict__ gtoff,
+                                 int64_t hreg, int64_t treg, uint32_t *__restrict__ cnt, uint32_t *__restrict__ cur, const int64_t *__restrict__ hbeg,
+                                 const int64_t *__restrict__ tbeg, TaskList htask, TaskList ttask, uint4 *__restrict__ spool, uint4 *__restrict__ tpool,
+                                 TcClasses cc) {
+    const int kClasses = cc.count();
+    const int64_t p = int64_t(blockIdx.x) * blockDim.x + threadIdx.x;
+    if (p >= n_recv) return;
+    uint32_t *c = cnt + p * kClasses;
+    for (int slot = 0; slot < 4; ++slot) {
+        const bool tail = slot >= 2;
+        const int fs = slot & 1;
+        const uint64_t g = gunits[4 * p + slot];
+        if (g == 0) continue;
+        const unsigned long long form = fs ? kFormDelta : kFormList;
+        const int64_t reg = tail ? treg + gtoff[2 * p + fs] : hreg + ghoff[2 * p + fs];
+        for (uint64_t o = 0; o < g; o += kGatherChunk) {
+            const unsigned long long units = g - o < kGatherChunk ? g - o : kGatherChunk;
+            const unsigned long long d = ((unsigned long long)(reg + int64_t(o)) << 24) | (form << 22) | units;
+            const int cls = tail ? tail_class(cc, d) : hub_class(cc, d);
+            if (!FILL) atomicAdd(&c[cls], 1u);
+            else (tail ? ttask : htask).put((tail ? tbeg : hbeg)[p] + c[cls] + atomicAdd(&cur[p * kClasses + cls], 1u), d);
+        }
+        if (FILL) {
+            const uint4 filler = fs ? make_uint4(0u, 0u, 0u, 0u) : tail ? make_uint4(0xfffffffeu, 0xfffffffeu, 0xfffffffeu, 0xfffffffeu) : make_uint4(~0u, ~0u, ~0u, ~0u);
+            for (uint64_t o = g; o < gather_region_units(g); ++o) (tail ? tpool : spool)[reg + int64_t(o)] = filler;
+        }
+    }
+}
 template <bool FILL>
 __global__ __launch_bounds__(256) void k_task_lists(int64_t n_heavy, const int32_t *__restrict__ order, const int64_t *__restrict__ hoff,
                                                     const uint16_t *__restrict__ hadj, const int64_t *__restrict__ toff, const int32_t *__restrict__ tadj,
@@ -773,7 +845,8 @@
                                                     uint32_t *__restrict__ cnt, uint32_t *__restrict__ cur, const int64_t *__restrict__ hbeg,
                                                     const int64_t *__restrict__ tbeg, TaskList htask, TaskList ttask,
                                                     int32_t *__restrict__ tunits, unsigned long long *__restrict__ reversed, const uint32_t *__restrict__ spool,
-                                                    const uint32_t *__restrict__ tpool, int32_t inline_limit, int inline_first, int32_t core, int nparts, int part, TcClasses cc) {
+                                                    const uint32_t *__restrict__ tpool, int32_t inline_limit, int inline_first, int32_t core, int nparts, int part, TcClasses cc,
+                                                    const GatherPlan gp) {
     const int kClasses = cc.count();
     const int lane = threadIdx.x & 63;
     const int64_t wave0 = (int64_t(blockIdx.x) * blockDim.x + threadIdx.x) >> 6;
@@ -813,7 +886,24 @@
             }
             const bool fwd = v >= 0 && !reverse && own_u;
             if (reverse && nparts > 1 && shard_of(opos[v], nparts) != part) v = -1;
-            const unsigned long long fh = (fwd && i > 0) ? srow[v] : 0ull, fh2 = (fwd && i > 0) ? srow2[v] : 0ull, ft = (fwd && i > hl) ? trow[v] : 0ull;
+            unsigned long long fh = (fwd && i > 0) ? srow[v] : 0ull, fh2 = (fwd && i > 0) ? srow2[v] : 0ull, ft = (fwd && i > hl) ? trow[v] : 0ull;
+            if (gp.R > 0) {
+                const uint32_t mh = gather_moved_of(fh, gp.R), mh2 = gather_moved_of(fh2, gp.R), mt = gather_moved_of(ft, gp.R);
+                const int sh_ = gather_slot((uint32_t(fh) >> 22) & 3u), sh2_ = gather_slot((uint32_t(fh2) >> 22) & 3u), st_ = gather_slot((uint32_t(ft) >> 22) & 3u);
+                uint32_t *gc = (FILL ? gp.gcur : gp.gunits) + 4 * pos;
+                for (int slot = 0; slot < kGatherForms; ++slot) {
+                    const uint32_t a = sh_ == slot ? mh : 0u, b = sh2_ == slot ? mh2 : 0u, c = st_ == slot ? mt : 0u;
+                    const uint32_t at = claim_units(gc + slot, a + b, lane), att = claim_units(gc + 2 + slot, c, lane);
+                    if (FILL) {
+                        if (a) gather_copy(gp, false, pos, fh, a, at);
+                        if (b) gather_copy(gp, false, pos, fh2, b, at + a);
+                        if (c) gather_copy(gp, true, pos, ft, c, att);
+                    }
+                }
+                fh = mh ? gather_shrink(fh, mh) : fh;
+                fh2 = mh2 ? gather_shrink(fh2, mh2) : fh2;
+                ft = mt ? gather_shrink(ft, mt) : ft;
+            }
             const bool fh_on = (fh & 0x3fffffull) != 0, fh2_on = (fh2 & 0x3fffffull) != 0, ft_on = (ft & 0x3fffffull) != 0;
             const uint32_t sh = claim_by_class(FILL ? ru : cu, hub_class(cc, fh), fh_on, lane);
             const uint32_t sh2 = claim_by_class(FILL ? ru : cu, hub_class(cc, fh2), fh2_on, lane);
@@ -826,8 +916,19 @@
             kept += __popcll(__ballot(fwd));
             if (v >= 0 && reverse) {
                 const int64_t pv = opos[v];
-                const unsigned long long rh = ch ? (du_s & ~0x3fffffull) | ch : 0ull, rh2 = ch2 ? (du_s2 & ~0x3fffffull) | ch2 : 0ull,
-                                         rt = ct ? (du_t & ~0x3fffffull) | ct : 0ull;
+                unsigned long long rd[3] = {ch ? (du_s & ~0x3fffffull) | ch : 0ull, ch2 ? (du_s2 & ~0x3fffffull) | ch2 : 0ull, ct ? (du_t & ~0x3fffffull) | ct : 0ull};
+                if (gp.R > 0) {
+#pragma unroll
+                    for (int k = 0; k < 3; ++k) {
+                        const uint32_t mv = gather_moved_of(rd[k], gp.R);
+                        if (mv == 0) continue;
+                        const int slot = (k == 2 ? 2 : 0) + gather_slot((uint32_t(rd[k]) >> 22) & 3u);
+                        if (!FILL) atomicAdd(&gp.gunits[4 * pv + slot], mv);
+                        else gather_copy(gp, k == 2, pv, rd[k], mv, atomicAdd(&gp.gcur[4 * pv + slot], mv));
+                        rd[k] = gather_shrink(rd[k], mv);
+                    }
+                }
+                const unsigned long long rh = rd[0], rh2 = rd[1], rt = rd[2];
                 uint32_t *cv = cnt + pv * kClasses;
                 if (!FILL) {
                     if (rh) atomicAdd(&cv[hub_class(cc, rh)], 1u);
@@ -938,7 +1039,7 @@
     g->htask_entries = g->ttask_entries = g->hitems = g->titems = g->inline_hentries = g->inline_tentries = 0;
     g->n_ledge = g->ledge_total = 0;
     for (int c = 0; c < 8; ++c) g->lpack_base[c] = g->lpack_n[c] = g->lpack_total[c] = 0;
-    g->task_reverse = g->inline_units = g->spool_units = g->tpool_units = 0;
+    g->task_reverse = g->inline_units = g->spool_units = g->tpool_units = g->gather_units = 0;
     g->stats_part = g->stats_nparts = -1;
 }
 
@@ -1402,12 +1503,19 @@
         DevGuard g_uh{uh};
         if (int rc = dmalloc(&ut, n + 1, nullptr)) return rc;
         DevGuard g_ut{ut};
-        hipLaunchKernelGGL(k_inline_units, dim3(unsigned(n / 256 + 1)), dim3(256), 0, s, n, inl_h, inl_t, uh, ut);
+        hipLaunchKernelGGL(k_inline_units, dim3(unsigned(n / 256 + 1)), dim3(256), 0, s, n, inl_h, inl_t, false, uh, ut);
         if (int rc = exclusive_scan_i64(uh, ihoff, n + 1, s)) return rc;
         if (int rc = exclusive_scan_i64(ut, itoff, n + 1, s)) return rc;
         GMSX_HIP(hipMemcpy(&inline_h_units, ihoff + n, sizeof(int64_t), hipMemcpyDeviceToHost));
         GMSX_HIP(hipMemcpy(&inline_t_units, itoff + n, sizeof(int64_t), hipMemcpyDeviceToHost));
         g->inline_units = inline_h_units + inline_t_units;
+        if (g->tc_gather > 0) {
+            hipLaunchKernelGGL(k_inline_units, dim3(unsigned(n / 256 + 1)), dim3(256), 0, s, n, inl_h, inl_t, true, uh, ut);
+            if (int rc = exclusive_scan_i64(uh, ihoff, n + 1, s)) return rc;
+            if (int rc = exclusive_scan_i64(ut, itoff, n + 1, s)) return rc;
+            GMSX_HIP(hipMemcpy(&inline_h_units, ihoff + n, sizeof(int64_t), hipMemcpyDeviceToHost));
+            GMSX_HIP(hipMemcpy(&inline_t_units, itoff + n, sizeof(int64_t), hipMemcpyDeviceToHost));
+        }
     }
 
     pt.mark("inline row sizes");
@@ -1457,8 +1565,8 @@
         int64_t big_units = 0, small_units = 0;
         GMSX_HIP(hipMemcpy(&big_units, uoff + n2, sizeof(int64_t), hipMemcpyDeviceToHost));
         GMSX_HIP(hipMemcpy(&small_units, soff + n2, sizeof(int64_t), hipMemcpyDeviceToHost));
-        g->spool_units = big_units + small_units + inline_h_units;
-        inline_h_base = big_units + small_units;
+        inline_h_base = g->tc_gather > 0 ? int64_t(gather_region_units(uint64_t(big_units + small_units))) : big_units + small_units;
+        g->spool_units = inline_h_base + inline_h_units;
         if (g->spool_units >= (int64_t(1) << 40)) return GMSX_ERR_DEVICE_MEM;
         if (int rc = dmalloc(&g->srow, n, g)) return rc;
         if (int rc = dmalloc(&g->srow2, n, g)) return rc;
@@ -1497,7 +1605,7 @@
         int64_t big_units = 0, small_units = 0;
         GMSX_HIP(hipMemcpy(&big_units, uoff + n, sizeof(int64_t), hipMemcpyDeviceToHost));
         GMSX_HIP(hipMemcpy(&small_units, soff + n, sizeof(int64_t), hipMemcpyDeviceToHost));
-        inline_t_base = big_units + small_units;
+        inline_t_base = g->tc_gather > 0 ? int64_t(gather_region_units(uint64_t(big_units + small_units))) : big_units + small_units;
         g->tpool_units = inline_t_base + inline_t_units;
         if (g->tpool_units >= (int64_t(1) << 40)) return GMSX_ERR_DEVICE_MEM;
         if (int rc = dmalloc(&g->trow, n, g)) return rc;
@@ -1619,9 +1727,30 @@
         if (int rc = dmalloc(&g->tunits, n_heavy + 1, g)) return rc;
         GMSX_HIP(hipMemsetAsync(g->tunits, 0, size_t(n_heavy + 1) * sizeof(int32_t), s));
         unsigned long long *totals = nullptr;
-        if (int rc = dmalloc(&totals, 4, nullptr)) return rc;
+        if (int rc = dmalloc(&totals, 5, nullptr)) return rc;
         DevGuard g_tot{totals};
-        GMSX_HIP(hipMemsetAsync(totals, 0, 4 * sizeof(unsigned long long), s));
+        GMSX_HIP(hipMemsetAsync(totals, 0, 5 * sizeof(unsigned long long), s));
+        GatherPlan gp{};
+        gp.R = g->tc_gather;
+        g->gather_units = 0;
+        int64_t *ghsize = nullptr, *gtsize = nullptr, *ghoff = nullptr, *gtoff = nullptr;
+        DevGuard g_gu{nullptr}, g_gc{nullptr}, g_ghs{nullptr}, g_gts{nullptr}, g_gho{nullptr}, g_gto{nullptr};
+        if (gp.R > 0) {
+            if (int rc = dmalloc(&gp.gunits, 4 * n_recv + 1, nullptr)) return rc;
+            g_gu.p = gp.gunits;
+            if (int rc = dmalloc(&gp.gcur, 4 * n_recv + 1, nullptr)) return rc;
+            g_gc.p = gp.gcur;
+            if (int rc = dmalloc(&ghsize, 2 * n_recv + 1, nullptr)) return rc;
+            g_ghs.p = ghsize;
+            if (int rc = dmalloc(&gtsize, 2 * n_recv + 1, nullptr)) return rc;
+            g_gts.p = gtsize;
+            if (int rc = dmalloc(&ghoff, 2 * n_recv + 1, nullptr)) return rc;
+            g_gho.p = ghoff;
+            if (int rc = dmalloc(&gtoff, 2 * n_recv + 1, nullptr)) return rc;
+            g_gto.p = gtoff;
+            GMSX_HIP(hipMemsetAsync(gp.gunits, 0, size_t(4 * n_recv + 1) * sizeof(uint32_t), s));
+            GMSX_HIP(hipMemsetAsync(gp.gcur, 0, size_t(4 * n_recv + 1) * sizeof(uint32_t), s));
+        }
         int64_t *hcnt = nullptr, *tcnt = nullptr, *hbeg = nullptr, *tbeg = nullptr;
         if (int rc = dmalloc(&hcnt, n_recv + 1, nullptr)) return rc;
         DevGuard g_hc{hcnt};
@@ -1639,12 +1768,48 @@
             if (n > 0) hipLaunchKernelGGL(k_task_limits, dim3(vb), dim3(256), 0, s, n, g->srow, g->srow2, g->trow, hub_max, tail_max, totals + 3);
         }
         if (n > 0)
-            hipLaunchKernelGGL(k_inline_entries<false>, dim3(vb), dim3(256), 0, s, n, g->dplus, opos, lidx, n_heavy, g->inline_limit, ihoff, itoff, inline_h_base,
+            hipLaunchKernelGGL(k_inline_entries<false>, dim3(vb), dim3(256), 0, s, n, g->dplus, opos, lidx, n_heavy, g->inline_limit, ihoff, itoff, inl_h, inl_t, inline_h_base,
                                inline_t_base, cnt, cur, hbeg, tbeg, TaskList{}, TaskList{}, totals, cc);
         if (n_heavy > 0)
             hipLaunchKernelGGL(k_task_lists<false>, dim3(grid), dim3(256), 0, s, n_heavy, g->order, g->hoff, g->hadj, g->toff, g->tadj, g->dplus, g->srow, g->srow2, g->ksplit, g->trow,
                                two_sided, opos, cnt, cur, hbeg, tbeg, TaskList{}, TaskList{}, g->tunits,
-                               totals + 2, g->spool, g->tpool, g->inline_limit, g->inline_first, g->tc_core, g->shard_nparts, g->shard_part, cc);
+                               totals + 2, g->spool, g->tpool, g->inline_limit, g->inline_first, g->tc_core, g->shard_nparts, g->shard_part, cc, gp);
+        if (gp.R > 0) {
+            hipLaunchKernelGGL(k_gather_sizes, dim3(unsigned(2 * n_recv / 256 + 1)), dim3(256), 0, s, n_recv, gp.gunits, ghsize, gtsize, totals + 4);
+            if (int rc = exclusive_scan_i64(ghsize, ghoff, 2 * n_recv + 1, s)) return rc;
+            if (int rc = exclusive_scan_i64(gtsize, gtoff, 2 * n_recv + 1, s)) return rc;
+            int64_t gh_units = 0, gt_units = 0;
+            GMSX_HIP(hipMemcpy(&gh_units, ghoff + 2 * n_recv, sizeof(int64_t), hipMemcpyDeviceToHost));
+            GMSX_HIP(hipMemcpy(&gt_units, gtoff + 2 * n_recv, sizeof(int64_t), hipMemcpyDeviceToHost));
+            gp.hoff = ghoff;
+            gp.toff = gtoff;
+            gp.hreg = int64_t(gather_region_units(uint64_t(g->spool_units)));
+            gp.treg = int64_t(gather_region_units(uint64_t(g->tpool_units)));
+            if (gp.hreg + gh_units + kPoolSlack >= (int64_t(1) << 32) || gp.treg + gt_units + kPoolSlack >= (int64_t(1) << 32)) return GMSX_ERR_DEVICE_MEM;
+            auto grow = [&](uint32_t *&pool, int64_t &pool_units, int64_t reg, int64_t extra, uint32_t filler) -> int {
+                if (extra == 0) return GMSX_OK;
+                uint32_t *bigger = nullptr;
+                const int64_t units = reg + extra;
+                if (int rc = dmalloc(&bigger, (units + kPoolSlack) * 4, g)) return rc;
+                DevGuard g_b{bigger};
+                GMSX_HIP(hipMemcpyAsync(bigger, pool, size_t(pool_units) * 16, hipMemcpyDeviceToDevice, s));
+                if (reg > pool_units) GMSX_HIP(hipMemsetD32Async(reinterpret_cast<hipDeviceptr_t>(bigger + pool_units * 4), int(filler), size_t(reg - pool_units) * 4, s));
+                GMSX_HIP(hipMemsetD32Async(reinterpret_cast<hipDeviceptr_t>(bigger + units * 4), int(filler), size_t(kPoolSlack) * 4, s));
+                GMSX_HIP(hipStreamSynchronize(s));
+                g_b.p = pool;
+                g->device_bytes -= (pool_units + kPoolSlack) * 16;
+                pool = bigger;
+                pool_units = units;
+                return GMSX_OK;
+            };
+            if (int rc = grow(g->spool, g->spool_units, gp.hreg, gh_units, 0u)) return rc;
+            if (int rc = grow(g->tpool, g->tpool_units, gp.treg, gt_units, 0xFFFFFFFEu)) return rc;
+            gp.spool = reinterpret_cast<uint4 *>(g->spool);
+            gp.tpool = reinterpret_cast<uint4 *>(g->tpool);
+            if (n_recv > 0)
+                hipLaunchKernelGGL(k_gather_entries<false>, dim3(unsigned(n_recv / 256 + 1)), dim3(256), 0, s, n_recv, gp.gunits, ghoff, gtoff, gp.hreg, gp.treg, cnt, cur, hbeg,
+                                   tbeg, TaskList{}, TaskList{}, gp.spool, gp.tpool, cc);
+        }
         pt.mark("task lists count");
         hipLaunchKernelGGL(k_list_sizes, dim3(unsigned(n_recv / 256 + 1)), dim3(256), 0, s, n_recv, cnt, hcnt, tcnt, cc);
         if (int rc = exclusive_scan_i64(hcnt, hbeg, n_recv + 1, s)) return rc;
@@ -1657,17 +1822,21 @@
         g->inline_hentries = int64_t(tot[0]);
         g->inline_tentries = int64_t(tot[1]);
         g->task_reverse = int64_t(tot[2]);
+        if (gp.R > 0) GMSX_HIP(hipMemcpy(&g->gather_units, totals + 4, sizeof(int64_t), hipMemcpyDeviceToHost));
         if (g->htask_entries >= (int64_t(1) << 40) || g->ttask_entries >= (int64_t(1) << 40)) return GMSX_ERR_DEVICE_MEM;
         if (int rc = dmalloc(&g->htask.lo, g->htask_entries + 2, g)) return rc;
         if (int rc = dmalloc(&g->htask.hi, g->htask_entries + 2, g)) return rc;
         if (int rc = dmalloc(&g->ttask.lo, g->ttask_entries + 2, g)) return rc;
         if (int rc = dmalloc(&g->ttask.hi, g->ttask_entries + 2, g)) return rc;
         if (n > 0)
-            hipLaunchKernelGGL(k_inline_entries<true>, dim3(vb), dim3(256), 0, s, n, g->dplus, opos, lidx, n_heavy, g->inline_limit, ihoff, itoff, inline_h_base,
+            hipLaunchKernelGGL(k_inline_entries<true>, dim3(vb), dim3(256), 0, s, n, g->dplus, opos, lidx, n_heavy, g->inline_limit, ihoff, itoff, inl_h, inl_t, inline_h_base,
                                inline_t_base, cnt, cur, hbeg, tbeg, g->htask, g->ttask, totals, cc);
         if (n_heavy > 0)
             hipLaunchKernelGGL(k_task_lists<true>, dim3(grid), dim3(256), 0, s, n_heavy, g->order, g->hoff, g->hadj, g->toff, g->tadj, g->dplus, g->srow, g->srow2, g->ksplit, g->trow,
-                               two_sided, opos, cnt, cur, hbeg, tbeg, g->htask, g->ttask, g->tunits, totals + 2, g->spool, g->tpool, g->inline_limit, g->inline_first, g->tc_core, g->shard_nparts, g->shard_part, cc);
+                               two_sided, opos, cnt, cur, hbeg, tbeg, g->htask, g->ttask, g->tunits, totals + 2, g->spool, g->tpool, g->inline_limit, g->inline_first, g->tc_core, g->shard_nparts, g->shard_part, cc, gp);
+        if (gp.R > 0 && n_recv > 0)
+            hipLaunchKernelGGL(k_gather_entries<true>, dim3(unsigned(n_recv / 256 + 1)), dim3(256), 0, s, n_recv, gp.gunits, ghoff, gtoff, gp.hreg, gp.treg, cnt, cur, hbeg,
+                               tbeg, g->htask, g->ttask, gp.spool, gp.tpool, cc);
         pt.mark("task lists fill");
         const int hub_phases = cc.hub_phases();
         const int64_t slots = int64_t(hub_phases) * n_recv;
@@ -1714,17 +1883,26 @@
 }
 
 static int build_tc_once(gmsx_graph *g) {
-    g->tc_base_bytes = g->device_bytes;
-    g->tc_building = true;
-    const int rc = build_tc_sets(g);
-    g->tc_building = false;
-    g->tc_bytes = g->device_bytes - g->tc_base_bytes;
-    if (rc) {
+    const bool fixed = opt("TC_GATHER") != nullptr;
+    const int tries[3] = {fixed ? std::max(0, std::min(kGatherMax, int(opt_int("TC_GATHER", kTcGatherDefault)))) : kTcGatherDefault, 3, 0};
+    int rc = GMSX_OK;
+    for (int k = 0; k < (fixed ? 1 : 3); ++k) {
+        if (k > 0 && tries[k] >= tries[k - 1]) continue;
+        g->tc_gather = tries[k];
+        g->tc_base_bytes = g->device_bytes;
+        g->tc_building = true;
+        rc = build_tc_sets(g);
+        g->tc_building = false;
+        g->tc_bytes = g->device_bytes - g->tc_base_bytes;
+        if (rc == GMSX_OK) {
+            g->tc_ready = true;
+            return GMSX_OK;
+        }
         free_tc(g);
-        return rc;
-    }
-    g->tc_ready = true;
-    return GMSX_OK;
+        if (rc != GMSX_ERR_DEVICE_MEM) return rc;
+        (void)hipGetLastError();
+    }
+    return rc;
 }
 
 int ensure_tc(const gmsx_graph *cg) {
diff --git a/gms_amd/csrc/hip/device_graph.hpp b/gms_amd/csrc/hip/device_graph.hpp
--- a/gms_amd/csrc/hip/device_graph.hpp
+++ b/gms_amd/csrc/hip/device_graph.hpp
@@ -88,6 +88,8 @@
     int inline_first = 64;
     int32_t inline_limit = 0;
     int64_t inline_units = 0;
+    int tc_gather = 0;
+    int64_t gather_units = 0;
     unsigned long long *trow = nullptr;
     uint32_t *tpool = nullptr;
     int64_t tpool_units = 0;
diff --git a/gms_amd/csrc/hip/tc.hip b/gms_amd/csrc/hip/tc.hip
--- a/gms_amd/csrc/hip/tc.hip
+++ b/gms_amd/csrc/hip/tc.hip
@@ -854,6 +854,7 @@
     const int64_t wave0 = (int64_t(blockIdx.x) * blockDim.x + threadIdx.x) >> 6;
     const int64_t nwaves = (int64_t(gridDim.x) * blockDim.x) >> 6;
     unsigned long long c[15] = {0, 0, 0, 0, 0, 0, 0, 0, 0, 0, 0, 0, 0, 0, 0};
+    unsigned long long lines = 0, partial = 0;
     for (int64_t q = wave0; q < hitems + titems; q += nwaves) {
         const bool tail = q >= hitems;
         const gmsx_tc_item &it = tail ? titem[q - hitems] : hitem[q];
@@ -872,6 +873,9 @@
             if (tail) c[fd == kFormDelta ? 4 : 3] += db;
             else c[fd == kFormList ? 0 : fd == kFormBitset ? 1 : 2] += db;
             c[5] += 6;
+            const unsigned long long first = d >> 24, end = first + (d & 0x3fffffull);
+            lines += ((end + 7) >> 3) - (first >> 3);
+            partial += ((tail || fd != kFormBitset) && (end & 7ull)) ? 1 : 0;
         }
     }
     for (int64_t pos = first_light + wave0; pos < end_light; pos += nwaves) {
@@ -900,6 +904,12 @@
         for (int s = 32; s > 0; s >>= 1) x += __shfl_down(x, s);
         if (lane == 0 && x) atomicAdd(&out[k], x);
     }
+    for (int s = 32; s > 0; s >>= 1) {
+        lines += __shfl_down(lines, s);
+        partial += __shfl_down(partial, s);
+    }
+    if (lane == 0 && lines) atomicAdd(&out[18], 128ull * lines);
+    if (lane == 0 && partial) atomicAdd(&out[19], partial);
 }
 
 __device__ __forceinline__ int hist_bin(unsigned long long units) {
@@ -1278,6 +1288,8 @@
         GMSX_HIP(hipGetLastError());
         out21[7] = uint64_t(g->inline_units) * 16ull;
         out21[12] = uint64_t(g->inline_hentries + g->inline_tentries);
+        out21[17] = uint64_t(g->gather_units) * 16ull;
+        out21[20] = uint64_t(g->tc_gather);
         out21[15] = core_bytes_of(g, 0, 1);
         out21[16] = uint64_t(g->tc_core);
         return GMSX_OK;
diff --git a/gms_amd/csrc/host/loader.cpp b/gms_amd/csrc/host/loader.cpp
--- a/gms_amd/csrc/host/loader.cpp
+++ b/gms_amd/csrc/host/loader.cpp
@@ -677,7 +677,7 @@
     {"INLINE_LIMIT", "", false}, {"TC_INLINE_FIRST", "", false}, {"TC_DELTA", "", false}, {"TC_DELTA_PCT", "", false}, {"TC_GAP12", "", false},
     {"TC_HYBRID", "", false}, {"TC_TAIL_DELTA", "", false}, {"TC_TWO_SIDED", "", false}, {"TC_HOT_WINDOWS", "", false}, {"TC_HOT_KB", "", false},
     {"TC_HOT_MIN", "", false}, {"TC_TEST_MAX_UNITS", "", false}, {"TC_KEEP_ROWS", "", false}, {"TC_MEM_LIMIT_MB", "", false}, {"TC_OVERLAP", "", false},
-    {"TC_PERSIST", "", false}, {"TC_ITEM_WGS", "", false}, {"TC_CORE", "", false}, {"TC_LIGHT_PACKED", "", false}, {"SORT_CHUNK", "", false}, {"UPLOAD_STAGED", "", false}, {"INIT_LAZY", "", false},
+    {"TC_PERSIST", "", false}, {"TC_ITEM_WGS", "", false}, {"TC_CORE", "", false}, {"TC_LIGHT_PACKED", "", false}, {"TC_GATHER", "", false}, {"SORT_CHUNK", "", false}, {"UPLOAD_STAGED", "", false}, {"INIT_LAZY", "", false},
     {"KC_SLAB_MB", "", false}, {"KC_MAXD", "", false}, {"KC_STREAMS", "", false},
     {"KC_REVERSE", "", false}, {"KC_REV_MIN", "", false}, {"KC_REV_FACTOR", "", false}, {"KC_REV_TAIL", "", false}, {"KC_REV_TAIL_MIN", "", false}, {"KC_TRI", "", false}, {"KC_MFMA", "", false}, {"KC_POOL_MB", "", false},
     {"BK_MAXC", "", false}, {"BK_ARENA_MB", "", false}, {"BK_GROUPS", "", false}, {"BK_SMALL_P", "", false}, {"BK_SMALL_P_GROUPS", "", false},
diff --git a/gms_amd/csrc/host/tc_gather_plan.hpp b/gms_amd/csrc/host/tc_gather_plan.hpp
--- /dev/null
+++ b/gms_amd/csrc/host/tc_gather_plan.hpp
@@ -0,0 +1,38 @@
+#pragma once
+#include <cstdint>
+
+#if defined(__HIPCC__) || defined(__CUDACC__)
+#define GMSX_GATHER_HD __host__ __device__
+#else
+#define GMSX_GATHER_HD
+#endif
+
+namespace gmsx {
+
+constexpr uint32_t kGatherLineUnits = 8;
+constexpr uint32_t kGatherChunk = 64;
+constexpr int kGatherMax = 7;
+constexpr int kTcGatherDefault = 7;
+constexpr int kGatherForms = 2;
+constexpr uint32_t kGatherFormList = 0, kGatherFormBitset = 1, kGatherFormDelta = 2, kGatherFormGap12 = 3;
+
+GMSX_GATHER_HD inline bool gather_form_moves(uint32_t form) { return form == kGatherFormList || form == kGatherFormDelta; }
+GMSX_GATHER_HD inline int gather_slot(uint32_t form) { return form == kGatherFormDelta ? 1 : 0; }
+
+GMSX_GATHER_HD inline uint32_t gather_moved(uint64_t first, uint32_t units, uint32_t form, int R) {
+    if (R <= 0 || units == 0 || !gather_form_moves(form)) return 0;
+    const uint32_t r = uint32_t((first + units) & (kGatherLineUnits - 1));
+    if (r == 0 || r > uint32_t(R > kGatherMax ? kGatherMax : R)) return 0;
+    if (units < kGatherLineUnits && units <= uint32_t(R)) return units;
+    return r < units ? r : 0;
+}
+GMSX_GATHER_HD inline unsigned long long gather_shrink(unsigned long long d, uint32_t moved) {
+    const uint32_t units = uint32_t(d) & 0x3fffffu;
+    return moved >= units ? 0ull : d - moved;
+}
+GMSX_GATHER_HD inline uint32_t gather_moved_of(unsigned long long d, int R) {
+    return gather_moved(d >> 24, uint32_t(d) & 0x3fffffu, (uint32_t(d) >> 22) & 3u, R);
+}
+GMSX_GATHER_HD inline uint64_t gather_region_units(uint64_t g) { return (g + kGatherLineUnits - 1) & ~uint64_t(kGatherLineUnits - 1); }
+
+}
```

After: 18.25 billion, median of 6. +9.7%, better.
